# smu-ivpl/FastInterCU-VVC

Measured on AMD Instinct MI355X. Metric: CU-inferences/sec (batch 4096, 128x128), higher is better.
Workload: dtype f16 (fp32 accumulate)

## Files before the change

fastintercu-vvc_amd/csrc/mlt_dispatch.cpp:

```cpp
#include "mlt_runtime.h"

const char *tuning_env(const char *name) {
  const char *e = std::getenv("MLT_TUNING");
  return (e && e[0] == '1') ? std::getenv(name) : nullptr;
}

const Tuning &tuning() {
  static const Tuning t = [] {
    auto num = [](const char *name, long dflt) { const char *e = tuning_env(name); return e ? std::atol(e) : dflt; };
    auto on = [](const char *name) { return tuning_env(name) != nullptr; };
    auto cap = [&](const char *name) { const long v = num(name, 0); return (int)(v > 0 ? v : 256); };
    Tuning u{};
    u.debug_dump_dir = tuning_env("MLT_DEBUG_DUMP_DIR");
    u.xl_kill = (int)num("MLT_XL_KILL", 0); u.xl_kill_layer = (int)num("MLT_XL_KILL_LAYER", -1);
    u.lat_pixels = num("MLT_LAT_PIXELS", 16384L);
    u.no_exact_lat = on("MLT_NO_EXACT_LAT"); u.exact_patch_big = !on("MLT_EXACT_PATCH_64K");
    u.wg_cap = cap("MLT_WG_CAP"); u.wg_cap0 = cap("MLT_WG_CAP0"); u.wg_cap1 = cap("MLT_WG_CAP1"); u.wg_cap2 = cap("MLT_WG_CAP2");
    u.l0_mfma32 = on("MLT_L0_MFMA32"); u.l1_mfma32 = !on("MLT_L1_MFMA16");
    u.no_block_fusion = on("MLT_NO_BLOCK_FUSION");
    u.no_chain = on("MLT_NO_CHAIN") || u.no_block_fusion; u.no_chain_s2 = on("MLT_NO_CHAIN_S2"); u.no_c16 = on("MLT_NO_C16"); u.chain64 = !on("MLT_NO_CHAIN64");
    u.no_l0_s5 = on("MLT_NO_L0_S5");
    u.l0_stream_min = on("MLT_NO_L0_STREAM") ? 0 : (int)num("MLT_L0_STREAM_MIN", 128);
    u.l1_stream_min = on("MLT_NO_L1_STREAM") ? 0 : (int)num("MLT_L1_STREAM_MIN", 128);
    u.guard_wait_mode = on("MLT_GUARD_SPIN_WAIT") ? 1 : on("MLT_GUARD_BLOCKING_WAIT") ? 2 : 0;
    u.no_small_mix = on("MLT_NO_SMALL_MIX"); u.no_mag_guard = on("MLT_NO_MAG_GUARD");
    u.no_graph = on("MLT_NO_GRAPH") || u.debug_dump_dir != nullptr;
    return u;
  }();
  return t;
}

namespace {

int gap_slots(int hw) { return hw >= 32 ? hw / 32 : 1; }

size_t ws_per_cu(const mlt::Model &m, int S, bool some_exact = false) {
  const int h0 = S / 2 > 0 ? S / 2 : 1;
  const int planes = (m.exact || some_exact) ? 2 : 1;
  size_t b = 4 * ((size_t)h0 * h0 * 32 * 2 * planes + 256);
  int h = S;
  for (int s = 0; s < m.n_stages; ++s) {
    h = h / 2 > 0 ? h / 2 : 1;
    b += (size_t)h * h * m.planes[s] * 2 * planes + 256;
    if (s >= 1) b += (size_t)gap_slots(h * h) * m.planes[s] * 4 + 256;
  }
  return b + 4096;
}

int ensure_ws(mlt_ctx *ctx, size_t bytes) {
  if (bytes <= ctx->ws_bytes) return MLT_OK;
  if (ctx->ws) { HIP_TRY(ctx, hipStreamSynchronize(ctx->stream)); (void)hipFree(ctx->ws); ctx->ws = nullptr; ctx->ws_bytes = 0; }
  ++ctx->ws_gen;
  HIP_TRY(ctx, hipMalloc((void **)&ctx->ws, bytes));
  ctx->ws_bytes = bytes;
  return MLT_OK;
}
}
void release_ws(mlt_ctx *ctx) {
  if (ctx->ws) { (void)hipFree(ctx->ws); ctx->ws = nullptr; ctx->ws_bytes = 0; }
  ++ctx->ws_gen;
}
namespace {

int debug_dump(mlt_ctx *ctx, const char *name, const void *dptr, size_t bytes) {
  const char *dir = tuning().debug_dump_dir;
  static int seq = 0;
  if (!dir) return MLT_OK;
  std::vector<char> host(bytes);
  HIP_TRY(ctx, hipStreamSynchronize(ctx->stream));
  HIP_TRY(ctx, hipMemcpy(host.data(), dptr, bytes, hipMemcpyDeviceToHost));
  char path[1200];
  std::snprintf(path, sizeof path, "%s/%02d_%s.bin", dir, seq++, name);
  if (FILE *f = std::fopen(path, "wb")) { std::fwrite(host.data(), 1, bytes, f); std::fclose(f); }
  return MLT_OK;
}

}

int Launch::prof_begin(const std::string &name, double flops, double bytes, hipEvent_t &e0, hipEvent_t &e1, const char *variant) {
  if (ctx->plan) { ctx->plan->push_back(variant && variant[0] ? name + " [" + variant + "]" : name); return MLT_OK; }
  if (!ctx->profile) return MLT_OK;
  auto it = ctx->prof.find(name);
  if (it == ctx->prof.end()) { ctx->prof_order.push_back(name); it = ctx->prof.emplace(name, ProfAcc()).first; }
  it->second.launches++; it->second.flops += flops; it->second.bytes += bytes;
  HIP_TRY(ctx, hipEventCreate(&e0));
  HIP_TRY(ctx, hipEventCreate(&e1));
  it->second.ev.emplace_back(e0, e1);
  HIP_TRY(ctx, hipEventRecord(e0, ctx->stream));
  return MLT_OK;
}
int Launch::prof_end(hipEvent_t e1) {
  if (!ctx->profile) return MLT_OK;
  HIP_TRY(ctx, hipEventRecord(e1, ctx->stream));
  return MLT_OK;
}

namespace {

void plan_note(mlt_ctx *ctx, std::initializer_list<std::pair<const char *, const void *>> ptrs, std::initializer_list<std::pair<const char *, long>> vals = {}) {
  if (!ctx->plan || !ctx->plan_detail || ctx->plan->empty()) return;
  std::string t = " {";
  char b[64];
  bool first = true;
  for (const auto &q : ptrs) {
    if (!q.second) continue;
    std::snprintf(b, sizeof b, "%s%s=0x%llx", first ? "" : " ", q.first, (unsigned long long)(uintptr_t)q.second);
    t += b; first = false;
  }
  for (const auto &q : vals) {
    std::snprintf(b, sizeof b, "%s%s=%ld", first ? "" : " ", q.first, q.second);
    t += b; first = false;
  }
  ctx->plan->back() += t + "}";
}

struct ConvIO {
  const void *x = nullptr;
  void *y = nullptr;
  void *y_sc = nullptr;
  const void *res = nullptr;
  float *gap = nullptr;
  bool relu = false;
  bool y_c16 = false;
  bool ysc_c16 = false;
  size_t x_lo = 0, y_lo = 0, res_lo = 0, ysc_lo = 0;
};

int run_conv(mlt_ctx *ctx, const mlt::PackedConv &pc, int n, int hin, const ConvIO &io, int *hout_out) {
  const int hout = hin / pc.stride > 0 ? hin / pc.stride : 1;
  *hout_out = hout;
  ConvArgs a{};
  a.x = io.x; a.y = io.y; a.w = pc.d_w; a.bias = pc.d_bias; a.res = io.res; a.n = n; a.relu = io.relu ? 1 : 0;
  a.y_sc = io.y_sc; a.bias_sc = pc.d_bias_sc; a.acc_scale = pc.acc_scale; a.y_c16 = io.y_c16 ? 1 : 0; a.ysc_c16 = io.ysc_c16 ? 1 : 0;
  a.hin_l = ilog2(hin); a.hout_l = ilog2(hout);
  a.x_lo_off = io.x_lo; a.y_lo_off = io.y_lo; a.res_lo_off = io.res_lo; a.ysc_lo_off = io.ysc_lo; a.w_lo_off = pc.plane_halves * 2;
  a.lo8_scale = 0x01010101 * ((127 - pc.lo8_exp) & 0xFF);
  a.xl_sa0 = 0x01010101 * ((127 - pc.xl_ewl) & 0xFF); a.xl_sa1 = 0x01010101 * ((127 - pc.xl_ewh) & 0xFF); a.xl_sb1 = 0x01010101 * (127 - 12);
  { const int kill = tuning().xl_kill, only = tuning().xl_kill_layer;
    if (only < 0 || only == pc.cin * 1000 + pc.cout) { if (kill & 1) a.xl_sa0 = 0; if (kill & 2) a.xl_sb1 = 0; } }
  const long lat_px = tuning().lat_pixels;
  const bool no_exact_lat = tuning().no_exact_lat;
  const bool lat = !(pc.exact && no_exact_lat) && pc.lat && hout >= 8 && (pc.w2 ? pc.stride == 1 : (long)n * hout * hout <= lat_px);
  const int dma = (pc.exact || pc.w2 || lat) ? 0 : (pc.dma == 1 && hout >= 16) ? 1 : (pc.dma == 2 && hout >= 8) ? 2 : 0;
  const int MT = lat ? 128 : dma == 2 ? pc.mt_dma : pc.mt;
  const int nsplit = pc.xl ? 6 : pc.exact ? 2 : pc.w2 ? 4 : 1;
  const int act_planes = (nsplit == 2 || nsplit == 6) ? 2 : 1;
  int tw = hout < 32 ? hout : 32;
  int th = MT / tw < hout ? MT / tw : hout;
  int spw = MT / (tw * th);
  const int halo = pc.taps == 9 ? 3 : 1;
  const int PS = pc.kc * 2 + 16;
  const int ph = (th - 1) * pc.stride + halo, pw = (tw - 1) * pc.stride + halo;
  int half = pc.stride == 2 ? (pw + 1) / 2 : 0;
  if (pc.stride == 2 && tw == 8 && (2 * half) % 4 != 2) ++half;
  int rp = pc.stride == 2 ? 2 * half : pw;
  if (pc.stride == 1 && tw == 8) while (rp % 4 != 2) ++rp;
  size_t patch_budget = 64 * 1024;
  if (nsplit == 2 || nsplit == 6) {
    const int tt = pc.taps + (pc.has_sc ? 1 : 0), nbuf = tt / pc.gt > 1 ? 2 : 1;
    const size_t ring = (size_t)nbuf * 2 * pc.gt * (pc.kc / 16) * (pc.ct / 32) * 1024;
    const bool big = tuning().exact_patch_big;
    if (big && ring + 64 * 1024 < 160 * 1024) patch_budget = 160 * 1024 - ring;
  }
  while (spw > 1 && (((size_t)spw * ph * rp * PS + 1023) / 1024 * 1024) * act_planes > patch_budget) spw /= 2;
  a.tw_l = ilog2(tw); a.th_l = ilog2(th); a.spw_l = ilog2(spw);
  a.ph = ph; a.pw = pw; a.rp = rp; a.half = half;
  auto magic = [](int d) { return d < 2 ? 0u : (uint32_t)((0x100000000ull + d - 1) / d); };
  a.pw_magic = magic(pw); a.ph_magic = magic(ph);
  a.patch_bytes = (int)((((size_t)spw * ph * rp * PS) + 1023) / 1024 * 1024);
  if (dma) {
    a.patch_bytes = (int)((((size_t)spw * ph * rp * pc.kc * 2) + 1023) / 1024 * 1024);
    a.rp_magic = magic(rp);
    a.zero = ctx->zero_page;
  }
  const int extra_lds = 0;
  const int hw = hout * hout;
  a.gap = io.gap; a.gap_slots = gap_slots(hw); a.gap_l = hw >= 32 ? 5 : ilog2(hw);
  a.ntiles = ((n + spw - 1) / spw) * (hout / th) * (hout / tw);
  const int wg_cap = tuning().wg_cap;
  const int gt = (nsplit == 4 && !lat) ? pc.gt_w2 : pc.gt;
  const bool persistent = (gt == pc.taps + (pc.has_sc ? 1 : 0) && pc.cin == pc.kc) || dma == 2;
  const int cap = dma == 2 ? wg_cap * ((pc.mt_dma >= 256 || pc.stride == 2) ? 1 : 2) / (pc.cout / pc.ct) : wg_cap;
  const int grid_x = (persistent && a.ntiles > cap) ? cap : a.ntiles;
  char name[48];
  std::snprintf(name, sizeof name, "conv3x3_s%d_%dto%d_h%d%s", pc.stride, pc.cin, pc.cout, hout, pc.has_sc ? "+sc" : "");
  const double px = (double)n * hw;
  const double flops = 2.0 * px * pc.cout * pc.cin * (pc.taps + (pc.has_sc ? 1 : 0));
  const double in_bytes = (double)n * hin * hin * pc.cin * 2;
  const double bytes = in_bytes + px * pc.cout * 2 * ((io.y ? 1 : 0) + (io.y_sc ? 1 : 0) + (io.res ? 1 : 0)) + (double)pc.w.size() * 2;
  Launch L{ctx};
  hipEvent_t e0 = nullptr, e1 = nullptr;
  char variant[96];
  std::snprintf(variant, sizeof variant, "%s%s%s%s%s", nsplit == 1 ? "single pass" : nsplit == 2 ? "exact" : nsplit == 4 ? "hi+lo weights" : nsplit == 6 ? "exact-lite" : "?",
                pc.taps == 1 ? ", centre tap" : lat ? ", latency tiles" : dma == 1 ? ", resident weights + LDS-DMA patches" : dma == 2 ? ", weight ring + LDS-DMA" : "",
                io.y_c16 ? ", y chunk-major" : "", io.ysc_c16 ? ", sc chunk-major" : "", io.gap ? ", GAP" : "");
  int rc = L.prof_begin(name, flops, bytes, e0, e1, variant);
  if (rc) return rc;
  plan_note(ctx, {{"x", io.x}, {"y", io.y}, {"y_sc", io.y_sc}, {"res", io.res}, {"gap", io.gap}},
            {{"x_lo", (long)io.x_lo}, {"y_lo", (long)io.y_lo}, {"res_lo", (long)io.res_lo}, {"ysc_lo", (long)io.ysc_lo}, {"relu", io.relu}, {"grid", grid_x}});
  LAUNCH_TRY(ctx, mlt_launch_conv(pc.cin, pc.cout, pc.stride, nsplit, pc.taps == 1 ? MLT_CONV_CENTRE : lat ? MLT_CONV_LATENCY : dma ? MLT_CONV_DMA : MLT_CONV_DEFAULT, a, grid_x, extra_lds, ctx->stream));
  if ((rc = L.prof_end(e1))) return rc;
  if (io.y && (rc = debug_dump(ctx, name, io.y, (size_t)px * pc.cout * 2))) return rc;
  if (io.y_sc && (rc = debug_dump(ctx, (std::string(name) + "_sc").c_str(), io.y_sc, (size_t)px * pc.cout * 2))) return rc;
  return MLT_OK;
}

int run_stem5(mlt_ctx *ctx, const mlt::PackedConv &pc, int n, int S, const Planes &pl, void *y, void *y_sc, size_t lo_off) {
  const int hout = S / 2;
  Stem5Args a{};
  pl.fill(a);
  a.w = pc.d_w; a.bias = pc.d_bias; a.bias_sc = pc.d_bias_sc; a.y = y; a.y_sc = y_sc;
  a.y_lo_off = lo_off; a.ysc_lo_off = lo_off; a.w_lo_off = pc.plane_halves * 2; a.acc_scale = pc.acc_scale;
  a.n = n; a.s_l = ilog2(S); a.hout_l = ilog2(hout);
  const int MT = 256;
  const int tw = hout < 32 ? hout : 32;
  const int th = MT / tw < hout ? MT / tw : hout;
  const int spw = MT / (tw * th);
  a.tw_l = ilog2(tw); a.th_l = ilog2(th); a.spw_l = ilog2(spw);
  a.rh = 2 * th + 3; a.rw = 2 * tw + 3; a.halfw = (a.rw + 1) / 2;
  a.rw_magic = (uint32_t)((0x100000000ull + a.rw - 1) / a.rw);
  a.rh_magic = (uint32_t)((0x100000000ull + a.rh - 1) / a.rh);
  const int lds = spw * a.rh * 2 * a.halfw * 4;
  const int grid_x = ((n + spw - 1) / spw) * (hout / th) * (hout / tw);
  char name[48];
  std::snprintf(name, sizeof name, "stem5x5_s2_2to32_h%d+sc", hout);
  const double px = (double)n * hout * hout;
  Launch L{ctx};
  hipEvent_t e0 = nullptr, e1 = nullptr;
  int rc = L.prof_begin(name, 2.0 * px * 32 * (50 + 18), (double)n * S * S * 4 + px * 32 * 2 * 2, e0, e1, pc.xl ? "exact-lite" : pc.exact ? "exact" : pc.w2 ? "hi+lo weights" : "single pass");
  if (rc) return rc;
  plan_note(ctx, {{"y", y}, {"y_sc", y_sc}}, {{"lo", (long)lo_off}, {"grid", grid_x}});
  LAUNCH_TRY(ctx, mlt_launch_stem5(a, pc.exact ? 2 : pc.w2 ? 3 : 1, grid_x, lds, ctx->stream));
  if ((rc = L.prof_end(e1))) return rc;
  if ((rc = debug_dump(ctx, name, y, (size_t)px * 32 * 2))) return rc;
  return debug_dump(ctx, (std::string(name) + "_sc").c_str(), y_sc, (size_t)px * 32 * 2);
}

int run_stem_block(mlt_ctx *ctx, const mlt::Model &m, int n, int S, const Planes &pl, void *y, int32_t *d_flat, bool flat_is_clear) {
  const int h = S / 2;
  const mlt::PackedConv &c2 = m.blocks[0][0].conv2;
  StemBlockArgs a{};
  pl.fill(a);
  a.w = m.stem_b.d_w; a.w2 = c2.d_w; a.bias = m.stem.d_bias; a.bias_sc = m.stem.d_bias_sc; a.bias2 = c2.d_bias; a.y = y;
  a.flat = d_flat;
  a.w_lo_off = m.stem_b.plane_halves * 2; a.w2_lo_off = c2.plane_halves * 2; a.scale2 = c2.acc_scale;
  if (d_flat && !flat_is_clear) LAUNCH_TRY(ctx, hipMemsetAsync(d_flat, 0, (size_t)n * 4, ctx->stream));
  a.acc_scale = m.stem.acc_scale; a.n = n; a.hout_l = ilog2(h); a.ntiles = n * (h / 16) * (h / 32);
  const int wg_cap = tuning().wg_cap2;
  const int grid_x = a.ntiles > wg_cap ? wg_cap : a.ntiles;
  char name[48];
  std::snprintf(name, sizeof name, "stem+block_s2_2to32_h%d(layer0.0)", h);
  const double px = (double)n * h * h;
  Launch L{ctx};
  hipEvent_t e0 = nullptr, e1 = nullptr;
  int rc = L.prof_begin(name, 2.0 * px * 32 * (50 + 18 + 288), (double)n * S * S * 4 + px * 32 * 2, e0, e1, m.w2 ? "hi+lo weights" : "single pass");
  if (rc) return rc;
  plan_note(ctx, {{"y", y}, {"flat", d_flat}}, {{"flat_is_clear", flat_is_clear}, {"grid", grid_x}});
  LAUNCH_TRY(ctx, mlt_launch_stem_block(a, m.w2, grid_x, ctx->stream));
  if ((rc = L.prof_end(e1))) return rc;
  return debug_dump(ctx, name, y, (size_t)px * 32 * 2);
}

int run_layer0_stream(mlt_ctx *ctx, const mlt::Model &m0, const mlt::Model &m1, int n, const Planes &pl, void *y, int32_t *d_flat, bool flat_is_clear,
                      const mlt::PackedConv *c5, void *y_t, void *y_sc) {
  const mlt::PackedConv &c2 = m0.blocks[0][0].conv2;
  const mlt::Block &B1 = m1.blocks[0][1];
  Layer0Args a{};
  pl.fill(a);
  a.w = m0.stem_b.d_w; a.w2 = c2.d_w; a.w3 = B1.conv1.d_w; a.w4 = B1.conv2.d_w;
  a.bias = m0.stem.d_bias; a.bias_sc = m0.stem.d_bias_sc; a.bias2 = c2.d_bias; a.bias3 = B1.conv1.d_bias; a.bias4 = B1.conv2.d_bias;
  a.y = y; a.flat = d_flat; a.acc_scale = m0.stem.acc_scale; a.n = n;
  if (c5) { a.w5 = c5->d_w; a.bias5 = c5->d_bias; a.bias5_sc = c5->d_bias_sc; a.scale5 = c5->acc_scale; a.y_t = y_t; a.y_sc = y_sc; }
  if (d_flat && !flat_is_clear) LAUNCH_TRY(ctx, hipMemsetAsync(d_flat, 0, (size_t)n * 4, ctx->stream));
  const int wg_cap = tuning().wg_cap0;
  const int grid_x = n > wg_cap ? wg_cap : n;
  const double px = (double)n * 64 * 64;
  Launch L{ctx};
  hipEvent_t e0 = nullptr, e1 = nullptr;
  int rc = c5 ? L.prof_begin("layer0_stream_h64(stem+layer0+layer1.0.conv1+sc)", 2.0 * px * 32 * (50 + 18 + 3 * 288) + 2.0 * (px / 4) * 64 * (288 + 32),
                             (double)n * 128 * 128 * 4 + (px / 4) * 64 * 2 * 2, e0, e1)
              : L.prof_begin("layer0_stream_h64(stem+layer0.0+layer0.1)", 2.0 * px * 32 * (50 + 18 + 3 * 288), (double)n * 128 * 128 * 4 + px * 32 * 2, e0, e1);
  if (rc) return rc;
  const bool mfma32 = tuning().l0_mfma32;
  plan_note(ctx, {{"y", c5 ? nullptr : y}, {"y_t", c5 ? y_t : nullptr}, {"y_sc", c5 ? y_sc : nullptr}, {"flat", d_flat}}, {{"flat_is_clear", flat_is_clear}, {"grid", grid_x}});
  LAUNCH_TRY(ctx, mlt_launch_layer0_stream(a, c5 != nullptr, mfma32, grid_x, ctx->stream));
  if ((rc = L.prof_end(e1))) return rc;
  if (c5) {
    if ((rc = debug_dump(ctx, "conv3x3_s2_32to64_h32+sc", y_t, (size_t)(px / 4) * 64 * 2))) return rc;
    return debug_dump(ctx, "conv3x3_s2_32to64_h32+sc_sc", y_sc, (size_t)(px / 4) * 64 * 2);
  }
  return debug_dump(ctx, "block_s1_32_h64(conv1+conv2)", y, (size_t)px * 32 * 2);
}

int run_block32(mlt_ctx *ctx, const mlt::Block &B, int n, int h, const void *x, void *y) {
  Block32Args a{};
  const bool w2 = B.conv1.w2;
  a.x = x; a.y = y; a.w1 = B.conv1.d_w; a.w2 = B.conv2.d_w; a.bias1 = B.conv1.d_bias; a.bias2 = B.conv2.d_bias;
  a.w1_lo_off = B.conv1.plane_halves * 2; a.w2_lo_off = B.conv2.plane_halves * 2; a.scale1 = B.conv1.acc_scale; a.scale2 = B.conv2.acc_scale;
  a.n = n; a.h_l = ilog2(h); a.ntiles = n * (h / (w2 ? 8 : 16)) * (h / 32);
  const int wg_cap = tuning().wg_cap;
  const int grid_x = a.ntiles > wg_cap ? wg_cap : a.ntiles;
  char name[48];
  std::snprintf(name, sizeof name, "block_s1_32_h%d(conv1+conv2)", h);
  const double px = (double)n * h * h;
  Launch L{ctx};
  hipEvent_t e0 = nullptr, e1 = nullptr;
  int rc = L.prof_begin(name, 2.0 * px * 32 * 32 * 9 * 2, px * 32 * 2 * 2 + 2.0 * 18 * 1024, e0, e1, w2 ? "hi+lo weights" : "single pass");
  if (rc) return rc;
  plan_note(ctx, {{"x", x}, {"y", y}}, {{"grid", grid_x}});
  LAUNCH_TRY(ctx, mlt_launch_block32(a, w2, grid_x, ctx->stream));
  if ((rc = L.prof_end(e1))) return rc;
  return debug_dump(ctx, name, y, (size_t)px * 32 * 2);
}

int run_chain3(mlt_ctx *ctx, const mlt::Block &B0, const mlt::Block &B1, int n, int h, const void *t, const void *sc, void *y, float *gap,
               const void *s2_in, bool x_c16, bool y_c16, void *b0_hbm, bool sc_c16) {
  const int c = B0.conv2.cout;
  ChainArgs a{};
  a.x = s2_in ? s2_in : t; a.nconv = 3; a.y = y; a.gap = gap; a.n = n; a.zero = ctx->zero_page;
  a.x_c16 = x_c16 ? 1 : 0; a.y_c16 = y_c16 ? 1 : 0; a.res0_c16 = sc_c16 ? 1 : 0;
  const mlt::PackedConv *pcs[3] = {&B0.conv2, &B1.conv1, &B1.conv2};
  const bool w2 = B0.conv2.w2;
  for (int k = 0; k < 3; ++k) {
    a.cv[k].w = pcs[k]->d_w; a.cv[k].bias = pcs[k]->d_bias; a.cv[k].acc_scale = pcs[k]->acc_scale; a.cv[k].relu = 1;
    a.cv[k].w_lo_off = pcs[k]->plane_halves * 2;
    a.cv[k].lo8_scale = 0x01010101 * ((127 - pcs[k]->lo8_exp) & 0xFF);
  }
  a.cv[0].res_mode = s2_in ? 2 : 1; a.cv[0].res = sc; a.cv[0].save = 1; a.cv[2].res_mode = 2;
  if (c == 64) {
    a.cv[0].save = 0; a.cv[0].y = b0_hbm; a.cv[2].res_mode = 1; a.cv[2].res = b0_hbm;
  }
  if (s2_in) {
    const mlt::PackedConv &p2 = B0.conv1_s2c;
    a.s2_w = p2.d_w; a.s2_bias = p2.d_bias; a.s2_bias_sc = p2.d_bias_sc; a.s2_scale = p2.acc_scale;
  }
  const int hw = h * h;
  a.gap_slots = gap_slots(hw); a.gap_l = hw >= 32 ? 5 : ilog2(hw);
  const int wg_cap = tuning().wg_cap;
  const int spw = c == 256 ? 2 : 1;
  const int ntiles = (n + spw - 1) / spw;
  const int grid_x = ntiles > wg_cap ? wg_cap : ntiles;
  char name[48];
  std::snprintf(name, sizeof name, s2_in ? "stage_%d_h%d(s2+sc,conv2,conv1,conv2)" : "chain3_s1_%d_h%d(conv2+conv1+conv2)", c, h);
  const double px = (double)n * hw;
  const double flops = 3.0 * 2.0 * px * c * c * 9 + (s2_in ? 2.0 * px * c * (c / 2) * 10 : 0.0);
  const double bytes = (s2_in ? px * 4 * (c / 2) * 2 : px * c * 2 * 2) + (y ? px * c * 2 : 0.0) + 3.0 * (double)B0.conv2.w.size() * 2 +
                       (s2_in ? (double)B0.conv1_s2c.w.size() * 2 : 0.0);
  Launch L{ctx};
  hipEvent_t e0 = nullptr, e1 = nullptr;
  char variant[96];
  std::snprintf(variant, sizeof variant, "%s%s%s%s%s", w2 ? "hi+lo weights" : "single pass", x_c16 ? ", x chunk-major" : "", sc_c16 ? ", sc chunk-major" : "", y_c16 ? ", y chunk-major" : "",
                gap ? ", GAP" : "");
  int rc = L.prof_begin(name, flops, bytes, e0, e1, variant);
  if (rc) return rc;
  plan_note(ctx, {{"x", a.x}, {"sc", s2_in ? nullptr : sc}, {"y", y}, {"gap", gap}, {"b0", c == 64 ? b0_hbm : nullptr}}, {{"grid", grid_x}});
  LAUNCH_TRY(ctx, mlt_launch_chain(c, h, s2_in != nullptr, ctx->lds_oob_zero, w2, a, grid_x, ctx->stream));
  if ((rc = L.prof_end(e1))) return rc;
  if (y && (rc = debug_dump(ctx, name, y, (size_t)px * c * 2))) return rc;
  return MLT_OK;
}

int run_layer1_stream(mlt_ctx *ctx, const mlt::Block &B0, const mlt::Block &B1, int n, const void *t, const void *sc, void *y, float *gap, bool y_c16) {
  Layer1Args a{};
  a.t = t; a.sc = sc; a.y = y; a.y_c16 = y_c16 ? 1 : 0; a.gap = gap; a.gap_slots = gap_slots(32 * 32); a.n = n;
  const mlt::PackedConv *pcs[3] = {&B0.conv2, &B1.conv1, &B1.conv2};
  for (int k = 0; k < 3; ++k) { a.w[k] = pcs[k]->d_w; a.bias[k] = pcs[k]->d_bias; a.scale[k] = pcs[k]->acc_scale; }
  const int wg_cap = tuning().wg_cap1;
  const int grid_x = n > wg_cap ? wg_cap : n;
  const double px = (double)n * 32 * 32;
  Launch L{ctx};
  hipEvent_t e0 = nullptr, e1 = nullptr;
  int rc = L.prof_begin("layer1_stream_h32(conv2+conv1+conv2)", 3.0 * 2.0 * px * 64 * 64 * 9, px * 64 * 2 * 3 + 3.0 * 72 * 1024, e0, e1, y_c16 ? "single pass, y chunk-major, GAP" : "single pass, GAP");
  if (rc) return rc;
  const bool mfma32 = tuning().l1_mfma32;
  plan_note(ctx, {{"t", t}, {"sc", sc}, {"y", y}, {"gap", gap}}, {{"grid", grid_x}});
  LAUNCH_TRY(ctx, mlt_launch_layer1_stream(a, mfma32, grid_x, ctx->stream));
  if ((rc = L.prof_end(e1))) return rc;
  return debug_dump(ctx, "chain3_s1_64_h32(conv2+conv1+conv2)", y, (size_t)px * 64 * 2);
}

enum : unsigned { CLS_QUADS = 1u, CLS_FLAT = 2u, CLS_L0_STREAM = 4u, CLS_L1_STREAM = 8u, CLS_CHAIN0 = 16u  };
unsigned batch_class(const NetCfg &c, int n, const Planes &pl, bool has_flat) {
  const Tuning &tn = tuning();
  unsigned cls = 0;
  if (pl.aligned8()) cls |= CLS_QUADS;
  if (has_flat) cls |= CLS_FLAT;
  if (tn.l0_stream_min > 0 && n >= tn.l0_stream_min) cls |= CLS_L0_STREAM;
  if (tn.l1_stream_min > 0 && n >= tn.l1_stream_min) cls |= CLS_L1_STREAM;
  for (int s = 1; s < c.m->n_stages; ++s) {
    const int h = c.h_in(s), ho = h / 2 > 0 ? h / 2 : 1;
    if ((long)n * ho * ho > tn.lat_pixels) cls |= CLS_CHAIN0 << s;
  }
  return cls;
}


NetPlan plan_network(const mlt_ctx *ctx, const NetCfg &c, unsigned cls) {
  const Tuning &tn = tuning();
  const mlt::Model &m = *c.m;
  NetPlan P;
  auto add = [&](PlanStep::Kind k, int s) -> PlanStep & { PlanStep st{}; st.kind = k; st.s = (int8_t)s; P.push_back(st); return P.back(); };
  auto wants_chain = [&](int s) -> bool {
    if (s <= 0 || s >= m.n_stages || tn.no_chain || !(cls & (CLS_CHAIN0 << s))) return false;
    const mlt::Model &mm = c.model_of(s, 1);
    if (mm.exact || (mm.w2 && !ctx->lds_oob_zero)) return false;
    const int h = c.h_in(s), ho = h / 2 > 0 ? h / 2 : 1;
    const mlt::PackedConv &c2 = mm.blocks[s][0].conv2;
    const bool packing_ok = (m.planes[s] == 64 ? (c2.ct == 64 && c2.gt == 9 && tn.chain64) : (c2.ct == 128 && c2.gt == 3)) && (!mm.w2 || c2.lo8 || m.planes[s] == 64);
    return mlt_chain_supported(m.planes[s], ho) && c2.taps == 9 && c2.kc == 64 && packing_ok;
  };
  auto wants_s2 = [&](int s) -> bool {
    if (!wants_chain(s) || tn.no_chain_s2 || c.model_of(s, 0).w2 || c.model_of(s, 1).w2) return false;
    const mlt::PackedConv &p2 = c.model_of(s, 0).blocks[s][0].conv1_s2c;
    return ctx->plan ? !p2.w.empty() : p2.d_w != nullptr;
  };
  bool cur_c16 = false;
  bool l0_front = false;
  for (int s = 0; s < m.n_stages; ++s) {
    const bool last = s == m.n_stages - 1;
    const mlt::Model &ms = c.model_of(s, 0);
    const mlt::Model &mt = c.model_of(s, 1);
    const int h = c.h_in(s), ho = h / 2 > 0 ? h / 2 : 1;
    const bool fused_b0 = s == 0 && !ms.exact && ho >= 32 && !tn.no_block_fusion && (cls & CLS_QUADS);
    if (s == 0 && (cls & CLS_FLAT) && !fused_b0) add(PlanStep::FLAT_STAT, 0);
    if (fused_b0 && ho == 64 && !ms.w2 && !mt.exact && !mt.w2 && (cls & CLS_L0_STREAM)) {
      const mlt::Model &m10 = c.model_of(1, 0);
      const mlt::PackedConv &c5 = m10.blocks[1][0].conv1;
      l0_front = !tn.no_l0_s5 && m.n_stages > 1 && !m10.exact && !m10.w2 && wants_chain(1) && !wants_s2(1) && m.planes[1] == 64 && !tn.no_c16 &&
                 c5.has_sc && c5.taps == 9 && c5.kc == 32 && c5.ct == 64 && c5.cin == 32 && c5.cout == 64 && c5.stride == 2;
      add(PlanStep::LAYER0_STREAM, 0).front = l0_front;
      continue;
    }
    if (fused_b0) add(PlanStep::STEM_BLOCK, 0);
    else {
      const bool chain = wants_chain(s), chain_s2 = wants_s2(s);
      bool sc_c16 = false;
      if (s == 0) add(PlanStep::STEM5, 0);
      else if (chain_s2) {}
      else if (s == 1 && l0_front) sc_c16 = true;
      else {
        sc_c16 = chain && m.planes[s] == 64 && !tn.no_c16 && !ms.exact;
        add(PlanStep::CONV_S2, s).sc_c16 = sc_c16;
      }
      if (chain) {
        const bool out_c16 = !last && !tn.no_c16 && wants_s2(s + 1);
        const mlt::PackedConv &q2 = mt.blocks[s][0].conv2;
        const bool stream = s == 1 && !chain_s2 && m.planes[s] == 64 && ho == 32 && sc_c16 && !mt.w2 && !mt.exact && (cls & CLS_L1_STREAM) &&
                            q2.taps == 9 && q2.kc == 64 && q2.ct == 64 && !last;
        PlanStep &st = add(stream ? PlanStep::LAYER1_STREAM : PlanStep::CHAIN, s);
        st.inside_s2 = chain_s2; st.x_c16 = cur_c16; st.sc_c16 = sc_c16; st.y_c16 = out_c16;
        cur_c16 = out_c16;
        continue;
      }
      add(PlanStep::CONV_B0C2, s);
    }
    if (s == 0 && !mt.exact && ho >= 32 && !tn.no_block_fusion) { add(PlanStep::BLOCK32, 0); continue; }
    add(PlanStep::CONV_B1C1, s);
    PlanStep &st = add(PlanStep::CONV_B1C2, s);
    st.y_c16 = !last && !tn.no_c16 && wants_s2(s + 1);
    cur_c16 = st.y_c16;
  }
  add(PlanStep::HEADS, m.n_stages - 1);
  return P;
}

}

int run_network(mlt_ctx *ctx, SizeState &st, const NetCfg &c, int n, const PassIO &io, const GuardOut &go) {
  const int S = st.size;
  mlt::Model &m = *c.m;
  const unsigned cls = batch_class(c, n, io.pl, go.d_flat != nullptr);
  NetPlan fresh;
  const NetPlan *plan;
  if (st.loaded && !ctx->plan) {
    const PlanKey key{c.m, c.mback, c.mx, c.back_mask, c.x_units, cls};
    auto it = st.plans.find(key);
    if (it == st.plans.end()) it = st.plans.emplace(key, plan_network(ctx, c, cls)).first;
    plan = &it->second;
  } else {
    fresh = plan_network(ctx, c, cls);
    plan = &fresh;
  }
  int rc = ctx->plan ? MLT_OK : ensure_ws(ctx, ws_per_cu(m, S, c.x_units != 0) * (size_t)n);
  if (rc) return rc;
  char *p = ctx->ws;
  auto carve = [&](size_t bytes) { char *r = p; p += (bytes + 255) / 256 * 256; return (void *)r; };
  const int h0 = S / 2 > 0 ? S / 2 : 1;
  const int nplanes = (m.exact || c.x_units) ? 2 : 1;
  void *pool[4];
  for (int i = 0; i < 4; ++i) pool[i] = carve((size_t)n * h0 * h0 * 32 * 2 * nplanes);
  void *outs[5];
  float *gaps[5] = {nullptr, nullptr, nullptr, nullptr, nullptr};
  {
    int h = S;
    for (int s = 0; s < m.n_stages; ++s) {
      h = h / 2 > 0 ? h / 2 : 1;
      outs[s] = carve((size_t)n * h * h * m.planes[s] * 2 * nplanes);
      if (s >= 1) gaps[s] = (float *)carve((size_t)n * gap_slots(h * h) * m.planes[s] * 4);
    }
  }
  Launch L{ctx};
  const bool quad_ok = (cls & CLS_QUADS) != 0;
  for (const PlanStep &ps : *plan) {
    const int s = ps.s;
    const bool last = s == m.n_stages - 1;
    mlt::Model &ms = c.model_of(s, 0), &mt = c.model_of(s, 1);
    const int h = c.h_in(s), ho = h / 2 > 0 ? h / 2 : 1;
    const void *cur = s > 0 ? outs[s - 1] : nullptr;
    const bool ex0 = ms.exact, ex1 = mt.exact;
    const size_t lo_in = ex0 ? (size_t)n * h * h * (s == 0 ? 32 : m.planes[s - 1]) * 2 : 0;
    const size_t lo_st = (ex0 || ex1) ? (size_t)n * ho * ho * m.planes[s] * 2 : 0;
    const bool in_has_lo = s > 0 && c.model_of(s - 1, 1).exact;
    const bool b0_has_lo = s == 0 ? ex0 : ex1;
    int hh = 0;
    ConvIO cv;
    switch (ps.kind) {
    case PlanStep::FLAT_STAT: {
      FlatStatArgs fa{};
      io.pl.fill(fa);
      fa.flat = go.d_flat; fa.n = n; fa.s_l = ilog2(S);
      hipEvent_t e0 = nullptr, e1 = nullptr;
      if ((rc = L.prof_begin("guard_flat_stat", 0.0, (double)n * S * S * 4, e0, e1))) return rc;
      plan_note(ctx, {{"flat", go.d_flat}}, {{"quads", quad_ok}});
      LAUNCH_TRY(ctx, mlt_launch_flat_stat(fa, quad_ok, ctx->stream));
      rc = L.prof_end(e1);
      break;
    }
    case PlanStep::LAYER0_STREAM:
      rc = run_layer0_stream(ctx, ms, mt, n, io.pl, outs[0], go.d_flat, go.flat_is_clear,
                             ps.front ? &c.model_of(1, 0).blocks[1][0].conv1 : nullptr, pool[0], pool[1]);
      break;
    case PlanStep::STEM_BLOCK:
      rc = run_stem_block(ctx, ms, n, S, io.pl, pool[2], go.d_flat, go.flat_is_clear);
      break;
    case PlanStep::STEM5:
      rc = run_stem5(ctx, ms.stem, n, S, io.pl, pool[0], pool[1], lo_st);
      break;
    case PlanStep::CONV_S2:
      cv.x = cur; cv.y = pool[0]; cv.y_sc = pool[1]; cv.relu = true;
      cv.x_lo = in_has_lo ? lo_in : 0; cv.y_lo = lo_st; cv.ysc_lo = lo_st;
      cv.ysc_c16 = ps.sc_c16;
      rc = run_conv(ctx, ms.blocks[s][0].conv1, n, h, cv, &hh);
      break;
    case PlanStep::CHAIN:
      rc = run_chain3(ctx, mt.blocks[s][0], mt.blocks[s][1], n, ho, pool[0], pool[1], last ? nullptr : outs[s], gaps[s], ps.inside_s2 ? cur : nullptr,
                      ps.x_c16, ps.y_c16, pool[2], ps.sc_c16);
      break;
    case PlanStep::LAYER1_STREAM:
      rc = run_layer1_stream(ctx, mt.blocks[s][0], mt.blocks[s][1], n, pool[0], pool[1], outs[s], gaps[s], ps.y_c16);
      break;
    case PlanStep::CONV_B0C2:
      cv.x = pool[0]; cv.y = pool[2]; cv.res = pool[1]; cv.relu = true;
      cv.x_lo = cv.y_lo = cv.res_lo = lo_st;
      if (s > 0 && ex1 && !ex0) cv.x_lo = cv.res_lo = 0;
      rc = run_conv(ctx, (s == 0 ? ms : mt).blocks[s][0].conv2, n, ho, cv, &hh);
      break;
    case PlanStep::BLOCK32:
      rc = run_block32(ctx, mt.blocks[0][1], n, ho, pool[2], outs[0]);
      break;
    case PlanStep::CONV_B1C1:
      cv.x = pool[2]; cv.y = pool[3]; cv.relu = true;
      cv.x_lo = cv.y_lo = lo_st;
      if (!b0_has_lo) cv.x_lo = 0;
      rc = run_conv(ctx, mt.blocks[s][1].conv1, n, ho, cv, &hh);
      break;
    case PlanStep::CONV_B1C2:
      cv.x = pool[3]; cv.y = last ? nullptr : outs[s]; cv.res = pool[2]; cv.relu = true; cv.gap = gaps[s];
      cv.x_lo = cv.y_lo = cv.res_lo = lo_st;
      if (!b0_has_lo) cv.res_lo = 0;
      cv.y_c16 = ps.y_c16;
      rc = run_conv(ctx, mt.blocks[s][1].conv2, n, ho, cv, &hh);
      break;
    case PlanStep::HEADS: {
      HeadArgs ha{};
      for (int t = 1; t < m.n_stages; ++t) {
        const int hd = t - 1, hs = c.h_in(t + 1);
        ha.gap[hd] = gaps[t]; ha.slots[hd] = gap_slots(hs * hs); ha.w[hd] = m.heads[hd].d_w; ha.b[hd] = m.heads[hd].d_b;
        ha.c[hd] = m.planes[t]; ha.hw[hd] = hs * hs; ha.classes[hd] = m.heads[hd].classes;
      }
      ha.n_heads = m.n_heads; ha.decision_head = st.head_index; ha.poc = io.poc; ha.qp = io.qp; ha.logits = io.logits; ha.split = io.split;
      ha.mag = go.d_mag;
      ha.dec = io.dec; ha.min_conf = st.min_conf;
      ha.cand = io.cand; ha.cand_cov = st.cand_cov; ha.cand_max = st.cand_max;
      const GuardTail *tail = go.tail;
      if (tail && (n == 1 || tail->next)) {
        ha.g_conf_band = tail->conf_band; ha.g_cand_band = tail->cand_band;
        ha.g_next = tail->next;
        ha.g_count = tail->count; ha.g_idx = tail->idx; ha.g_flat = tail->flat; ha.g_flat_thr = tail->flat_thr; ha.g_near_thr = tail->near_thr; ha.g_margin = tail->margin;
        ha.g_mag_thr = tail->mag_thr;
      }
      hipEvent_t e0 = nullptr, e1 = nullptr;
      if (io.sweep.n_qps > 0) {
        HeadSweepArgs sa{};
        sa.h = ha; sa.h.mag = nullptr;
        sa.n_qps = io.sweep.n_qps; sa.slab = io.sweep.slab; sa.fix_idx = io.sweep.idx; sa.mask = io.sweep.mask; sa.active = io.sweep.idx ? nullptr : io.sweep.active;
        std::memcpy(sa.qps, io.sweep.qps, sizeof sa.qps);
        if ((rc = L.prof_begin("heads_sweep", 0.0, 0.0, e0, e1))) return rc;
        LAUNCH_TRY(ctx, mlt_launch_heads_sweep(sa, n, ctx->stream));
        rc = L.prof_end(e1);
        break;
      }
      if ((rc = L.prof_begin("heads", 0.0, 0.0, e0, e1))) return rc;
      plan_note(ctx, {{"gap0", ha.gap[0]}, {"gap1", ha.gap[1]}, {"gap2", ha.gap[2]}, {"gap3", ha.gap[3]}},
                {{"slots0", ha.slots[0]}, {"slots1", ha.slots[1]}, {"slots2", ha.slots[2]}, {"slots3", ha.slots[3]}, {"c0", ha.c[0]}, {"c1", ha.c[1]}, {"c2", ha.c[2]}, {"c3", ha.c[3]},
                 {"hw0", ha.hw[0]}, {"hw1", ha.hw[1]}, {"hw2", ha.hw[2]}, {"hw3", ha.hw[3]}, {"heads", ha.n_heads}});
      LAUNCH_TRY(ctx, mlt_launch_heads(ha, n, ctx->stream));
      rc = L.prof_end(e1);
      break;
    }
    }
    if (rc) return rc;
  }
  return MLT_OK;
}

extern "C" {
#pragma GCC visibility push(default)

int mlt_plan_describe(const void *blob, size_t bytes, int size, int n, int tier, unsigned w2_units, unsigned x_units, int aligned, char *out, size_t cap) {
  const int si = size_index(size);
  if (!blob || !out || cap == 0 || si < 0 || n <= 0) return -1;
  mlt_ctx ctx;
  std::vector<std::string> plan;
  ctx.plan = &plan;
  ctx.plan_detail = (aligned & 2) != 0;
  ctx.lds_oob_zero = true;
  SizeState &st = ctx.sz[si];
  st.size = size; st.enabled = st.loaded = true;
  st.head_index = size == 128 ? 2 : 0;
  std::string err;
  const bool whole_exact = tier == 1 || tier == 5;
  if (!mlt::build_model(blob, bytes, tier == 5 ? mlt::MLT_MODEL_XLITE : tier == 1 ? mlt::MLT_MODEL_EXACT : mlt::MLT_MODEL_FAST, size, st.model, err)) return -1;
  if (!whole_exact && w2_units && !mlt::build_model(blob, bytes, mlt::MLT_MODEL_W2, size, st.model_w2, err)) return -1;
  if (!whole_exact && x_units && !mlt::build_model(blob, bytes, mlt::MLT_MODEL_EXACT, size, st.model_exact, err)) return -1;
  st.exact = whole_exact;
  st.w2 = !whole_exact && w2_units != 0; st.w2_units = st.w2 ? w2_units : 0; st.x_units = whole_exact ? 0 : x_units;
  const int16_t *planes = (const int16_t *)(uintptr_t)((aligned & 1) ? 0x1000 : 0x1002);
  int32_t *const flat_fake = (int32_t *)(uintptr_t)0x2000;
  ctx.ws = (char *)(uintptr_t)0x100000000ull;
  GuardOut go;
  go.d_flat = whole_exact ? nullptr : flat_fake;
  const int rc = run_network(&ctx, st, st.main_cfg(), n, PassIO{Planes::dense(planes, planes, size), nullptr, nullptr, nullptr, nullptr, nullptr}, go);
  ctx.ws = nullptr;
  if (rc) return -1;
  size_t pos = 0;
  for (const std::string &l : plan) {
    if (pos + l.size() + 2 > cap) return -1;
    std::memcpy(out + pos, l.data(), l.size());
    pos += l.size();
    out[pos++] = '\n';
  }
  out[pos] = 0;
  return (int)plan.size();
}

#pragma GCC visibility pop
}
```

fastintercu-vvc_amd/csrc/mlt_kernels.h:

```cpp
#pragma once
#include <hip/hip_runtime.h>
#include <stdint.h>

#define MLT_MAX_HEADS_K 4
#define MLT_MAX_LOGITS_K 16
#define MLT_FLAT_RANGE 6
#define MLT_FLAT_EXACT_SHIFT 16

struct ConvArgs {
  const void *x;
  void *y;
  const void *w;
  const float *bias;
  const void *res;
  const void *zero;
  int n;
  int ntiles;
  int hin_l, hout_l;
  int tw_l, th_l, spw_l;
  int ph, pw, rp, half;
  uint32_t pw_magic, ph_magic, rp_magic;
  int patch_bytes;
  int relu;
  int y_c16;
  int ysc_c16;
  float acc_scale;
  void *y_sc;
  const float *bias_sc;
  float *gap;
  int gap_slots, gap_l;
  size_t x_lo_off, y_lo_off, res_lo_off, ysc_lo_off, w_lo_off;
  int lo8_scale;
  int xl_sa0, xl_sa1, xl_sb1;
};

struct ConvCfg { int kc, ct, mt, gt, dma, mt_dma, lat, gt_w2; };

struct Stem5Args {
  const int16_t *org, *pred;
  long org_row_stride, org_cu_stride, pred_row_stride, pred_cu_stride;
  const void *w;
  const float *bias, *bias_sc;
  void *y, *y_sc;
  size_t y_lo_off, ysc_lo_off, w_lo_off;
  float acc_scale;
  int n, s_l, hout_l, tw_l, th_l, spw_l;
  int rh, rw, halfw;
  uint32_t rw_magic, rh_magic;
};

struct Block32Args {
  const void *x;
  void *y;
  const void *w1, *w2;
  const float *bias1, *bias2;
  int n, h_l, ntiles;
  size_t w1_lo_off, w2_lo_off;
  float scale1, scale2;
};

struct StemBlockArgs {
  const int16_t *org, *pred;
  long org_row_stride, org_cu_stride, pred_row_stride, pred_cu_stride;
  const void *w;
  const void *w2;
  const float *bias, *bias_sc, *bias2;
  void *y;
  int32_t *flat;
  float acc_scale;
  int n, hout_l, ntiles;
  size_t w_lo_off, w2_lo_off;
  float scale2;
};

#define MLT_L0F_LDS_BYTES 161040
#define MLT_L0_LDS_BYTES 145872
struct Layer0Args {
  const int16_t *org, *pred;
  long org_row_stride, org_cu_stride, pred_row_stride, pred_cu_stride;
  const void *w;
  const void *w2, *w3, *w4;
  const float *bias, *bias_sc, *bias2, *bias3, *bias4;
  void *y;
  int32_t *flat;
  float acc_scale;
  int n;
  const void *w5;
  const float *bias5, *bias5_sc;
  void *y_t, *y_sc;
  float scale5;
};

#define MLT_L1_LDS_BYTES 159008
struct Layer1Args {
  const void *t;
  const void *sc;
  const void *w[3];
  const float *bias[3];
  float scale[3];
  void *y;
  int y_c16;
  float *gap;
  int gap_slots, n;
};

struct ChainConv {
  const void *w;
  size_t w_lo_off;
  int lo8_scale;
  const float *bias;
  float acc_scale;
  int relu;
  int res_mode;
  int save;
  const void *res;
  void *y;
};
struct ChainArgs {
  const void *x;
  const void *s2_w;
  const float *s2_bias, *s2_bias_sc;
  float s2_scale;
  const void *zero;
  ChainConv cv[3];
  int nconv;
  void *y;
  int y_c16;
  int x_c16;
  int res0_c16;
  float *gap;
  int gap_slots, gap_l;
  int n;
};
hipError_t mlt_launch_chain(int c, int h, bool with_s2, bool oob_zero, bool w2, const ChainArgs &a, int grid_x, hipStream_t st);
bool mlt_chain_supported(int c, int h);
hipError_t mlt_probe_lds_oob(int *d_ok, hipStream_t st);
bool mlt_stage_supported(int c, int h);

struct DecisionRec {
  int32_t split_mode, raw_mode;
  float confidence, margin;
  int32_t level_mode[MLT_MAX_HEADS_K];
  float level_conf[MLT_MAX_HEADS_K];
};
#define MLT_CONF_BAND_FRAC 0.75f

#define MLT_MAX_CAND_K 6
struct CandRec {
  uint32_t mask;
  int32_t count;
  int8_t order[8];
  float prob[MLT_MAX_CAND_K];
};

struct HeadArgs {
  const float *gap[MLT_MAX_HEADS_K];
  int slots[MLT_MAX_HEADS_K];
  const float *w[MLT_MAX_HEADS_K];
  const float *b[MLT_MAX_HEADS_K];
  int c[MLT_MAX_HEADS_K], hw[MLT_MAX_HEADS_K], classes[MLT_MAX_HEADS_K];
  int n_heads, decision_head;
  const int32_t *poc, *qp;
  float *logits;
  int32_t *split;
  DecisionRec *dec;
  float min_conf, g_conf_band;
  CandRec *cand;
  float cand_cov, g_cand_band;
  int cand_max;
  int32_t *g_count, *g_idx, *g_flat;
  int g_flat_thr, g_near_thr;
  float g_margin;
  float *mag;
  float g_mag_thr;
  int32_t *g_next;
};

#define MLT_SWEEP_MAX_QPS_K 32
struct HeadSweepArgs {
  HeadArgs h;
  int32_t qps[MLT_SWEEP_MAX_QPS_K];
  int n_qps;
  long slab;
  const int32_t *fix_idx;
  uint32_t *mask;
  const uint32_t *active;
};

struct FlatStatArgs {
  const int16_t *org, *pred;
  long org_row_stride, org_cu_stride, pred_row_stride, pred_cu_stride;
  int32_t *flat;
  int n, s_l;
};
struct GuardSelectArgs {
  const int32_t *flat;
  const float *logits;
  int32_t *idx;
  int32_t *count;
  int n, n_logits, head_off, head_classes;
  int flat_thr;
  int near_thr;
  float margin;
  const float *mag;
  float mag_thr;
  float min_conf, conf_band;
  float cand_cov, cand_band;
  int cand_max;
};
struct GuardGatherArgs {
  const int16_t *org, *pred;
  long org_row_stride, org_cu_stride, pred_row_stride, pred_cu_stride;
  const int32_t *poc, *qp, *idx;
  int16_t *g_org, *g_pred;
  int32_t *g_poc, *g_qp;
  int k, s_l;
};
struct GuardScatterArgs {
  const int32_t *idx, *g_split;
  const float *g_logits;
  int32_t *split;
  float *logits;
  int k, n_logits;
  const DecisionRec *g_dec;
  DecisionRec *dec;
  const CandRec *g_cand;
  CandRec *cand;
};
struct PictureGatherArgs {
  const int16_t *org, *pred;
  long org_pitch, pred_pitch;
  const int32_t *xy;
  int16_t *g_org, *g_pred;
  int c, s_l;
  int vec_org, vec_pred;
};
hipError_t mlt_launch_picture_gather(const PictureGatherArgs &a, hipStream_t st);
#define MLT_TREES_LEVELS 4
#define MLT_TREES_ROW 15
struct TreeNodeRec {
  int32_t x, y;
  int16_t size;
  int8_t depth;
  uint8_t flags;
  int32_t parent, first_child, split_mode;
  float confidence;
  uint32_t cand_mask;
};
struct TreesEntry {
  const int16_t *org, *pred;
  long org_pitch, pred_pitch;
  int32_t vec_org, vec_pred;
  int32_t poc, qp;
};
struct TreesSegs { int32_t *start, *n, *pack_base; };
struct TreeExpandArgs {
  TreeNodeRec *nodes;
  int32_t *xy;
  int32_t *pic;
  int node_cap;
  int lvl_start, lvl_n;
  int size;
  int lvl, n_levels;
  const DecisionRec *dec;
  const CandRec *cand;
  const float *logits;
  int n_logits, head_off, head_classes;
  uint32_t descend_mask;
  int by_candidates;
  const int32_t *next_roots;
  int n_next_roots, root_flags;
  int32_t *count;
  TreesSegs segs;
  int n_pictures;
  int32_t *first_node;
};
struct TreeRasterArgs {
  const TreeNodeRec *nodes;
  const int32_t *pic;
  int lvl_start, lvl_n;
  int blk_l;
  uint8_t *map;
  size_t map_bytes;
  int map_w, map_h;
};
struct PictureGatherMultiArgs {
  const TreesEntry *entries;
  const int32_t *pic;
  const int32_t *xy;
  int16_t *g_org, *g_pred;
  int32_t *g_poc, *g_qp;
  int c, s_l, n_entries;
};
struct TreesPackArgs {
  const TreeNodeRec *nodes; const int32_t *pic; const float *logits; const DecisionRec *dec; const CandRec *cand;
  TreeNodeRec *o_nodes; float *o_logits; DecisionRec *o_dec; CandRec *o_cand;
  TreesSegs segs;
  const int32_t *first_node;
  int n_pictures, n_levels, total;
  int lvl_start[MLT_TREES_LEVELS], n_logits[MLT_TREES_LEVELS];
};
struct TreeSweepExpandArgs {
  TreeNodeRec *nodes;
  int32_t *xy;
  uint32_t *alive, *desc;
  int32_t *pic;
  int32_t *seg_start, *seg_n;
  int n_pictures;
  int node_cap;
  int lvl_start, lvl_n;
  int next_start, next_cap;
  int size, lvl;
  const DecisionRec *dec;
  const CandRec *cand;
  const float *logits;
  long slab;
  int n_qps, n_logits, head_off, head_classes;
  uint32_t descend_mask;
  int by_candidates;
  const int32_t *next_roots;
  int n_next_roots, root_flags;
  int32_t *count;
};
struct TreeSweepRasterArgs {
  const TreeNodeRec *nodes;
  const uint32_t *alive, *desc;
  const int32_t *pic;
  const DecisionRec *dec;
  long slab;
  int lvl_start, lvl_n, blk_l, n_qps, n_pictures;
  uint8_t *map;
  size_t map_bytes;
  int map_w, map_h;
};
struct TreeSweepPackArgs {
  const TreeNodeRec *nodes; const uint32_t *alive, *desc; const DecisionRec *dec; const float *logits; const CandRec *cand;
  const int32_t *pic, *seg_start, *seg_n;
  int n_pictures;
  int32_t *idx, *total, *first_node, *union_nodes;
  TreeNodeRec *o_nodes; float *o_logits; DecisionRec *o_dec; CandRec *o_cand;
  int n_qps, n_levels, node_cap, out_cap;
  int lvl_start[MLT_TREES_LEVELS], lvl_n[MLT_TREES_LEVELS], lvl_cap[MLT_TREES_LEVELS];
  int n_logits[MLT_TREES_LEVELS], head_off[MLT_TREES_LEVELS], head_classes[MLT_TREES_LEVELS], has_cand[MLT_TREES_LEVELS];
};
hipError_t mlt_launch_tree_expand_sweep(const TreeSweepExpandArgs &a, hipStream_t st);
hipError_t mlt_launch_tree_sweep_raster(const TreeSweepRasterArgs &a, hipStream_t st);
hipError_t mlt_launch_tree_sweep_rank(const TreeSweepPackArgs &a, hipStream_t st);
hipError_t mlt_launch_tree_sweep_pack(const TreeSweepPackArgs &a, hipStream_t st);
hipError_t mlt_launch_tree_expand(const TreeExpandArgs &a, hipStream_t st);
hipError_t mlt_launch_tree_raster(const TreeRasterArgs &a, hipStream_t st);
hipError_t mlt_launch_picture_gather_multi(const PictureGatherMultiArgs &a, hipStream_t st);
hipError_t mlt_launch_trees_pack(const TreesPackArgs &a, hipStream_t st);
hipError_t mlt_launch_flat_stat(const FlatStatArgs &a, bool aligned8, hipStream_t st);
hipError_t mlt_launch_guard_select(const GuardSelectArgs &a, hipStream_t st);
hipError_t mlt_launch_guard_gather(const GuardGatherArgs &a, hipStream_t st);
hipError_t mlt_launch_guard_scatter(const GuardScatterArgs &a, hipStream_t st);

enum { MLT_CONV_DEFAULT = 0, MLT_CONV_DMA = 1, MLT_CONV_LATENCY = 2, MLT_CONV_CENTRE = 3 };
bool mlt_conv_has_centre_variant(int cin, int cout);
hipError_t mlt_launch_conv(int cin, int cout, int stride, int nsplit, int variant, const ConvArgs &a, int grid_x, int extra_lds, hipStream_t st);
bool mlt_conv_cfg(int cin, int cout, int stride, int exact, ConvCfg *out);
hipError_t mlt_launch_stem5(const Stem5Args &a, int nsplit, int grid_x, int lds, hipStream_t st);
hipError_t mlt_launch_block32(const Block32Args &a, bool w2, int grid_x, hipStream_t st);
hipError_t mlt_launch_stem_block(const StemBlockArgs &a, bool w2, int grid_x, hipStream_t st);
hipError_t mlt_launch_layer0_stream(const Layer0Args &a, bool fuse5, bool mfma32, int grid_x, hipStream_t st);
hipError_t mlt_launch_layer1_stream(const Layer1Args &a, bool mfma32, int grid_x, hipStream_t st);
hipError_t mlt_launch_heads(const HeadArgs &a, int n, hipStream_t st);
hipError_t mlt_launch_heads_sweep(const HeadSweepArgs &a, int n, hipStream_t st);
```

fastintercu-vvc_amd/csrc/mlt_kernels.hip:

```cpp
#include <hip/hip_runtime.h>
#include <hip/hip_fp16.h>
#include <stdint.h>

#include <atomic>
#include <utility>

#include "mlt_kernels.h"

#ifndef CFG_ASM_PIPE
#define CFG_ASM_PIPE 1
#endif
#ifndef CFG_S2_BIAS_EARLY
#define CFG_S2_BIAS_EARLY 1
#endif
#ifndef CFG_DMA_SPREAD
#define CFG_DMA_SPREAD 5
#endif
#ifndef CFG_RING_FD16
#define CFG_RING_FD16 1
#endif
#ifndef CFG_RING_RES_EARLY
#define CFG_RING_RES_EARLY 1
#endif
#ifndef CFG_BIAS_EARLY
#define CFG_BIAS_EARLY 1
#endif

#ifdef MLT_PHASE_TIMING
__device__ unsigned long long g_phase[16][8];
__device__ unsigned long long g_phase_chain[4][16];
extern "C" __attribute__((visibility("default"))) int mlt_debug_phase_read(unsigned long long *out, int reset) {
  if (hipMemcpyFromSymbol(out, HIP_SYMBOL(g_phase), sizeof(g_phase)) != hipSuccess) return 1;
  if (reset) {
    static unsigned long long z[16][8];
    if (hipMemcpyToSymbol(HIP_SYMBOL(g_phase), z, sizeof(z)) != hipSuccess) return 1;
  }
  return 0;
}
__device__ unsigned long long g_phase_l0[4][8];
extern "C" __attribute__((visibility("default"))) int mlt_debug_phase_read_l0(unsigned long long *out, int reset) {
  if (hipMemcpyFromSymbol(out, HIP_SYMBOL(g_phase_l0), sizeof(g_phase_l0)) != hipSuccess) return 1;
  if (reset) {
    static unsigned long long z[4][8];
    if (hipMemcpyToSymbol(HIP_SYMBOL(g_phase_l0), z, sizeof(z)) != hipSuccess) return 1;
  }
  return 0;
}
extern "C" __attribute__((visibility("default"))) int mlt_debug_phase_read_chain(unsigned long long *out, int reset) {
  if (hipMemcpyFromSymbol(out, HIP_SYMBOL(g_phase_chain), sizeof(g_phase_chain)) != hipSuccess) return 1;
  if (reset) {
    static unsigned long long z[4][16];
    if (hipMemcpyToSymbol(HIP_SYMBOL(g_phase_chain), z, sizeof(z)) != hipSuccess) return 1;
  }
  return 0;
}
#define PHC_STAMP(t_) asm volatile("s_memtime %0\n\ts_waitcnt lgkmcnt(0)" : "=s"(t_)::"memory")
#define PHC_DECL unsigned int phc_acc[16] = {0, 0, 0, 0, 0, 0, 0, 0, 0, 0, 0, 0, 0, 0, 0, 0}; unsigned long long phc_t; PHC_STAMP(phc_t)
#define PHC_MARK(i) do { unsigned long long n_; PHC_STAMP(n_); phc_acc[i] += (unsigned int)(n_ - phc_t); phc_t = n_; } while (0)
#define PHC_FLUSH(id) do { if (threadIdx.x == 0) { for (int i_ = 0; i_ < 16; ++i_) atomicAdd(&g_phase_chain[id][i_], (unsigned long long)phc_acc[i_]); } } while (0)
#define PH_DECL unsigned long long ph_acc[8] = {0, 0, 0, 0, 0, 0, 0, 0}, ph_t = __builtin_readcyclecounter()
#define PH_MARK(i) do { unsigned long long n_ = __builtin_readcyclecounter(); ph_acc[i] += n_ - ph_t; ph_t = n_; } while (0)
#define PH_FLUSH(id) do { if (threadIdx.x == 0) { for (int i_ = 0; i_ < 8; ++i_) atomicAdd(&g_phase[id][i_], ph_acc[i_]); } } while (0)
#else
#define PH_DECL
#define PH_MARK(i)
#define PH_FLUSH(id)
#define PHC_DECL
#define PHC_MARK(i)
#define PHC_FLUSH(id)
#endif

typedef _Float16 half8 __attribute__((ext_vector_type(8)));
typedef _Float16 half4 __attribute__((ext_vector_type(4)));
typedef _Float16 half2v __attribute__((ext_vector_type(2)));
typedef float float16v __attribute__((ext_vector_type(16)));
typedef float float4v __attribute__((ext_vector_type(4)));

#define LDS_PTR(p) ((__attribute__((address_space(3))) void *)(p))
#define GLB_PTR(p) ((const __attribute__((address_space(1))) void *)(p))

__device__ __forceinline__ void glds16(const void *gsrc_lane, void *lds_wave_base) {
  __builtin_amdgcn_global_load_lds(GLB_PTR(gsrc_lane), LDS_PTR(lds_wave_base), 16, 0, 0);
}

template <int... I, class F> __device__ __forceinline__ void static_for_impl(std::integer_sequence<int, I...>, F &&f) {
  (f(std::integral_constant<int, I>{}), ...);
}
template <int N, class F> __device__ __forceinline__ void static_for(F &&f) {
  static_for_impl(std::make_integer_sequence<int, N>{}, static_cast<F &&>(f));
}

template <int OFF> __device__ __forceinline__ void lds_read128(half8 &dst, uint32_t addr) {
  static_assert(OFF >= 0 && OFF < 65536, "ds_read offset field is 16 bits");
  asm volatile("ds_read_b128 %0, %1 offset:%2" : "=v"(dst) : "v"(addr), "n"(OFF) : "memory");
}
template <int N> __device__ __forceinline__ void lds_wait() {
  static_assert(N >= 0 && N <= 15, "lgkmcnt is 4 bits");
  asm volatile("s_waitcnt lgkmcnt(%0)" ::"n"(N) : "memory");
}
__device__ __forceinline__ void lds_touch(half8 &v) { asm volatile("" : "+v"(v)); }

__device__ __forceinline__ void stagger_start(int phases, int units) {
  const int k = ((int)blockIdx.x % phases) * units;
  for (int i = 0; i < k; ++i) __builtin_amdgcn_s_sleep(127);
}

__device__ __forceinline__ uint32_t udiv_magic(uint32_t n, uint32_t magic) { return magic ? __umulhi(n, magic) : n; }

__device__ __forceinline__ uint32_t prep_pair(int16_t so, int16_t sp) {
  uint16_t o = (uint16_t)so, q = (uint16_t)sp;
  uint16_t r = o > q ? o - q : q - o;
  o = o > 1023 ? 1023 : o;
  r = r > 1023 ? 1023 : r;
  half2v hv;
  hv[0] = (_Float16)(float)o;
  hv[1] = (_Float16)(float)r;
  return *(uint32_t *)&hv;
}


__device__ __forceinline__ int quad_flat_bits(uint32_t w0, uint32_t w1, uint32_t w2, uint32_t w3) {
  const half2v a = *(half2v *)&w0, b = *(half2v *)&w1, c = *(half2v *)&w2, d = *(half2v *)&w3;
  const half2v mx = __builtin_elementwise_max(__builtin_elementwise_max(a, b), __builtin_elementwise_max(c, d));
  const half2v mn = __builtin_elementwise_min(__builtin_elementwise_min(a, b), __builtin_elementwise_min(c, d));
  const half2v r = mx - mn;
  const half2v d1 = (a + c) - (b + b), d2 = (b + d) - (c + c);
  const half2v l = __builtin_elementwise_max(__builtin_elementwise_max(d1, -d1), __builtin_elementwise_max(d2, -d2));
  const _Float16 R = (_Float16)MLT_FLAT_RANGE, one = (_Float16)1, zero = (_Float16)0;
  const bool near = (r[0] <= R || l[0] <= one) && (r[1] <= R || l[1] <= one);
  const bool exact = (r[0] == zero || l[0] == zero) && (r[1] == zero || l[1] == zero);
  return (near ? 1 : 0) | (exact ? 2 : 0);
}

typedef int int8v __attribute__((ext_vector_type(8)));
typedef short short2v __attribute__((ext_vector_type(2)));
__device__ __forceinline__ void cvt_frag_fp8(const half8 &v, uint32_t &d0, uint32_t &d1) {
  const half2v top = {(_Float16)448, (_Float16)448};
  const half2v *h = (const half2v *)&v;
  short2v r = {0, 0};
  r = __builtin_amdgcn_cvt_scalef32_pk_fp8_f16(r, __builtin_elementwise_min(h[0], top), 1.0f, false);
  r = __builtin_amdgcn_cvt_scalef32_pk_fp8_f16(r, __builtin_elementwise_min(h[1], top), 1.0f, true);
  d0 = *(uint32_t *)&r;
  short2v q = {0, 0};
  q = __builtin_amdgcn_cvt_scalef32_pk_fp8_f16(q, __builtin_elementwise_min(h[2], top), 1.0f, false);
  q = __builtin_amdgcn_cvt_scalef32_pk_fp8_f16(q, __builtin_elementwise_min(h[3], top), 1.0f, true);
  d1 = *(uint32_t *)&q;
}
__device__ __forceinline__ float16v mfma_lo8(const half8 &a_lo, const half8 &a_hi, const half8 &b_lo, const half8 &b_hi, const float16v &c, int scale_a) {
  int8v a, b;
  const uint32_t *pl = (const uint32_t *)&a_lo, *ph = (const uint32_t *)&a_hi, *ql = (const uint32_t *)&b_lo, *qh = (const uint32_t *)&b_hi;
#pragma unroll
  for (int e = 0; e < 4; ++e) { a[e] = (int)pl[e]; a[4 + e] = (int)ph[e]; b[e] = (int)ql[e]; b[4 + e] = (int)qh[e]; }
  return __builtin_amdgcn_mfma_scale_f32_32x32x64_f8f6f4(a, b, c, 0, 0, 0, scale_a, 0, 0x7F7F7F7F);
}

#define MLT_XL_LO_EXP 12
__device__ __forceinline__ void cvt_frag_fp8_lo(const half8 &v, uint32_t &d0, uint32_t &d1) {
  const half2v top = {(_Float16)0.109375, (_Float16)0.109375}, mul = {(_Float16)4096, (_Float16)4096};
  const half2v *h = (const half2v *)&v;
  short2v r = {0, 0}, q = {0, 0};
  auto prep = [&](half2v x) { return __builtin_elementwise_max(__builtin_elementwise_min(x, top), -top) * mul; };
  r = __builtin_amdgcn_cvt_scalef32_pk_fp8_f16(r, prep(h[0]), 1.0f, false);
  r = __builtin_amdgcn_cvt_scalef32_pk_fp8_f16(r, prep(h[1]), 1.0f, true);
  q = __builtin_amdgcn_cvt_scalef32_pk_fp8_f16(q, prep(h[2]), 1.0f, false);
  q = __builtin_amdgcn_cvt_scalef32_pk_fp8_f16(q, prep(h[3]), 1.0f, true);
  d0 = *(uint32_t *)&r;
  d1 = *(uint32_t *)&q;
}
__device__ __forceinline__ float16v mfma_xl8(const half8 &a_lo, const half8 &a_hi, const half8 &b_lo, const half8 &b_hi, const float16v &c, int scale_a, int scale_b) {
  int8v a, b;
  const uint32_t *pl = (const uint32_t *)&a_lo, *ph = (const uint32_t *)&a_hi, *ql = (const uint32_t *)&b_lo, *qh = (const uint32_t *)&b_hi;
#pragma unroll
  for (int e = 0; e < 4; ++e) { a[e] = (int)pl[e]; a[4 + e] = (int)ph[e]; b[e] = (int)ql[e]; b[4 + e] = (int)qh[e]; }
  return __builtin_amdgcn_mfma_scale_f32_32x32x64_f8f6f4(a, b, c, 0, 0, 0, scale_a, 0, scale_b);
}

typedef uint32_t uint4v __attribute__((ext_vector_type(4)));
__device__ __forceinline__ uint4v pair16(half4 qa, half4 qb) {
  uint32_t ax = ((uint32_t *)&qa)[0], ay = ((uint32_t *)&qa)[1], bx = ((uint32_t *)&qb)[0], by = ((uint32_t *)&qb)[1];
  auto r0 = __builtin_amdgcn_permlane32_swap(ax, bx, false, false);
  auto r1 = __builtin_amdgcn_permlane32_swap(ay, by, false, false);
  uint4v v;
  v[0] = r0[0]; v[1] = r1[0]; v[2] = r0[1]; v[3] = r1[1];
  return v;
}
__device__ __forceinline__ void unpair16(uint4v v, half4 &qa, half4 &qb) {
  auto r0 = __builtin_amdgcn_permlane32_swap(v[0], v[2], false, false);
  auto r1 = __builtin_amdgcn_permlane32_swap(v[1], v[3], false, false);
  ((uint32_t *)&qa)[0] = r0[0]; ((uint32_t *)&qa)[1] = r1[0];
  ((uint32_t *)&qb)[0] = r0[1]; ((uint32_t *)&qb)[1] = r1[1];
}

typedef float float2v __attribute__((ext_vector_type(2)));
template <int Q, class ACC = float16v> __device__ __forceinline__ half4 act_quad(const ACC &A, float scale, const float4v &b, bool has_res, const half4 &r, bool relu, float *x4 = nullptr) {
  half4 out;
#pragma unroll
  for (int ep = 0; ep < 2; ++ep) {
    float2v a2 = {A[4 * Q + 2 * ep], A[4 * Q + 2 * ep + 1]};
    const float2v b2 = {b[2 * ep], b[2 * ep + 1]};
    float2v x2 = a2 * scale + b2;
    if (has_res) {
      const float2v r2 = {(float)r[2 * ep], (float)r[2 * ep + 1]};
      x2 += r2;
    }
    if (x4) { x4[2 * ep] = x2[0]; x4[2 * ep + 1] = x2[1]; }
    half2v h2 = __builtin_convertvector(x2, half2v);
    if (relu) h2 = __builtin_elementwise_max(h2, (half2v){(_Float16)0, (_Float16)0});
    out[2 * ep] = h2[0];
    out[2 * ep + 1] = h2[1];
  }
  return out;
}

#include "mlt_conv_kernels.inc"
#include "mlt_chain_kernel.inc"
#include "mlt_front_kernels.inc"
#include "mlt_layer0_kernel.inc"
#include "mlt_layer1_kernel.inc"
#include "mlt_tail_kernels.inc"
#include "mlt_picture_kernels.inc"
#include "mlt_tree_kernels.inc"

struct DeviceOnce {
  std::atomic<uint64_t> mask[4] = {};
  bool need(int *dev) const {
    if (hipGetDevice(dev) != hipSuccess) *dev = 0;
    return !(mask[(*dev >> 6) & 3].load(std::memory_order_acquire) & (1ull << (*dev & 63)));
  }
  void done(int dev) { mask[(dev >> 6) & 3].fetch_or(1ull << (dev & 63), std::memory_order_release); }
};
template <class K> static hipError_t ensure_big_lds(K kern, DeviceOnce &once) {
  int dev = 0;
  if (!once.need(&dev)) return hipSuccess;
  hipError_t e = hipFuncSetAttribute((const void *)kern, hipFuncAttributeMaxDynamicSharedMemorySize, 160 * 1024);
  if (e == hipSuccess) once.done(dev);
  return e;
}
template <int CIN, int COUT, int STRIDE, int TAPS, bool SC, int KC, int NSPLIT, int WCB, int WPB, int WAVES_C, int WAVES_P, int GT, int RB, int UN, int MINW, bool DMA, int CBP = 0, bool KMAJ = false>
static hipError_t launch_conv_t(const ConvArgs &a, int grid_x, int extra_lds, hipStream_t st) {
  auto kern = conv_mfma_kernel<CIN, COUT, STRIDE, TAPS, SC, KC, NSPLIT, WCB, WPB, WAVES_C, WAVES_P, GT, RB, UN, MINW, DMA, CBP, KMAJ>;
  constexpr int CBT = WCB * WAVES_C;
  constexpr int TT = TAPS + (SC ? 1 : 0);
  constexpr int NBUF = (TT / GT) > 1 ? RB : 1;
  const int patch_lds = (DMA ? 2 : ((NSPLIT == 2 || NSPLIT == 6) ? 2 : 1)) * a.patch_bytes;
  const int patch8 = NSPLIT == 5 ? ((a.patch_bytes / (KC * 2 + 16) + 1) * (KC + 16) + 1023) / 1024 * 1024 : 0;
  const int lds = patch_lds + NBUF * ((NSPLIT == 2 || NSPLIT == 3 || NSPLIT == 6 ? 2 : 1) * GT * (KC / 16) * CBT * 1024 + (NSPLIT == 5 ? GT * CBT * 2048 : 0)) + patch8 + extra_lds;
  static DeviceOnce once;
  if (hipError_t e = ensure_big_lds(kern, once); e != hipSuccess) return e;
  if (lds > 160 * 1024) return hipErrorInvalidValue;
  dim3 grid(grid_x, COUT / (32 * CBT));
  hipLaunchKernelGGL(kern, grid, dim3(64 * WAVES_C * WAVES_P), lds, st, a);
  return hipGetLastError();
}

template <int CIN, int COUT, int STRIDE, bool SC, int KC, int WCB, int WPB, int WAVES_C, int WAVES_P, int GT, int RB, int UNP, int MINW, int NWL, int FD>
static hipError_t launch_ring_dma_t(const ConvArgs &a, int grid_x, hipStream_t st) {
  auto kern = conv_ring_dma_kernel<CIN, COUT, STRIDE, SC, KC, WCB, WPB, WAVES_C, WAVES_P, GT, RB, UNP, MINW, NWL, FD>;
  constexpr int CBT = WCB * WAVES_C, NW = WAVES_C * WAVES_P;
  constexpr int NWP = NWL ? NWL - NWL / 2 : NW - NW / 2;
  const int lds = 2 * a.patch_bytes + RB * GT * (KC / 16) * CBT * 1024 + (NWL ? 32 * CBT * 4 * (SC ? 2 : 1) : 0);
  static DeviceOnce once;
  if (hipError_t e = ensure_big_lds(kern, once); e != hipSuccess) return e;
  if (lds > 160 * 1024 || (a.patch_bytes >> 10) > UNP * NWP) return hipErrorInvalidValue;
  dim3 grid(grid_x, COUT / (32 * CBT));
  hipLaunchKernelGGL(kern, grid, dim3(64 * (NW + NWL)), lds, st, a);
  return hipGetLastError();
}

#ifndef CFG_3264_GT
#define CFG_3264_GT 10
#endif
#ifndef CFG_3264_RB
#define CFG_3264_RB 1
#endif
#ifndef CFG_S1_RB
#define CFG_S1_RB 2
#endif
#ifndef CFG_64_WPB
#define CFG_64_WPB 1
#endif
#ifndef CFG_64_WP
#define CFG_64_WP 8
#endif
#ifndef CFG_64_WCB
#define CFG_64_WCB 2
#endif
#ifndef CFG_64_WC
#define CFG_64_WC 1
#endif
#ifndef CFG_S2BIG_WCB
#define CFG_S2BIG_WCB 2
#endif
#ifndef CFG_S2BIG_WC
#define CFG_S2BIG_WC 2
#endif
#ifndef CFG_BIG_WPB
#define CFG_BIG_WPB 1
#endif
#ifndef CFG_BIG_WP
#define CFG_BIG_WP 8
#endif
#ifndef CFG_GTE_S1
#define CFG_GTE_S1 1
#endif
#ifndef CFG_GTE_S2
#define CFG_GTE_S2 2
#endif
#ifndef CFG_UNE_32
#define CFG_UNE_32 5
#endif
#ifndef CFG_UNE_64
#define CFG_UNE_64 3
#endif
#ifndef CFG_UNE_S2
#define CFG_UNE_S2 3
#endif
#ifndef CFG_BIG_WP_EXACT
#define CFG_BIG_WP_EXACT 4
#endif
#ifndef CFG_BIG_WCB
#define CFG_BIG_WCB 2
#endif
#ifndef CFG_128_WPB
#define CFG_128_WPB CFG_BIG_WPB
#endif
#ifndef CFG_S2BIG_WPB
#define CFG_S2BIG_WPB 1
#endif
#ifndef CFG_S2BIG_WP
#define CFG_S2BIG_WP 4
#endif
#ifndef CFG_3264_WP
#define CFG_3264_WP 4
#endif
#ifndef CFG_3264_UN
#define CFG_3264_UN 5
#endif
#ifndef CFG_3264_WCB
#define CFG_3264_WCB 1
#endif
#ifndef CFG_3264_WC
#define CFG_3264_WC 2
#endif
#ifndef CFG_32_WPB
#define CFG_32_WPB 2
#endif
#ifndef CFG_32_WP
#define CFG_32_WP 8
#endif
#ifndef CFG_64_GT
#define CFG_64_GT 9
#endif
#ifndef CFG_BIG_GT
#define CFG_BIG_GT 3
#endif
#ifndef CFG_S1_MINW
#define CFG_S1_MINW 1
#endif
#ifndef CFG_S2_MINW
#define CFG_S2_MINW 1
#endif
#ifndef CFG_32_MINW
#define CFG_32_MINW 1
#endif
#ifndef CFG_BIG_WC
#define CFG_BIG_WC 2
#endif
#ifndef CFG_64_DMA
#define CFG_64_DMA 1
#endif
#ifndef CFG_64_DMA_UN
#define CFG_64_DMA_UN 6
#endif
#ifndef CFG_BIG_DMA
#define CFG_BIG_DMA 0
#endif
#ifndef CFG_BIG_DMA_WP
#define CFG_BIG_DMA_WP 4
#endif
#ifndef CFG_BIG_DMA_WPB
#define CFG_BIG_DMA_WPB 1
#endif
#ifndef CFG_BIG_DMA_UNP
#define CFG_BIG_DMA_UNP 7
#endif
#ifndef CFG_BIG_DMA_NWL
#define CFG_BIG_DMA_NWL 0
#endif
#ifndef CFG_BIG_DMA_FD
#define CFG_BIG_DMA_FD 2
#endif
#ifndef CFG_BIG_DMA_MINW
#define CFG_BIG_DMA_MINW 4
#endif
#ifndef CFG_BIG_DMA_RB
#define CFG_BIG_DMA_RB 2
#endif
#ifndef CFG_256_DMA_RB
#define CFG_256_DMA_RB (CFG_BIG_DMA_RB > 3 ? 3 : CFG_BIG_DMA_RB)
#endif
#ifndef CFG_S2A_DMA
#define CFG_S2A_DMA 1
#endif
#ifndef CFG_S2B_DMA
#define CFG_S2B_DMA 1
#endif
#ifndef CFG_S2_DMA_RB
#define CFG_S2_DMA_RB 2
#endif
#ifndef CFG_S2A_GT
#define CFG_S2A_GT 5
#endif
#ifndef CFG_S2B_GT
#define CFG_S2B_GT 5
#endif
#ifndef CFG_S2_DMA_NWL
#define CFG_S2_DMA_NWL 0
#endif
#ifndef CFG_S2_DMA_MINW
#define CFG_S2_DMA_MINW 2
#endif
#ifndef CFG_LAT
#define CFG_LAT 1
#endif
#ifndef CFG_LAT_GT
#define CFG_LAT_GT 9
#endif
#ifndef CFG_LAT_GT2
#define CFG_LAT_GT2 10
#endif
struct CfgRow { int cin, cout, stride, kc[2], wcb, wpb, wc, wp, gt[2], dma, wpb_dma, wp_dma, lat; };
static const CfgRow kCfg[] = {
    {32, 32, 1, {32, 32}, 1, CFG_32_WPB, 1, CFG_32_WP, {9, 3}},
    {32, 64, 2, {32, 32}, CFG_3264_WCB, 1, CFG_3264_WC, CFG_3264_WP, {CFG_3264_GT, CFG_GTE_S2}},
    {64, 64, 1, {64, 32}, CFG_64_WCB, CFG_64_WPB, CFG_64_WC, CFG_64_WP, {CFG_64_GT, CFG_GTE_S1}, CFG_64_DMA, 0, 0, CFG_LAT},
    {64, 128, 2, {32, 32}, CFG_S2BIG_WCB, CFG_S2BIG_WPB, CFG_S2BIG_WC, CFG_S2BIG_WP, {2, CFG_GTE_S2}, CFG_S2A_DMA ? 2 : 0, CFG_S2BIG_WPB, CFG_S2BIG_WP, CFG_LAT},
    {128, 128, 1, {64, 32}, CFG_BIG_WCB, CFG_128_WPB, CFG_BIG_WC, CFG_BIG_WP, {CFG_BIG_GT, CFG_GTE_S1}, CFG_BIG_DMA ? 2 : 0, CFG_BIG_DMA_WPB, CFG_BIG_DMA_WP, CFG_LAT},
    {128, 256, 2, {32, 32}, CFG_S2BIG_WCB, CFG_S2BIG_WPB, CFG_S2BIG_WC, CFG_S2BIG_WP, {CFG_S2B_GT, CFG_GTE_S2}, CFG_S2B_DMA ? 2 : 0, CFG_S2BIG_WPB, CFG_S2BIG_WP, CFG_LAT},
    {256, 256, 1, {64, 32}, CFG_BIG_WCB, CFG_BIG_WPB, CFG_BIG_WC, CFG_BIG_WP, {CFG_BIG_GT, CFG_GTE_S1}, CFG_BIG_DMA ? 2 : 0, CFG_BIG_DMA_WPB, CFG_BIG_DMA_WP, CFG_LAT},
    {64, 96, 2, {32, 32}, 3, 1, 1, 4, {1, CFG_GTE_S2}},
    {96, 96, 1, {32, 32}, 3, 1, 1, 4, {3, CFG_GTE_S1}},
    {96, 128, 2, {32, 32}, 2, 2, 2, 2, {2, CFG_GTE_S2}},
};

static int w2_gt(int cin, int cout, int stride, int gt_exact) {
  if (cin == 32 && cout == 32 && stride == 1) return 9;
  if (cin == 32 && cout == 64 && stride == 2) return CFG_3264_GT;
  if (cin == 64 && cout == 128 && stride == 2) return 2;
  if (cin == 128 && cout == 256 && stride == 2) return 2;
  return gt_exact;
}

bool mlt_conv_cfg(int cin, int cout, int stride, int exact, ConvCfg *out) {
  for (const CfgRow &r : kCfg)
    if (r.cin == cin && r.cout == cout && r.stride == stride) {
      out->kc = r.kc[exact ? 1 : 0];
      out->ct = 32 * r.wcb * r.wc;
      out->dma = exact ? 0 : r.dma;
      out->mt = 32 * r.wpb * ((exact && r.cin >= 128 && r.stride == 1) ? CFG_BIG_WP_EXACT : r.wp);
      out->mt_dma = r.dma == 2 ? 32 * r.wpb_dma * r.wp_dma : out->mt;
      out->lat = (r.lat && r.wcb * r.wc == (r.cout == 64 ? 2 : 4)) ? 1 : 0;
      out->gt = r.gt[exact ? 1 : 0];
      out->gt_w2 = w2_gt(r.cin, r.cout, r.stride, r.gt[1]);
      return true;
    }
  return false;
}

#define CONV_CASE2(CIN, COUT, STRIDE, SCF, KCF, KCE, WCB, WPB, WC, WPF, WPE, GTF, GTE, RBF, RBE, UNF, UNE, MWF)                              \
  if (cin == CIN && cout == COUT && stride == STRIDE) {                                                                             \
    if (!exact) return launch_conv_t<CIN, COUT, STRIDE, 9, SCF, KCF, 1, WCB, WPB, WC, WPF, GTF, RBF, UNF, MWF, false>(a, grid_x, extra_lds, st); \
    if (nsplit == 3) return launch_conv_t<CIN, COUT, STRIDE, 9, SCF, KCE, 3, WCB, WPB, WC, WPE, GTE, RBE, UNE, 1, false>(a, grid_x, extra_lds, st); \
    if (nsplit == 6) return launch_conv_t<CIN, COUT, STRIDE, 9, SCF, KCE, 6, WCB, WPB, WC, WPE, GTE, RBE, UNE, 1, false>(a, grid_x, extra_lds, st); \
    return launch_conv_t<CIN, COUT, STRIDE, 9, SCF, KCE, 2, WCB, WPB, WC, WPE, GTE, RBE, UNE, 1, false>(a, grid_x, extra_lds, st);          \
  }
#define CONV_CASE(CIN, COUT, STRIDE, SCF, KCF, KCE, WCB, WPB, WC, WP, GTF, GTE, RBF, RBE, UNF, UNE, MWF) \
  CONV_CASE2(CIN, COUT, STRIDE, SCF, KCF, KCE, WCB, WPB, WC, WP, WP, GTF, GTE, RBF, RBE, UNF, UNE, MWF)

bool mlt_conv_has_centre_variant(int cin, int cout) { return (cin == cout && (cin == 128 || cin == 256)) || (cin == 128 && cout == 256); }

hipError_t mlt_launch_conv(int cin, int cout, int stride, int nsplit, int variant, const ConvArgs &a, int grid_x, int extra_lds, hipStream_t st) {
  if (nsplit == 4) {
    if (stride == 1 && cin == cout && cin >= 64) {
      if (variant != MLT_CONV_LATENCY) return hipErrorInvalidValue;
      if (cin == 64) return launch_conv_t<64, 64, 1, 9, false, 64, 3, 1, 1, 1, 4, 9, 1, 6, 1, false, 2>(a, grid_x, extra_lds, st);
      if (cin == 128) return launch_conv_t<128, 128, 1, 9, false, 64, 5, 1, 1, 1, 4, 3, 2, 6, 1, false, 4>(a, grid_x, extra_lds, st);
      if (cin == 256) return launch_conv_t<256, 256, 1, 9, false, 64, 5, 1, 1, 1, 4, 3, 2, 6, 1, false, 4>(a, grid_x, extra_lds, st);
      return hipErrorInvalidValue;
    }
    if (variant != MLT_CONV_DEFAULT) return hipErrorInvalidValue;
    nsplit = 3;
  }
  const bool exact = nsplit >= 2;
  const bool dma = variant == MLT_CONV_DMA;
  if (variant == MLT_CONV_CENTRE && (nsplit == 3 || nsplit == 6)) return hipErrorInvalidValue;
  if (variant == MLT_CONV_CENTRE) {
    if (cin == 128 && cout == 128 && stride == 1)
      return exact ? launch_conv_t<128, 128, 1, 1, false, 32, 2, CFG_BIG_WCB, 1, CFG_BIG_WC, CFG_BIG_WP_EXACT, 1, 1, 2, 1, false>(a, grid_x, extra_lds, st)
                   : launch_conv_t<128, 128, 1, 1, false, 64, 1, CFG_BIG_WCB, 1, CFG_BIG_WC, CFG_BIG_WP, 1, 1, 2, 1, false>(a, grid_x, extra_lds, st);
    if (cin == 128 && cout == 256 && stride == 2)
      return exact ? launch_conv_t<128, 256, 2, 1, true, 32, 2, CFG_S2BIG_WCB, CFG_S2BIG_WPB, CFG_S2BIG_WC, CFG_S2BIG_WP, 1, 2, 3, 1, false>(a, grid_x, extra_lds, st)
                   : launch_conv_t<128, 256, 2, 1, true, 32, 1, CFG_S2BIG_WCB, CFG_S2BIG_WPB, CFG_S2BIG_WC, CFG_S2BIG_WP, 1, 2, 5, 1, false>(a, grid_x, extra_lds, st);
    if (cin == 256 && cout == 256 && stride == 1)
      return exact ? launch_conv_t<256, 256, 1, 1, false, 32, 2, CFG_BIG_WCB, 1, CFG_BIG_WC, CFG_BIG_WP_EXACT, 1, 1, 2, 1, false>(a, grid_x, extra_lds, st)
                   : launch_conv_t<256, 256, 1, 1, false, 64, 1, CFG_BIG_WCB, 1, CFG_BIG_WC, CFG_BIG_WP, 1, 1, 2, 1, false>(a, grid_x, extra_lds, st);
    return hipErrorInvalidValue;
  }
#if CFG_LAT
  if (variant == MLT_CONV_LATENCY && nsplit == 6) {
    if (cin == 64 && cout == 64 && stride == 1) return launch_conv_t<64, 64, 1, 9, false, 32, 6, 1, 1, 1, 4, CFG_GTE_S1, 2, 4, 1, false, 2>(a, grid_x, extra_lds, st);
    if (cin == 128 && cout == 128 && stride == 1) return launch_conv_t<128, 128, 1, 9, false, 32, 6, 1, 1, 1, 4, CFG_GTE_S1, 2, 4, 1, false, 4>(a, grid_x, extra_lds, st);
    if (cin == 256 && cout == 256 && stride == 1) return launch_conv_t<256, 256, 1, 9, false, 32, 6, 1, 1, 1, 4, CFG_GTE_S1, 2, 4, 1, false, 4>(a, grid_x, extra_lds, st);
    if (cin == 64 && cout == 128 && stride == 2) return launch_conv_t<64, 128, 2, 9, true, 32, 6, 1, 1, 1, 4, CFG_GTE_S2, 2, 5, 1, false, 4>(a, grid_x, extra_lds, st);
    if (cin == 128 && cout == 256 && stride == 2) return launch_conv_t<128, 256, 2, 9, true, 32, 6, 1, 1, 1, 4, CFG_GTE_S2, 2, 5, 1, false, 4>(a, grid_x, extra_lds, st);
    return hipErrorInvalidValue;
  }
  if (variant == MLT_CONV_LATENCY && nsplit == 2) {
    if (cin == 64 && cout == 64 && stride == 1) return launch_conv_t<64, 64, 1, 9, false, 32, 2, 1, 1, 1, 4, CFG_GTE_S1, 2, 4, 1, false, 2>(a, grid_x, extra_lds, st);
    if (cin == 128 && cout == 128 && stride == 1) return launch_conv_t<128, 128, 1, 9, false, 32, 2, 1, 1, 1, 4, CFG_GTE_S1, 2, 4, 1, false, 4>(a, grid_x, extra_lds, st);
    if (cin == 256 && cout == 256 && stride == 1) return launch_conv_t<256, 256, 1, 9, false, 32, 2, 1, 1, 1, 4, CFG_GTE_S1, 2, 4, 1, false, 4>(a, grid_x, extra_lds, st);
    if (cin == 64 && cout == 128 && stride == 2) return launch_conv_t<64, 128, 2, 9, true, 32, 2, 1, 1, 1, 4, CFG_GTE_S2, 2, 5, 1, false, 4>(a, grid_x, extra_lds, st);
    if (cin == 128 && cout == 256 && stride == 2) return launch_conv_t<128, 256, 2, 9, true, 32, 2, 1, 1, 1, 4, CFG_GTE_S2, 2, 5, 1, false, 4>(a, grid_x, extra_lds, st);
    return hipErrorInvalidValue;
  }
  if (variant == MLT_CONV_LATENCY && !exact) {
    if (cin == 64 && cout == 64 && stride == 1) return launch_conv_t<64, 64, 1, 9, false, 64, 1, 1, 1, 1, 4, 9, 1, 6, 1, false, 2>(a, grid_x, extra_lds, st);
    if (cin == 128 && cout == 128 && stride == 1) return launch_conv_t<128, 128, 1, 9, false, 64, 1, 1, 1, 1, 4, CFG_LAT_GT, 2, 6, 1, false, 4>(a, grid_x, extra_lds, st);
    if (cin == 256 && cout == 256 && stride == 1) return launch_conv_t<256, 256, 1, 9, false, 64, 1, 1, 1, 1, 4, CFG_LAT_GT, 2, 6, 1, false, 4>(a, grid_x, extra_lds, st);
    static_assert(CFG_LAT_GT2 == 10, "the stride-2 latency variants take all 10 weight taps of a chunk per step");
    if (cin == 64 && cout == 128 && stride == 2) return launch_conv_t<64, 128, 2, 9, true, 32, 1, 1, 1, 1, 4, CFG_LAT_GT2, 2, 10, 1, false, 4, true>(a, grid_x, extra_lds, st);
    if (cin == 128 && cout == 256 && stride == 2) return launch_conv_t<128, 256, 2, 9, true, 32, 1, 1, 1, 1, 4, CFG_LAT_GT2, 2, 10, 1, false, 4, true>(a, grid_x, extra_lds, st);
    return hipErrorInvalidValue;
  }
#endif
#if CFG_BIG_DMA
  if (dma && !exact && cin == 128 && cout == 128 && stride == 1)
    return launch_ring_dma_t<128, 128, 1, false, 64, CFG_BIG_WCB, CFG_BIG_DMA_WPB, CFG_BIG_WC, CFG_BIG_DMA_WP, CFG_BIG_GT, CFG_BIG_DMA_RB, CFG_BIG_DMA_UNP, CFG_BIG_DMA_MINW, CFG_BIG_DMA_NWL, CFG_BIG_DMA_FD>(a, grid_x, st);
  if (dma && !exact && cin == 256 && cout == 256 && stride == 1)
    return launch_ring_dma_t<256, 256, 1, false, 64, CFG_BIG_WCB, CFG_BIG_DMA_WPB, CFG_BIG_WC, CFG_BIG_DMA_WP, CFG_BIG_GT, CFG_256_DMA_RB, CFG_BIG_DMA_UNP, CFG_BIG_DMA_MINW, CFG_BIG_DMA_NWL, CFG_BIG_DMA_FD>(a, grid_x, st);
#endif
#if CFG_S2A_DMA
  if (dma && !exact && cin == 64 && cout == 128 && stride == 2)
    return launch_ring_dma_t<64, 128, 2, true, 32, CFG_S2BIG_WCB, CFG_S2BIG_WPB, CFG_S2BIG_WC, CFG_S2BIG_WP, CFG_S2A_GT, CFG_S2_DMA_RB, 20, CFG_S2_DMA_MINW, CFG_S2_DMA_NWL, 2>(a, grid_x, st);
#endif
#if CFG_S2B_DMA
  if (dma && !exact && cin == 128 && cout == 256 && stride == 2)
    return launch_ring_dma_t<128, 256, 2, true, 32, CFG_S2BIG_WCB, CFG_S2BIG_WPB, CFG_S2BIG_WC, CFG_S2BIG_WP, CFG_S2B_GT, CFG_S2_DMA_RB, 20, CFG_S2_DMA_MINW, CFG_S2_DMA_NWL, 2>(a, grid_x, st);
#endif
#if CFG_64_DMA
  if (dma && !exact && cin == 64 && cout == 64 && stride == 1)
    return launch_conv_t<64, 64, 1, 9, false, 64, 1, CFG_64_WCB, CFG_64_WPB, CFG_64_WC, CFG_64_WP, 9, 1, CFG_64_DMA_UN, CFG_S1_MINW, true>(a, grid_x, extra_lds, st);
#endif
  if (nsplit == 3 && variant == MLT_CONV_DEFAULT) {
    static_assert(CFG_3264_GT == 10, "32->64 stride-2: all ten weight taps resident");
    if (cin == 32 && cout == 32 && stride == 1) return launch_conv_t<32, 32, 1, 9, false, 32, 3, 1, CFG_32_WPB, 1, CFG_32_WP, 9, 1, 5, 1, false>(a, grid_x, extra_lds, st);
    if (cin == 32 && cout == 64 && stride == 2) return launch_conv_t<32, 64, 2, 9, true, 32, 3, CFG_3264_WCB, 1, CFG_3264_WC, CFG_3264_WP, CFG_3264_GT, 1, CFG_3264_UN, 1, false>(a, grid_x, extra_lds, st);
    if (cin == 64 && cout == 128 && stride == 2) return launch_conv_t<64, 128, 2, 9, true, 32, 3, CFG_S2BIG_WCB, CFG_S2BIG_WPB, CFG_S2BIG_WC, CFG_S2BIG_WP, 2, 2, 5, 1, false>(a, grid_x, extra_lds, st);
    if (cin == 128 && cout == 256 && stride == 2) return launch_conv_t<128, 256, 2, 9, true, 32, 3, CFG_S2BIG_WCB, CFG_S2BIG_WPB, CFG_S2BIG_WC, CFG_S2BIG_WP, 2, 2, 5, 1, false>(a, grid_x, extra_lds, st);
  }
  CONV_CASE(32, 32, 1, false, 32, 32, 1, CFG_32_WPB, 1, CFG_32_WP, 9, 3, 1, 2, 5, CFG_UNE_32, CFG_32_MINW)
  CONV_CASE(32, 64, 2, true, 32, 32, CFG_3264_WCB, 1, CFG_3264_WC, CFG_3264_WP, CFG_3264_GT, CFG_GTE_S2, CFG_3264_RB, 2, CFG_3264_UN, CFG_UNE_32, CFG_32_MINW)
  CONV_CASE(64, 64, 1, false, 64, 32, CFG_64_WCB, CFG_64_WPB, CFG_64_WC, CFG_64_WP, CFG_64_GT, CFG_GTE_S1, CFG_S1_RB, 2, 6, CFG_UNE_64, CFG_S1_MINW)
  CONV_CASE(64, 128, 2, true, 32, 32, CFG_S2BIG_WCB, CFG_S2BIG_WPB, CFG_S2BIG_WC, CFG_S2BIG_WP, 2, CFG_GTE_S2, 2, 2, 5, CFG_UNE_S2, CFG_S2_MINW)
  CONV_CASE2(128, 128, 1, false, 64, 32, CFG_BIG_WCB, CFG_128_WPB, CFG_BIG_WC, CFG_BIG_WP, CFG_BIG_WP_EXACT, CFG_BIG_GT, CFG_GTE_S1, CFG_S1_RB, 2, 3, 2, CFG_S1_MINW)
  CONV_CASE(128, 256, 2, true, 32, 32, CFG_S2BIG_WCB, CFG_S2BIG_WPB, CFG_S2BIG_WC, CFG_S2BIG_WP, CFG_S2B_GT, CFG_GTE_S2, 2, 2, 5, CFG_UNE_S2, CFG_S2_MINW)
  CONV_CASE2(256, 256, 1, false, 64, 32, CFG_BIG_WCB, CFG_BIG_WPB, CFG_BIG_WC, CFG_BIG_WP, CFG_BIG_WP_EXACT, CFG_BIG_GT, CFG_GTE_S1, CFG_S1_RB, 2, 4, 2, CFG_S1_MINW)
  CONV_CASE(64, 96, 2, true, 32, 32, 3, 1, 1, 4, 1, CFG_GTE_S2, 2, 2, 5, 3, 1)
  CONV_CASE(96, 96, 1, false, 32, 32, 3, 1, 1, 4, 3, CFG_GTE_S1, 2, 2, 3, 2, 1)
  CONV_CASE(96, 128, 2, true, 32, 32, 2, 2, 2, 2, 2, CFG_GTE_S2, 2, 2, 5, 3, 1)
  return hipErrorInvalidValue;
}

__global__ __launch_bounds__(64) void lds_oob_probe_kernel(int *ok) {
  extern __shared__ __attribute__((aligned(16))) char smem[];
  const int lane = threadIdx.x;
  *(uint4v *)(smem + 160 * 1024 - 1024 + lane * 16) = uint4v{0xDEADBEEFu, 0xDEADBEEFu, 0xDEADBEEFu, 0xDEADBEEFu};
  __syncthreads();
  half8 v;
  lds_read128<96>(v, 0x100000u + (uint32_t)lane * 16);
  lds_wait<0>();
  lds_touch(v);
  const uint4v u = *(const uint4v *)&v;
  const bool zero = (u[0] | u[1] | u[2] | u[3]) == 0;
  const unsigned long long all = __ballot(zero);
  if (lane == 0) *ok = all == ~0ull ? 1 : 0;
}
hipError_t mlt_probe_lds_oob(int *d_ok, hipStream_t st) {
  static DeviceOnce once;
  hipError_t e = ensure_big_lds(lds_oob_probe_kernel, once);
  if (e != hipSuccess) return e;
  hipLaunchKernelGGL(lds_oob_probe_kernel, dim3(1), dim3(64), 160 * 1024, st, d_ok);
  return hipGetLastError();
}

bool mlt_chain_supported(int c, int h) { return (c == 64 && h == 32) || (c == 128 && h == 16) || (c == 256 && h == 8); }
bool mlt_stage_supported(int c, int h) { return (c == 128 && h == 16) || (c == 256 && h == 8); }

#ifndef CFG_CHAIN64_GT
#define CFG_CHAIN64_GT 2
#endif
#ifndef CFG_CHAIN_FD
#define CFG_CHAIN_FD 2
#endif
#ifndef CFG_CHAIN_SPLIT
#define CFG_CHAIN_SPLIT 1
#endif
#ifndef CFG_CHAINW2_RB
#define CFG_CHAINW2_RB 3
#endif
template <class K> static hipError_t launch_chain_t(K kern, DeviceOnce &once, const ChainArgs &a, int grid_x, int threads, int lds, hipStream_t st) {
  if (hipError_t e = ensure_big_lds(kern, once); e != hipSuccess) return e;
  hipLaunchKernelGGL(kern, dim3(grid_x), dim3(threads), lds, st, a);
  return hipGetLastError();
}
hipError_t mlt_launch_chain(int c, int h, bool with_s2, bool oob_zero, bool w2, const ChainArgs &a, int grid_x, hipStream_t st) {
  static_assert(CFG_BIG_GT == 3 && CFG_BIG_WCB == 2 && CFG_BIG_WC == 2, "chain_kernel reads the packing of the stand-alone 128->128 / 256->256 layers");
  constexpr int lds = 64 * 1024 + 2 * (CFG_BIG_GT * 4 * 4 * 1024);
  static DeviceOnce once[13];
  if (w2) {
    if (!oob_zero || with_s2 || a.nconv != 3) return hipErrorInvalidValue;
    if (c == 64 && h == 32)
      return launch_chain_t(chain_kernel<64, 5, 0, 2, 4, 1, 8, 1, 2, 1, 2, 3, true, false, false, true, true, false>, once[10], a, grid_x, 512, 128 * 1024 + 2 * 16 * 1024, st);
    if (c == 128 && h == 16)
      return launch_chain_t(chain_kernel<128, 4, 0, 2, 2, 2, 4, 1, 2, 1, 2, 3, true, false, true, true, true, true>, once[11], a, grid_x, 512, (64 + 2 * 24 + 32) * 1024, st);
    if (c == 256 && h == 8)
      return launch_chain_t(chain_kernel<256, 3, 1, 2, 1, 2, 4, 1, 2, 1, 2, 3, true, false, true, true, true, true>, once[12], a, grid_x, 512, (64 + 2 * 24 + 32) * 1024, st);
    return hipErrorInvalidValue;
  }
  if (c == 64 && h == 32 && a.nconv == 3 && !with_s2) {
    static_assert(CFG_64_WCB == 2 && CFG_64_WC == 1 && CFG_64_GT == 9, "chain_kernel<64,...> reads the packing of the stand-alone 64->64 layer");
    constexpr int RB64 = CFG_CHAIN64_GT == 1 ? 4 : 2, lds64 = 128 * 1024 + 4 * 8 * 1024;
    if (oob_zero) return launch_chain_t(chain_kernel<64, 5, 0, 2, 4, 1, 8, CFG_CHAIN64_GT, RB64, 1, 2, 3, true, false, false, true>, once[6], a, grid_x, 512, lds64, st);
    return launch_chain_t(chain_kernel<64, 5, 0, 2, 4, 1, 8, CFG_CHAIN64_GT, RB64, 1, 2, 3, true, false, false, false>, once[7], a, grid_x, 512, lds64, st);
  }
  if (c == 128 && h == 16) {
    if (with_s2 && a.nconv == 3) {
      if (oob_zero) return launch_chain_t(chain_kernel<128, 4, 0, 2, 2, 2, 4, 3, 2, CFG_CHAIN_FD, 2, 3, true, true, true, true>, once[4], a, grid_x, 512, lds, st);
      return launch_chain_t(chain_kernel<128, 4, 0, 2, 2, 2, 4, 3, 2, CFG_CHAIN_FD, 2, 3, true, true, true, false>, once[8], a, grid_x, 512, lds, st);
    }
    if (a.nconv == 3) return launch_chain_t(chain_kernel<128, 4, 0, 2, 2, 2, 4, 3, 2, CFG_CHAIN_FD, 2, 3, CFG_CHAIN_SPLIT != 0>, once[0], a, grid_x, 512, lds, st);
    if (a.nconv == 2) return launch_chain_t(chain_kernel<128, 4, 0, 2, 2, 2, 4, 3, 2, CFG_CHAIN_FD, 2, 2, CFG_CHAIN_SPLIT != 0>, once[1], a, grid_x, 512, lds, st);
  }
  if (c == 256 && h == 8) {
    if (with_s2 && a.nconv == 3) {
      if (oob_zero) return launch_chain_t(chain_kernel<256, 3, 1, 2, 1, 2, 4, 3, 2, CFG_CHAIN_FD, 2, 3, true, true, true, true>, once[5], a, grid_x, 512, lds, st);
      return launch_chain_t(chain_kernel<256, 3, 1, 2, 1, 2, 4, 3, 2, CFG_CHAIN_FD, 2, 3, true, true, true, false>, once[9], a, grid_x, 512, lds, st);
    }
    if (a.nconv == 3) return launch_chain_t(chain_kernel<256, 3, 1, 2, 1, 2, 4, 3, 2, CFG_CHAIN_FD, 2, 3, CFG_CHAIN_SPLIT != 0>, once[2], a, grid_x, 512, lds, st);
    if (a.nconv == 2) return launch_chain_t(chain_kernel<256, 3, 1, 2, 1, 2, 4, 3, 2, CFG_CHAIN_FD, 2, 2, CFG_CHAIN_SPLIT != 0>, once[3], a, grid_x, 512, lds, st);
  }
  return hipErrorInvalidValue;
}

hipError_t mlt_launch_stem5(const Stem5Args &a, int nsplit, int grid_x, int lds, hipStream_t st) {
  if (nsplit == 3) hipLaunchKernelGGL(stem5_kernel<3>, dim3(grid_x), dim3(256), lds, st, a);
  else if (nsplit == 2) hipLaunchKernelGGL(stem5_kernel<2>, dim3(grid_x), dim3(256), lds, st, a);
  else hipLaunchKernelGGL(stem5_kernel<1>, dim3(grid_x), dim3(256), lds, st, a);
  return hipGetLastError();
}

hipError_t mlt_launch_block32(const Block32Args &a, bool w2, int grid_x, hipStream_t st) {
  static DeviceOnce once[2];
  if (w2) {
    constexpr int lds = (12 * 36 + 10 * 34) * 80 + 4 * 18 * 1024;
    if (hipError_t e = ensure_big_lds(block32_kernel<3, true>, once[1]); e != hipSuccess) return e;
    hipLaunchKernelGGL((block32_kernel<3, true>), dim3(grid_x), dim3(512), lds, st, a);
    return hipGetLastError();
  }
  constexpr int lds = (20 * 36 + 18 * 34) * 80 + 2 * 18 * 1024;
  if (hipError_t e = ensure_big_lds(block32_kernel<4, false>, once[0]); e != hipSuccess) return e;
  hipLaunchKernelGGL((block32_kernel<4, false>), dim3(grid_x), dim3(512), lds, st, a);
  return hipGetLastError();
}

hipError_t mlt_launch_stem_block(const StemBlockArgs &a, bool w2, int grid_x, hipStream_t st) {
  constexpr int lds = 3 * (39 * 72 * 4 + 16) + 2 * (18 * 34 * 80) + 18 * 1024 + 256 + 2 * 1024;
  static DeviceOnce once[2];
  if (w2) {
    if (hipError_t e = ensure_big_lds(stem_block_kernel<true>, once[1]); e != hipSuccess) return e;
    hipLaunchKernelGGL(stem_block_kernel<true>, dim3(grid_x), dim3(128 * CFG_SB_NWS), lds + 2 * 1024, st, a);
    return hipGetLastError();
  }
  if (hipError_t e = ensure_big_lds(stem_block_kernel<false>, once[0]); e != hipSuccess) return e;
  hipLaunchKernelGGL(stem_block_kernel<false>, dim3(grid_x), dim3(128 * CFG_SB_NWS), lds, st, a);
  return hipGetLastError();
}

template <bool F5, bool M16> static hipError_t launch_layer0_stream_t(const Layer0Args &a, int grid_x, hipStream_t st) {
  static DeviceOnce once;
  if (hipError_t e = ensure_big_lds(layer0_stream_kernel<F5, M16>, once); e != hipSuccess) return e;
  hipLaunchKernelGGL((layer0_stream_kernel<F5, M16>), dim3(grid_x), dim3(1024), F5 ? MLT_L0F_LDS_BYTES : MLT_L0_LDS_BYTES, st, a);
  return hipGetLastError();
}
hipError_t mlt_launch_layer0_stream(const Layer0Args &a, bool fuse5, bool mfma32, int grid_x, hipStream_t st) {
  if (fuse5) return mfma32 ? launch_layer0_stream_t<true, false>(a, grid_x, st) : launch_layer0_stream_t<true, true>(a, grid_x, st);
  return launch_layer0_stream_t<false, false>(a, grid_x, st);
}

hipError_t mlt_launch_layer1_stream(const Layer1Args &a, bool mfma32, int grid_x, hipStream_t st) {
  static DeviceOnce once[2];
  if (mfma32) {
    if (hipError_t e = ensure_big_lds(layer1_stream_kernel<false>, once[0]); e != hipSuccess) return e;
    hipLaunchKernelGGL(layer1_stream_kernel<false>, dim3(grid_x), dim3(1024), MLT_L1_LDS_BYTES, st, a);
    return hipGetLastError();
  }
  if (hipError_t e = ensure_big_lds(layer1_stream_kernel<true>, once[1]); e != hipSuccess) return e;
  hipLaunchKernelGGL(layer1_stream_kernel<true>, dim3(grid_x), dim3(1024), MLT_L1_LDS_BYTES, st, a);
  return hipGetLastError();
}

hipError_t mlt_launch_heads(const HeadArgs &a, int n, hipStream_t st) {
  if (a.cand || a.cand_cov > 0.f || a.cand_max > 0) hipLaunchKernelGGL(heads_cand_kernel, dim3(n), dim3(256), 0, st, a);
  else if (a.dec || a.min_conf > 0.f) hipLaunchKernelGGL(heads_kernel<true>, dim3(n), dim3(256), 0, st, a);
  else hipLaunchKernelGGL(heads_kernel<false>, dim3(n), dim3(256), 0, st, a);
  return hipGetLastError();
}

hipError_t mlt_launch_heads_sweep(const HeadSweepArgs &a, int n, hipStream_t st) {
  if (a.n_qps < 1 || a.n_qps > MLT_SWEEP_MAX_QPS_K || ((a.fix_idx || a.h.g_next) && !a.mask)) return hipErrorInvalidValue;
  hipLaunchKernelGGL(sweep_heads_kernel, dim3(n), dim3(256), 0, st, a);
  return hipGetLastError();
}

hipError_t mlt_launch_flat_stat(const FlatStatArgs &a, bool aligned8, hipStream_t st) {
  if (aligned8) hipLaunchKernelGGL(flat_stat_kernel<true>, dim3(a.n), dim3(256), 0, st, a);
  else hipLaunchKernelGGL(flat_stat_kernel<false>, dim3(a.n), dim3(256), 0, st, a);
  return hipGetLastError();
}

hipError_t mlt_launch_guard_select(const GuardSelectArgs &a, hipStream_t st) {
  hipLaunchKernelGGL(guard_select_kernel, dim3(1), dim3(1024), 0, st, a);
  return hipGetLastError();
}

hipError_t mlt_launch_guard_gather(const GuardGatherArgs &a, hipStream_t st) {
  hipLaunchKernelGGL(guard_gather_kernel, dim3(a.k, 2), dim3(256), 0, st, a);
  return hipGetLastError();
}

hipError_t mlt_launch_guard_scatter(const GuardScatterArgs &a, hipStream_t st) {
  const int items = a.k * (a.n_logits + 1);
  hipLaunchKernelGGL(guard_scatter_kernel, dim3((items + 255) / 256), dim3(256), 0, st, a);
  return hipGetLastError();
}

hipError_t mlt_launch_picture_gather(const PictureGatherArgs &a, hipStream_t st) {
  const size_t items = (size_t)a.c << (2 * a.s_l - 2);
  const size_t want = (items + 255) / 256;
  hipLaunchKernelGGL(picture_gather_kernel, dim3((unsigned)(want < 2048 ? want : 2048)), dim3(256), 0, st, a);
  return hipGetLastError();
}

hipError_t mlt_launch_tree_expand(const TreeExpandArgs &a, hipStream_t st) {
  if (a.n_pictures < 1 || a.n_pictures > MLT_TREES_MAX_PICTURES_K) return hipErrorInvalidValue;
  hipLaunchKernelGGL(tree_expand_kernel, dim3(1), dim3(MLT_TREE_TILE), 0, st, a);
  return hipGetLastError();
}

hipError_t mlt_launch_tree_raster(const TreeRasterArgs &a, hipStream_t st) {
  const size_t items = (size_t)a.lvl_n << (2 * a.blk_l);
  if (!items) return hipSuccess;
  const size_t want = (items + 255) / 256;
  hipLaunchKernelGGL(tree_raster_kernel, dim3((unsigned)(want < 2048 ? want : 2048)), dim3(256), 0, st, a);
  return hipGetLastError();
}

hipError_t mlt_launch_picture_gather_multi(const PictureGatherMultiArgs &a, hipStream_t st) {
  const size_t items = (size_t)a.c << (2 * a.s_l - 2);
  if (!items) return hipSuccess;
  const size_t want = (items + 255) / 256;
  hipLaunchKernelGGL(picture_gather_multi_kernel, dim3((unsigned)(want < 2048 ? want : 2048)), dim3(256), 0, st, a);
  return hipGetLastError();
}

hipError_t mlt_launch_trees_pack(const TreesPackArgs &a, hipStream_t st) {
  if (a.total <= 0) return hipSuccess;
  const int want = (a.total + 255) / 256;
  hipLaunchKernelGGL(tree_pack_kernel, dim3((unsigned)(want < 2048 ? want : 2048)), dim3(256), 0, st, a);
  return hipGetLastError();
}

hipError_t mlt_launch_tree_expand_sweep(const TreeSweepExpandArgs &a, hipStream_t st) {
  if (a.n_qps < 1 || a.n_qps > MLT_SWEEP_MAX_QPS_K || a.n_pictures < 1 || a.n_pictures > MLT_TREES_MAX_PICTURES_K) return hipErrorInvalidValue;
  hipLaunchKernelGGL(tree_expand_sweep_kernel, dim3(1), dim3(MLT_TREE_TILE), 0, st, a);
  return hipGetLastError();
}

hipError_t mlt_launch_tree_sweep_raster(const TreeSweepRasterArgs &a, hipStream_t st) {
  const size_t items = (size_t)a.lvl_n << (2 * a.blk_l);
  if (!items) return hipSuccess;
  const size_t want = (items + 255) / 256;
  hipLaunchKernelGGL(tree_sweep_raster_kernel, dim3((unsigned)(want < 2048 ? want : 2048)), dim3(256), 0, st, a);
  return hipGetLastError();
}

hipError_t mlt_launch_tree_sweep_rank(const TreeSweepPackArgs &a, hipStream_t st) {
  if (a.n_qps < 1 || a.n_qps > MLT_SWEEP_MAX_QPS_K || a.n_pictures < 1 || a.n_pictures > MLT_TREES_MAX_PICTURES_K) return hipErrorInvalidValue;
  hipLaunchKernelGGL(tree_sweep_rank_kernel, dim3((unsigned)(a.n_pictures * a.n_qps)), dim3(MLT_TREE_TILE), 0, st, a);
  return hipGetLastError();
}

hipError_t mlt_launch_tree_sweep_pack(const TreeSweepPackArgs &a, hipStream_t st) {
  if (a.n_qps < 1 || a.n_qps > MLT_SWEEP_MAX_QPS_K || a.n_pictures < 1 || a.n_pictures > MLT_TREES_MAX_PICTURES_K) return hipErrorInvalidValue;
  size_t items = 0;
  for (int l = 0; l < a.n_levels; ++l) items += (size_t)a.lvl_n[l];
  const size_t want = (items * (size_t)a.n_qps + 255) / 256;
  hipLaunchKernelGGL(tree_sweep_pack_kernel, dim3((unsigned)(want < 1 ? 1 : want < 2048 ? want : 2048)), dim3(256), 0, st, a);
  return hipGetLastError();
}
```

fastintercu-vvc_amd/csrc/mlt_layer0_kernel.inc:

```
#ifndef CFG_L0_PD
#define CFG_L0_PD 4
#endif
#ifndef CFG_L0_RD
#define CFG_L0_RD 4
#endif
#ifndef CFG_L0_PRIO
#define CFG_L0_PRIO 0
#endif
#ifndef CFG_L0_XPRE
#define CFG_L0_XPRE 1
#endif
#ifndef CFG_L0_PKEPI
#define CFG_L0_PKEPI 1
#endif
#ifndef CFG_L0_KO
#define CFG_L0_KO 0
#endif
#ifndef CFG_L0_MAP
#define CFG_L0_MAP 0
#endif
template <bool F5, bool M16>
__global__ __launch_bounds__(1024) void layer0_stream_kernel(const Layer0Args a) {
  constexpr int PS = 80, RW = 66, ROWB = RW * PS;
  constexpr int NRT = F5 ? 6 : 8, NRB = 8, NRU = F5 ? 6 : 8, NRO = F5 ? 6 : 0;
  constexpr int RP = 136, RAWB = RP * 4, NRAW = 16;
  typedef uint32_t uint2v __attribute__((ext_vector_type(2)));
  extern __shared__ __attribute__((aligned(16))) char smem[];
  char *Tr = smem, *Br = Tr + NRT * ROWB, *Ur = Br + NRB * ROWB, *Or = Ur + NRU * ROWB, *Z = Or + NRO * ROWB;
  char *Raw = Z + ROWB, *RawZ = Raw + NRAW * RAWB;
  float *BL = (float *)(RawZ + RAWB);
  constexpr int NBL = F5 ? 256 : 128;
  char *WB = (char *)(BL + NBL);
  int *FL = (int *)(WB + 4096);
  char *W5 = (char *)(FL + 4);
  constexpr int ZERO_BYTES = (NRT + NRB + NRU + NRO + 1) * ROWB + (NRAW + 1) * RAWB;
  static_assert(ZERO_BYTES % 16 == 0 && (F5 ? MLT_L0F_LDS_BYTES : MLT_L0_LDS_BYTES) == ZERO_BYTES + NBL * 4 + 4096 + 16 + (F5 ? 4096 : 0), "LDS layout");
  const int tid = threadIdx.x, lane = tid & 63;
  const int wave = __builtin_amdgcn_readfirstlane(tid >> 6);
  const int stage = F5 ? (wave < 2 ? 0 : wave < 4 ? 4 : wave >> 2) : CFG_L0_MAP ? wave & 3 : wave >> 2;
  const int unit = F5 ? wave & 3 : CFG_L0_MAP ? wave >> 2 : wave & 3;
  const int par = unit >> 1, blk = (F5 && stage == 0) ? wave : unit & 1;
  const int p = lane & 31, h = lane >> 5, x = 32 * blk + p;
  const int p16 = lane & 15, g4 = lane >> 4, x16 = 32 * blk + p16;
  if ((int)blockIdx.x >= a.n) return;
  if (CFG_L0_PRIO == 1) { if (stage == 0) __builtin_amdgcn_s_setprio(3); else if (stage == 1) __builtin_amdgcn_s_setprio(2); else if (stage == 2) __builtin_amdgcn_s_setprio(1); }
  if (CFG_L0_PRIO == 2) { if (stage == 3) __builtin_amdgcn_s_setprio(3); else if (stage == 2) __builtin_amdgcn_s_setprio(2); else if (stage == 1) __builtin_amdgcn_s_setprio(1); }
  if (CFG_L0_PRIO == 3) { if (stage == 0) __builtin_amdgcn_s_setprio(3); }
  const int nloc = (a.n - (int)blockIdx.x + (int)gridDim.x - 1) / (int)gridDim.x;
  const int rows_total = 64 * nloc, ksteps = 32 * nloc + (F5 ? 6 : 5);
  for (int o = tid * 16; o < ZERO_BYTES; o += 1024 * 16) *(uint4v *)(smem + o) = uint4v{0u, 0u, 0u, 0u};
  if (tid < 2) FL[tid] = 0;
  if (tid < 32) {
    BL[tid] = a.bias[tid];
    BL[32 + tid] = a.bias2[tid] + a.bias_sc[tid];
    BL[64 + tid] = a.bias3[tid];
    BL[96 + tid] = a.bias4[tid];
    if constexpr (F5) {
      BL[128 + tid] = a.bias5[tid]; BL[160 + tid] = a.bias5[32 + tid];
      BL[192 + tid] = a.bias5_sc[tid]; BL[224 + tid] = a.bias5_sc[32 + tid];
    }
  }
  if (wave < 4) *(uint4v *)(WB + wave * 1024 + lane * 16) = *(const uint4v *)((const char *)a.w + ((wave < 2 ? 7 : 3) + wave) * 1024 + lane * 16);
  if (F5 && wave >= 4 && wave < 8) {
    const int cb = (wave - 4) >> 1, ks = (wave - 4) & 1;
    *(uint4v *)(W5 + (cb * 2 + ks) * 1024 + lane * 16) = *(const uint4v *)((const char *)a.w5 + ((18 + ks) * 2 + cb) * 1024 + lane * 16);
  }
  asm volatile("s_waitcnt vmcnt(0) lgkmcnt(0)\n\ts_barrier" ::: "memory");
  auto read16 = [&](const char *row, int dword_index) -> half8 {
    const uint2v lo = *(const uint2v *)(row + 4 * dword_index), hi = *(const uint2v *)(row + 4 * dword_index + 8);
    uint4v v;
    v[0] = lo[0]; v[1] = lo[1]; v[2] = hi[0]; v[3] = hi[1];
    return *(half8 *)&v;
  };
  auto raw_row = [&](int c, int y) -> const char * { return (y >= 0 && y < 128) ? Raw + ((128 * c + y) & (NRAW - 1)) * RAWB : RawZ; };
  auto slot_of = [&](auto nrc, int g) -> int {
    constexpr int NRr = decltype(nrc)::value;
    if constexpr (NRr == 8) return g & 7;
    else return g - NRr * (int)__umulhi((uint32_t)g, (uint32_t)(0xFFFFFFFFu / NRr + 1));
  };
  auto map_row = [&](char *ring, auto nrc, int g, int r) -> const char * { return (r >= 0 && r < 64) ? ring + slot_of(nrc, g) * ROWB : Z; };
  constexpr std::integral_constant<int, NRT> nrt{};
  constexpr std::integral_constant<int, NRB> nrb{};
  constexpr std::integral_constant<int, NRU> nru{};
  constexpr std::integral_constant<int, NRO ? NRO : 8> nro{};
  const uint32_t lds0 = (uint32_t)(uintptr_t)LDS_PTR(smem);
  auto lds_of = [&](const char *q) -> uint32_t { return lds0 + (uint32_t)(q - smem); };
  auto conv18 = [&](const half8 (&wf)[18], auto &bf, bool pre, const char *rm, const char *r0, const char *rp, int bias_off, float4v (&bq)[4], auto pdc, auto bc) -> float16v {
    constexpr int PD = decltype(pdc)::value;
    constexpr bool BIAS = decltype(bc)::value;
    const int lo = x * PS + h * 16;
    const uint32_t rows[3] = {lds_of(rm) + lo, lds_of(r0) + lo, lds_of(rp) + lo};
    const uint32_t ba = BIAS ? lds_of((const char *)(BL + bias_off + 4 * h)) : 0u;
    static_assert(PD <= 6 && (!BIAS || PD >= 4), "the first PD items lie in one row; bias quads ride in the last four fragment slots");
    auto rd = [&](auto itc) {
      constexpr int item = decltype(itc)::value, tp = item >> 1, ks = item & 1, dy = tp / 3, dx = tp - dy * 3;
      if constexpr (CFG_L0_KO & 1) bf[item % PD] = wf[item];
      else lds_read128<dx * PS + ks * 32>(bf[item % PD], rows[dy]);
    };
    if (!pre) static_for<PD>([&](auto ic) { rd(ic); });
    float16v acc;
#pragma unroll
    for (int r = 0; r < 16; ++r) acc[r] = 0.f;
    static_for<18>([&](auto itc) {
      constexpr int item = decltype(itc)::value;
      constexpr int frags_behind = (17 - item) < (PD - 1) ? (17 - item) : (PD - 1);
      constexpr int bias_behind = !BIAS ? 0 : item - (18 - PD) > 0 ? (item - (18 - PD) < 4 ? item - (18 - PD) : 4) : 0;
      if constexpr (!(CFG_L0_KO & 1)) { lds_wait<frags_behind + bias_behind>(); lds_touch(bf[item % PD]); }
      if (CFG_L0_KO & 2) asm volatile("" ::"v"(bf[item % PD]), "v"(wf[item]));
      else acc = __builtin_amdgcn_mfma_f32_32x32x16_f16(wf[item], bf[item % PD], acc, 0, 0, 0);
      if constexpr (item + PD < 18) rd(std::integral_constant<int, item + PD>{});
      else if constexpr (BIAS && item - (18 - PD) < 4) lds_read128<(item - (18 - PD)) * 32>(bf[item % PD], ba);
    });
    if (CFG_L0_KO & 2) asm volatile("" : "+v"(acc));
    if constexpr (BIAS) {
      lds_wait<0>();
      static_for<4>([&](auto qc) {
        constexpr int q = decltype(qc)::value;
        lds_touch(bf[(18 - PD + q) % PD]);
        bq[q] = *(const float4v *)&bf[(18 - PD + q) % PD];
      });
    }
    return acc;
  };
  auto prefetch_row = [&](auto &bf, const char *rm, auto pdc) {
    constexpr int PD = decltype(pdc)::value;
    if constexpr (M16) {
      const uint32_t row = lds_of(rm) + x16 * PS + g4 * 16;
      static_for<PD>([&](auto ic) {
        constexpr int item = decltype(ic)::value, dx = item >> 1, hf = item & 1;
        lds_read128<(dx + 16 * hf) * PS>(bf[item], row);
      });
      return;
    }
    const uint32_t row = lds_of(rm) + x * PS + h * 16;
    static_for<PD>([&](auto ic) {
      constexpr int item = decltype(ic)::value, dx = item >> 1, ks = item & 1;
      lds_read128<dx * PS + ks * 32>(bf[item], row);
    });
  };
  auto load_wf = [&](half8 (&wf)[18], const void *w) {
#pragma unroll
    for (int i = 0; i < 18; ++i) wf[i] = *(const half8 *)((const char *)w + i * 1024 + lane * 16);
#pragma unroll
    for (int i = 0; i < 18; ++i) asm volatile("" ::"v"(wf[i]));
  };
  auto store_row = [&](char *ring, auto nrc, int g, const half4 (&o)[4]) {
    char *dst = ring + slot_of(nrc, g) * ROWB + (x + 1) * PS + 16 * h;
#pragma unroll
    for (int qq = 0; qq < 2; ++qq) *(uint4v *)(dst + 32 * qq) = pair16(o[2 * qq], o[2 * qq + 1]);
  };
  auto load_wf_m = [&](half8 (&wf)[18], const char *w, int istride) {
#pragma unroll
    for (int i = 0; i < 18; ++i) wf[i] = *(const half8 *)(w + (size_t)((i & ~1) + (g4 >> 1)) * istride + ((g4 & 1) * 32 + 16 * (i & 1) + p16) * 16);
#pragma unroll
    for (int i = 0; i < 18; ++i) asm volatile("" ::"v"(wf[i]));
  };
  auto conv18m = [&](const half8 (&wf)[18], auto &bf, bool pre, const char *rm, const char *r0, const char *rp, int bias_off, float4v (&bq)[2], auto pdc, auto bc, float4v (&acc)[2][2]) {
    constexpr int PD = decltype(pdc)::value;
    constexpr bool BIAS = decltype(bc)::value;
    const int lo = x16 * PS + g4 * 16;
    const uint32_t rows[3] = {lds_of(rm) + lo, lds_of(r0) + lo, lds_of(rp) + lo};
    const uint32_t ba = BIAS ? lds_of((const char *)(BL + bias_off + 4 * g4)) : 0u;
    static_assert(PD <= 6 && (!BIAS || PD >= 2), "the first PD items lie in one row; the two bias quads ride in the last fragment slots");
    auto rd = [&](auto itc) {
      constexpr int item = decltype(itc)::value, tp = item >> 1, hf = item & 1, dy = tp / 3, dx = tp - dy * 3;
      lds_read128<(dx + 16 * hf) * PS>(bf[item % PD], rows[dy]);
    };
    if (!pre) static_for<PD>([&](auto ic) { rd(ic); });
#pragma unroll
    for (int q = 0; q < 4; ++q) acc[q >> 1][q & 1] = float4v{0.f, 0.f, 0.f, 0.f};
    static_for<18>([&](auto itc) {
      constexpr int item = decltype(itc)::value, tp = item >> 1, hf = item & 1;
      constexpr int frags_behind = (17 - item) < (PD - 1) ? (17 - item) : (PD - 1);
      constexpr int bias_behind = !BIAS ? 0 : item - (18 - PD) > 0 ? (item - (18 - PD) < 2 ? item - (18 - PD) : 2) : 0;
      lds_wait<frags_behind + bias_behind>();
      lds_touch(bf[item % PD]);
      acc[0][hf] = __builtin_amdgcn_mfma_f32_16x16x32_f16(wf[2 * tp], bf[item % PD], acc[0][hf], 0, 0, 0);
      acc[1][hf] = __builtin_amdgcn_mfma_f32_16x16x32_f16(wf[2 * tp + 1], bf[item % PD], acc[1][hf], 0, 0, 0);
      if constexpr (item + PD < 18) rd(std::integral_constant<int, item + PD>{});
      else if constexpr (BIAS && item - (18 - PD) < 2) lds_read128<(item - (18 - PD)) * 64>(bf[item % PD], ba);
    });
    if constexpr (BIAS) {
      lds_wait<0>();
      static_for<2>([&](auto cc) {
        constexpr int c = decltype(cc)::value;
        lds_touch(bf[(18 - PD + c) % PD]);
        bq[c] = *(const float4v *)&bf[(18 - PD + c) % PD];
      });
    }
  };
  auto store_row_m = [&](char *ring, auto nrc, int g, const half4 (&o)[2][2]) {
    char *dst = ring + slot_of(nrc, g) * ROWB + (x16 + 1) * PS + 8 * g4;
#pragma unroll
    for (int q = 0; q < 4; ++q) *(half4 *)(dst + 32 * (q >> 1) + 16 * PS * (q & 1)) = o[q >> 1][q & 1];
  };
#ifdef MLT_PHASE_TIMING
#define L0_PH_FLUSH() do { if (lane == 0 && unit == 0 && stage < 4) { for (int i_ = 0; i_ < 8; ++i_) atomicAdd(&g_phase_l0[stage][i_], ph_acc[i_]); } } while (0)
#else
#define L0_PH_FLUSH()
#endif
#define L0_STEP_END_PRE(n) asm volatile("s_waitcnt lgkmcnt(%0)\n\ts_barrier" ::"n"(n) : "memory")
#define L0_STEP_END() do { if (CFG_L0_KO & 8) asm volatile("s_waitcnt lgkmcnt(0)" ::: "memory"); else asm volatile("s_waitcnt lgkmcnt(0)\n\ts_barrier" ::: "memory"); } while (0)
  auto step_end = [&](auto &bf, bool &pre, char *ring, auto nrc, int g_next, auto pdc) {
    constexpr int PD = decltype(pdc)::value;
    if (CFG_L0_XPRE && !(CFG_L0_KO & 9) && g_next >= 0 && g_next < rows_total) {
      prefetch_row(bf, map_row(ring, nrc, g_next - 1, (g_next & 63) - 1), pdc);
      pre = true;
      L0_STEP_END_PRE(PD);
    } else {
      pre = false;
      L0_STEP_END();
    }
  };

  if (stage == 0) {
    half8 am[5];
#pragma unroll
    for (int k = 0; k < 5; ++k) am[k] = *(const half8 *)((const char *)a.w + k * 1024 + lane * 16);
#pragma unroll
    for (int k = 0; k < 5; ++k) asm volatile("" ::"v"(am[k]));
    constexpr int RD = CFG_L0_RD;
    static_assert(RD % 2 == 0, "RD");
    uint2v vo[RD], vp[RD], no[RD], np[RD];
    const int rsel = F5 ? 2 * wave + h : unit;
    const bool rlane = F5 || h == 0;
    auto issue = [&](uint2v &o2, uint2v &p2, int G) {
      G = G < 128 * nloc ? G : 128 * nloc - 1;
      const int c = G >> 7, y = G & 127;
      const size_t n = (size_t)blockIdx.x + (size_t)c * gridDim.x;
      o2 = *(const uint2v *)(a.org + n * a.org_cu_stride + (size_t)y * a.org_row_stride + 4 * p);
      p2 = *(const uint2v *)(a.pred + n * a.pred_cu_stride + (size_t)y * a.pred_row_stride + 4 * p);
    };
    auto commit = [&](const uint2v &o2, const uint2v &p2, int G, bool live = true) {
      live = live && rlane && G < 128 * nloc;
      uint4v w;
#pragma unroll
      for (int jj = 0; jj < 4; ++jj) {
        const int16_t o = (int16_t)(o2[jj >> 1] >> (16 * (jj & 1))), q = (int16_t)(p2[jj >> 1] >> (16 * (jj & 1)));
        w[jj] = prep_pair(o, q);
      }
      if (a.flat) {
        const int fb = live ? quad_flat_bits(w[0], w[1], w[2], w[3]) : 0;
        const unsigned long long b1 = __ballot(fb & 1), b2 = __ballot(fb & 2);
        const int nflat = __builtin_popcount((unsigned)(h ? b1 >> 32 : b1)) + (__builtin_popcount((unsigned)(h ? b2 >> 32 : b2)) << MLT_FLAT_EXACT_SHIFT);
        if (nflat && p == 0 && live) atomicAdd(FL + ((G >> 7) & 1), nflat);
      }
      if (live) *(uint4v *)(Raw + (G & (NRAW - 1)) * RAWB + 16 + 16 * p) = w;
    };
    issue(vo[0], vp[0], rsel); commit(vo[0], vp[0], rsel);
    if (unit == 0) { issue(vo[0], vp[0], 4); commit(vo[0], vp[0], 4, h == 0); }
#pragma unroll
    for (int d = 0; d < RD; ++d) issue(vo[d], vp[d], 4 * d + 5 + rsel);
    L0_STEP_END();
    PH_DECL;
    for (int k0 = 0; k0 < ksteps; k0 += RD) { static_for<RD>([&](auto slc) {
      constexpr int sl = decltype(slc)::value;
      const int k = k0 + sl;
      if (k >= ksteps) return;
      PH_MARK(3);
      commit(vo[sl], vp[sl], 4 * k + 5 + rsel);
      if constexpr (sl < RD / 2) {
        issue(no[2 * sl], np[2 * sl], 4 * (k0 + RD + 2 * sl) + 5 + rsel);
        issue(no[2 * sl + 1], np[2 * sl + 1], 4 * (k0 + RD + 2 * sl + 1) + 5 + rsel);
      }
      PH_MARK(0);
#pragma unroll
      for (int u = 0; u < (F5 ? 2 : 1); ++u) {
      const int g = 2 * k + (F5 ? u : par);
      if (g < rows_total) {
        const int c = g >> 6, r = g & 63;
        half8 bk[5];
#pragma unroll
        for (int dy = 0; dy < 5; ++dy) bk[dy] = read16(raw_row(c, 2 * r - 2 + dy), 2 * x + 2 + 4 * h);
        float16v acc;
#pragma unroll
        for (int i = 0; i < 16; ++i) acc[i] = 0.f;
#pragma unroll
        for (int dy = 0; dy < 5; ++dy) acc = __builtin_amdgcn_mfma_f32_32x32x16_f16(am[dy], bk[dy], acc, 0, 0, 0);
        if (r == 0 || blk == 0) {
          const bool topb = r == 0, leftb = x == 0;
          if (blk == 0) {
            const uint32_t l4 = *(const uint32_t *)(raw_row(c, 2 * r + 2) + 16), c0 = *(const uint32_t *)(raw_row(c, 0) + 16);
            uint4v bb;
            if (h == 0) {
              bb[0] = ((const uint32_t *)&bk[0])[2]; bb[1] = ((const uint32_t *)&bk[1])[2];
              bb[2] = ((const uint32_t *)&bk[2])[2]; bb[3] = ((const uint32_t *)&bk[3])[2];
            } else {
              bb[0] = l4; bb[1] = topb ? c0 : 0u; bb[2] = 0u; bb[3] = 0u;
            }
            if (!leftb) bb = uint4v{0u, 0u, 0u, 0u};
            acc = __builtin_amdgcn_mfma_f32_32x32x16_f16(*(const half8 *)(WB + lane * 16), *(half8 *)&bb, acc, 0, 0, 0);
          }
          if (topb) {
            uint4v bb = *(const uint4v *)&bk[2];
            if (h == 1) { bb[1] = 0u; bb[2] = 0u; bb[3] = 0u; }
            acc = __builtin_amdgcn_mfma_f32_32x32x16_f16(*(const half8 *)(WB + 1024 + lane * 16), *(half8 *)&bb, acc, 0, 0, 0);
          }
        }
        PH_MARK(1);
        half4 ov[4];
        static_for<4>([&](auto qc) {
          constexpr int q = decltype(qc)::value;
          const float4v b1q = *(const float4v *)(BL + 4 * h + 8 * q);
          const half4 none{};
          ov[q] = act_quad<q>(acc, a.acc_scale, b1q, false, none, true);
        });
        store_row(Tr, nrt, g, ov);
        PH_MARK(2);
      }
      }
      L0_STEP_END();
    });
#pragma unroll
      for (int d = 0; d < RD; ++d) { vo[d] = no[d]; vp[d] = np[d]; }
    }
    L0_PH_FLUSH();
  } else if (stage == 1) {
    half8 wf[18], bf[CFG_L0_PD - 1];
    bool pre = false;
    constexpr std::integral_constant<int, CFG_L0_PD - 1> pdc{};
    if constexpr (M16) load_wf_m(wf, (const char *)a.w2, 1024); else load_wf(wf, a.w2);
    L0_STEP_END();
    PH_DECL;
    for (int k = 0; k < ksteps; ++k) {
      PH_MARK(3);
      const int g = 2 * k + par - 3;
      if constexpr (M16) {
        if (g >= 0 && g < rows_total) {
          const int c = g >> 6, r = g & 63;
          const char *s0 = (g4 >> 1) ? raw_row(c, 2 * r + 1) : (g4 & 1) ? raw_row(c, 2 * r) : raw_row(c, 2 * r - 1);
          const uint32_t wa = lds_of(WB + 2048 + (g4 >> 1) * 1024 + ((g4 & 1) * 32 + p16) * 16);
          float4v accs[2][2];
          {
            half8 a0, a1;
            lds_read128<0>(a0, wa);
            lds_read128<256>(a1, wa);
            const half8 sb0 = read16(s0, 2 * x16 + 2), sb1 = read16(s0, 2 * (x16 + 16) + 2);
            lds_wait<0>();
            lds_touch(a0); lds_touch(a1);
            const float4v z4 = {0.f, 0.f, 0.f, 0.f};
            accs[0][0] = __builtin_amdgcn_mfma_f32_16x16x32_f16(a0, sb0, z4, 0, 0, 0);
            accs[1][0] = __builtin_amdgcn_mfma_f32_16x16x32_f16(a1, sb0, z4, 0, 0, 0);
            accs[0][1] = __builtin_amdgcn_mfma_f32_16x16x32_f16(a0, sb1, z4, 0, 0, 0);
            accs[1][1] = __builtin_amdgcn_mfma_f32_16x16x32_f16(a1, sb1, z4, 0, 0, 0);
          }
          static_for<2>([&](auto cc) {
            constexpr int cq = decltype(cc)::value;
            const float4v bq = *(const float4v *)(BL + 32 + 16 * cq + 4 * g4);
#pragma unroll
            for (int hf = 0; hf < 2; ++hf)
#pragma unroll
              for (int ep = 0; ep < 2; ++ep) {
                const float2v s2 = {accs[cq][hf][2 * ep], accs[cq][hf][2 * ep + 1]}, b2 = {bq[2 * ep], bq[2 * ep + 1]};
                const float2v y2 = s2 * a.acc_scale + b2;
                accs[cq][hf][2 * ep] = y2[0]; accs[cq][hf][2 * ep + 1] = y2[1];
              }
          });
          float4v bqs[2], acc[2][2];
          PH_MARK(0);
          conv18m(wf, bf, pre, map_row(Tr, nrt, g - 1, r - 1), map_row(Tr, nrt, g, r), map_row(Tr, nrt, g + 1, r + 1), 32, bqs, pdc, std::false_type{}, acc);
          half4 hq[2][2];
          PH_MARK(1);
#pragma unroll
          for (int q = 0; q < 4; ++q)
#pragma unroll
            for (int ep = 0; ep < 2; ++ep) {
              const float2v c2 = {acc[q >> 1][q & 1][2 * ep], acc[q >> 1][q & 1][2 * ep + 1]}, y2 = {accs[q >> 1][q & 1][2 * ep], accs[q >> 1][q & 1][2 * ep + 1]};
              const float2v x2 = c2 + y2;
              half2v h2 = __builtin_convertvector(x2, half2v);
              h2 = __builtin_elementwise_max(h2, (half2v){(_Float16)0, (_Float16)0});
              hq[q >> 1][q & 1][2 * ep] = h2[0];
              hq[q >> 1][q & 1][2 * ep + 1] = h2[1];
            }
          store_row_m(Br, nrb, g, hq);
          PH_MARK(2);
        }
        step_end(bf, pre, Tr, nrt, g + 2, pdc);
        continue;
      }
      if (g >= 0 && g < rows_total) {
        const int c = g >> 6, r = g & 63;
        const char *s0 = h ? raw_row(c, 2 * r) : raw_row(c, 2 * r - 1);
        const half8 sb0 = read16(s0, 2 * x + 2), sb1 = read16(raw_row(c, 2 * r + 1), 2 * x + 2);
        float16v accs;
#pragma unroll
        for (int i = 0; i < 16; ++i) accs[i] = 0.f;
        accs = __builtin_amdgcn_mfma_f32_32x32x16_f16(*(const half8 *)(WB + 2048 + lane * 16), sb0, accs, 0, 0, 0);
        accs = __builtin_amdgcn_mfma_f32_32x32x16_f16(*(const half8 *)(WB + 3072 + lane * 16), sb1, accs, 0, 0, 0);
        static_for<4>([&](auto qc) {
          constexpr int q = decltype(qc)::value;
          const float4v bq = *(const float4v *)(BL + 32 + 4 * h + 8 * q);
#pragma unroll
          for (int ep = 0; ep < 2; ++ep) {
            const float2v s2 = {accs[4 * q + 2 * ep], accs[4 * q + 2 * ep + 1]}, b2 = {bq[2 * ep], bq[2 * ep + 1]};
            const float2v y2 = s2 * a.acc_scale + b2;
            accs[4 * q + 2 * ep] = y2[0]; accs[4 * q + 2 * ep + 1] = y2[1];
          }
        });
        float4v bqs[4];
        PH_MARK(0);
        const float16v acc = conv18(wf, bf, pre, map_row(Tr, nrt, g - 1, r - 1), map_row(Tr, nrt, g, r), map_row(Tr, nrt, g + 1, r + 1), 32, bqs, pdc, std::false_type{});
        half4 hq[4];
        PH_MARK(1);
        if (CFG_L0_KO & 4) { asm volatile("" ::"v"(acc), "v"(accs)); step_end(bf, pre, Tr, nrt, g + 2, pdc); continue; }
        static_for<4>([&](auto qc) {
          constexpr int q = decltype(qc)::value;
#pragma unroll
          for (int ep = 0; ep < 2; ++ep) {
            const float2v c2 = {acc[4 * q + 2 * ep], acc[4 * q + 2 * ep + 1]}, y2 = {accs[4 * q + 2 * ep], accs[4 * q + 2 * ep + 1]};
            const float2v x2 = c2 + y2;
            half2v h2 = __builtin_convertvector(x2, half2v);
            h2 = __builtin_elementwise_max(h2, (half2v){(_Float16)0, (_Float16)0});
            hq[q][2 * ep] = h2[0];
            hq[q][2 * ep + 1] = h2[1];
          }
        });
        store_row(Br, nrb, g, hq);
        PH_MARK(2);
      }
      step_end(bf, pre, Tr, nrt, g + 2, pdc);
    }
    L0_PH_FLUSH();
  } else if (stage == 2) {
    half8 wf[18], bf[CFG_L0_PD];
    bool pre = false;
    constexpr std::integral_constant<int, CFG_L0_PD> pdc{};
    if constexpr (M16) load_wf_m(wf, (const char *)a.w3, 1024); else load_wf(wf, a.w3);
    L0_STEP_END();
    PH_DECL;
    for (int k = 0; k < ksteps; ++k) {
      PH_MARK(3);
      const int g = 2 * k + par - 6;
      if constexpr (M16) {
        if (g >= 0 && g < rows_total) {
          const int r = g & 63;
          float4v bqs[2], acc[2][2];
          PH_MARK(0);
          conv18m(wf, bf, pre, map_row(Br, nrb, g - 1, r - 1), map_row(Br, nrb, g, r), map_row(Br, nrb, g + 1, r + 1), 64, bqs, pdc, std::true_type{}, acc);
          half4 o[2][2];
          PH_MARK(1);
          const half4 none{};
#pragma unroll
          for (int q = 0; q < 4; ++q) o[q >> 1][q & 1] = act_quad<0>(acc[q >> 1][q & 1], 1.f, bqs[q >> 1], false, none, true);
          store_row_m(Ur, nru, g, o);
          PH_MARK(2);
        }
        step_end(bf, pre, Br, nrb, g + 2, pdc);
        continue;
      }
      if (g >= 0 && g < rows_total) {
        const int r = g & 63;
        float4v bqs[4];
        PH_MARK(0);
        const float16v acc = conv18(wf, bf, pre, map_row(Br, nrb, g - 1, r - 1), map_row(Br, nrb, g, r), map_row(Br, nrb, g + 1, r + 1), 64, bqs, pdc, std::true_type{});
        half4 o[4];
        PH_MARK(1);
        if (CFG_L0_KO & 4) { asm volatile("" ::"v"(acc)); step_end(bf, pre, Br, nrb, g + 2, pdc); continue; }
        if constexpr (CFG_L0_PKEPI) {
          static_for<4>([&](auto qc) {
            constexpr int q = decltype(qc)::value;
            const half4 none{};
            o[q] = act_quad<q>(acc, 1.f, bqs[q], false, none, true);
          });
        } else {
#pragma unroll
          for (int q = 0; q < 4; ++q) {
            const float4v bq = bqs[q];
#pragma unroll
            for (int e = 0; e < 4; ++e) o[q][e] = (_Float16)fmaxf(acc[4 * q + e] + bq[e], 0.f);
          }
        }
        store_row(Ur, nru, g, o);
        PH_MARK(2);
      }
      step_end(bf, pre, Br, nrb, g + 2, pdc);
    }
    L0_PH_FLUSH();
  } else if (stage == 3) {
    half8 wf[18], bf[CFG_L0_PD];
    bool pre = false;
    constexpr std::integral_constant<int, CFG_L0_PD> pdc{};
    if constexpr (M16) load_wf_m(wf, (const char *)a.w4, 1024); else load_wf(wf, a.w4);
    L0_STEP_END();
    PH_DECL;
    for (int k = 0; k < ksteps; ++k) {
      PH_MARK(3);
      const int g = 2 * k + par - 9;
      if constexpr (M16) {
        if (g >= 0 && g < rows_total) {
          const int c = g >> 6, r = g & 63;
          float4v bqs[2], acc[2][2];
          PH_MARK(0);
          conv18m(wf, bf, pre, map_row(Ur, nru, g - 1, r - 1), map_row(Ur, nru, g, r), map_row(Ur, nru, g + 1, r + 1), 96, bqs, pdc, std::true_type{}, acc);
          const char *rsrc = Br + slot_of(nrb, g) * ROWB + (x16 + 1) * PS + 8 * g4;
          half4 hq[2][2];
          PH_MARK(1);
#pragma unroll
          for (int q = 0; q < 4; ++q) {
            const half4 rr = *(const half4 *)(rsrc + 32 * (q >> 1) + 16 * PS * (q & 1));
            hq[q >> 1][q & 1] = act_quad<0>(acc[q >> 1][q & 1], 1.f, bqs[q >> 1], true, rr, true);
          }
          const size_t n = (size_t)blockIdx.x + (size_t)c * gridDim.x;
          if (a.flat && r == 63 && blk == 0 && lane == 0) {
            const int v = FL[c & 1];
            FL[c & 1] = 0;
            if (v) atomicAdd(a.flat + n, v);
          }
          if constexpr (F5) store_row_m(Or, nro, g, hq);
          else {
            char *cu_out = (char *)a.y + n * (size_t)(64 * 64 * 32 * 2);
            const uint32_t ob = (uint32_t)(((r * 64 + x16) * 32 + 4 * g4) * 2);
#pragma unroll
            for (int q = 0; q < 4; ++q) *(half4 *)(cu_out + ob + 32 * (q >> 1) + 16 * 64 * (q & 1)) = hq[q >> 1][q & 1];
          }
        }
        PH_MARK(2);
        step_end(bf, pre, Ur, nru, g + 2, pdc);
        continue;
      }
      if (g >= 0 && g < rows_total) {
        const int c = g >> 6, r = g & 63;
        float4v bqs[4];
        PH_MARK(0);
        const float16v acc = conv18(wf, bf, pre, map_row(Ur, nru, g - 1, r - 1), map_row(Ur, nru, g, r), map_row(Ur, nru, g + 1, r + 1), 96, bqs, pdc, std::true_type{});
        const char *rsrc = Br + slot_of(nrb, g) * ROWB + (x + 1) * PS + 16 * h;
        half4 hq[4];
        PH_MARK(1);
        if (CFG_L0_KO & 4) { asm volatile("" ::"v"(acc)); step_end(bf, pre, Ur, nru, g + 2, pdc); continue; }
        static_for<2>([&](auto qc) {
          constexpr int qq = decltype(qc)::value;
          half4 rr[2];
          unpair16(*(const uint4v *)(rsrc + 32 * qq), rr[0], rr[1]);
          if constexpr (CFG_L0_PKEPI) {
            hq[2 * qq] = act_quad<2 * qq>(acc, 1.f, bqs[2 * qq], true, rr[0], true);
            hq[2 * qq + 1] = act_quad<2 * qq + 1>(acc, 1.f, bqs[2 * qq + 1], true, rr[1], true);
          } else {
#pragma unroll
            for (int kk = 0; kk < 2; ++kk) {
              const float4v bq = bqs[2 * qq + kk];
#pragma unroll
              for (int e = 0; e < 4; ++e) hq[2 * qq + kk][e] = (_Float16)fmaxf(acc[8 * qq + 4 * kk + e] + bq[e] + (float)rr[kk][e], 0.f);
            }
          }
        });
        const size_t n = (size_t)blockIdx.x + (size_t)c * gridDim.x;
        if (a.flat && r == 63 && blk == 0 && lane == 0) {
          const int v = FL[c & 1];
          FL[c & 1] = 0;
          if (v) atomicAdd(a.flat + n, v);
        }
        if constexpr (F5) store_row(Or, nro, g, hq);
        else {
          char *cu_out = (char *)a.y + n * (size_t)(64 * 64 * 32 * 2);
          const uint32_t ob = (uint32_t)(((r * 64 + x) * 32 + 8 * h) * 2);
#pragma unroll
          for (int qq = 0; qq < 2; ++qq) *(uint4v *)(cu_out + ob + 32 * qq) = pair16(hq[2 * qq], hq[2 * qq + 1]);
        }
      }
      PH_MARK(2);
      step_end(bf, pre, Ur, nru, g + 2, pdc);
    }
    L0_PH_FLUSH();
  } else if constexpr (F5) {
    const int cb = wave - 2;
    constexpr int PD = CFG_L0_PD;
    static_assert(PD == 4, "four slots for the shortcut's four operands");
    half8 wf[18], bf[PD];
    if constexpr (M16) load_wf_m(wf, (const char *)a.w5 + cb * 1024, 2048);
    else {
#pragma unroll
      for (int i = 0; i < 18; ++i) wf[i] = *(const half8 *)((const char *)a.w5 + (i * 2 + cb) * 1024 + lane * 16);
#pragma unroll
      for (int i = 0; i < 18; ++i) asm volatile("" ::"v"(wf[i]));
    }
    const uint32_t wsa = M16 ? lds_of(W5 + cb * 2048 + (g4 >> 1) * 1024 + ((g4 & 1) * 32 + p16) * 16) : lds_of(W5 + cb * 2048 + lane * 16);
    L0_STEP_END();
    for (int k = 0; k < ksteps; ++k) {
      const int G5 = k - 6;
      if constexpr (M16) {
        if (G5 >= 0 && G5 < 32 * nloc) {
          const int c = G5 >> 5, Y = G5 & 31, g0 = 2 * G5;
          const int lo = (2 * p16) * PS + g4 * 16;
          const uint32_t rows[3] = {lds_of(map_row(Or, nro, g0 - 1, 2 * Y - 1)) + lo, lds_of(Or + slot_of(nro, g0) * ROWB) + lo, lds_of(Or + slot_of(nro, g0 + 1) * ROWB) + lo};
          auto rd = [&](auto itc) {
            constexpr int item = decltype(itc)::value, tp = item >> 1, hf = item & 1, dy = tp / 3, dx = tp - dy * 3;
            lds_read128<(dx + 32 * hf) * PS>(bf[item % PD], rows[dy]);
          };
          static_for<PD>([&](auto ic) { rd(ic); });
          float4v acc[2][2];
#pragma unroll
          for (int q = 0; q < 4; ++q) acc[q >> 1][q & 1] = float4v{0.f, 0.f, 0.f, 0.f};
          static_for<18>([&](auto itc) {
            constexpr int item = decltype(itc)::value, tp = item >> 1, hf = item & 1, e = item - (18 - PD);
            lds_wait<((17 - item) < (PD - 1) ? (17 - item) : (PD - 1)) + (e > 0 ? e : 0)>();
            lds_touch(bf[item % PD]);
            acc[0][hf] = __builtin_amdgcn_mfma_f32_16x16x32_f16(wf[2 * tp], bf[item % PD], acc[0][hf], 0, 0, 0);
            acc[1][hf] = __builtin_amdgcn_mfma_f32_16x16x32_f16(wf[2 * tp + 1], bf[item % PD], acc[1][hf], 0, 0, 0);
            if constexpr (item + PD < 18) rd(std::integral_constant<int, item + PD>{});
            else if constexpr (e < 2) lds_read128<(1 + 32 * e) * PS>(bf[item % PD], rows[1]);
            else lds_read128<(e - 2) * 256>(bf[item % PD], wsa);
          });
          const size_t n = (size_t)blockIdx.x + (size_t)c * gridDim.x;
          char *cu_t = (char *)a.y_t + n * (size_t)(32 * 32 * 64 * 2) + (Y * 32 * 64 + cb * 32) * 2;
          char *cu_sc = (char *)a.y_sc + n * (size_t)(32 * 32 * 64 * 2) + (((2 * cb) << 10) + Y * 32) * 32;
          const uint32_t ot = (uint32_t)(p16 * 128 + g4 * 8), os = (uint32_t)(p16 * 32 + g4 * 8);
          const float *bl5 = BL + 128 + 32 * cb + 4 * g4;
          const half4 none{};
#pragma unroll
          for (int q = 0; q < 4; ++q)
            *(half4 *)(cu_t + ot + 32 * (q >> 1) + 16 * 128 * (q & 1)) = act_quad<0>(acc[q >> 1][q & 1], a.scale5, *(const float4v *)(bl5 + 16 * (q >> 1)), false, none, true);
          lds_wait<0>();
          static_for<PD>([&](auto ic) { lds_touch(bf[decltype(ic)::value]); });
          float4v accs[2][2];
          const float4v z4 = {0.f, 0.f, 0.f, 0.f};
#pragma unroll
          for (int q = 0; q < 4; ++q) accs[q >> 1][q & 1] = __builtin_amdgcn_mfma_f32_16x16x32_f16(bf[(18 - PD + 2 + (q >> 1)) % PD], bf[(18 - PD + (q & 1)) % PD], z4, 0, 0, 0);
#pragma unroll
          for (int q = 0; q < 4; ++q)
            *(half4 *)(cu_sc + os + (q >> 1) * (1024 * 32) + 16 * 32 * (q & 1)) = act_quad<0>(accs[q >> 1][q & 1], a.scale5, *(const float4v *)(bl5 + 64 + 16 * (q >> 1)), false, none, false);
        }
        L0_STEP_END();
        continue;
      }
      if (G5 >= 0 && G5 < 32 * nloc) {
        const int c = G5 >> 5, Y = G5 & 31, g0 = 2 * G5;
        const int lo = (2 * p) * PS + h * 16;
        const uint32_t rows[3] = {lds_of(map_row(Or, nro, g0 - 1, 2 * Y - 1)) + lo, lds_of(Or + slot_of(nro, g0) * ROWB) + lo, lds_of(Or + slot_of(nro, g0 + 1) * ROWB) + lo};
        auto rd = [&](auto itc) {
          constexpr int item = decltype(itc)::value, tp = item >> 1, ks = item & 1, dy = tp / 3, dx = tp - dy * 3;
          lds_read128<dx * PS + ks * 32>(bf[item % PD], rows[dy]);
        };
        static_for<PD>([&](auto ic) { rd(ic); });
        float16v acc;
#pragma unroll
        for (int i = 0; i < 16; ++i) acc[i] = 0.f;
        static_for<18>([&](auto itc) {
          constexpr int item = decltype(itc)::value, e = item - (18 - PD);
          lds_wait<((17 - item) < (PD - 1) ? (17 - item) : (PD - 1)) + (e > 0 ? e : 0)>();
          lds_touch(bf[item % PD]);
          acc = __builtin_amdgcn_mfma_f32_32x32x16_f16(wf[item], bf[item % PD], acc, 0, 0, 0);
          if constexpr (item + PD < 18) rd(std::integral_constant<int, item + PD>{});
          else if constexpr (e < 2) lds_read128<PS + e * 32>(bf[item % PD], rows[1]);
          else lds_read128<(e - 2) * 1024>(bf[item % PD], wsa);
        });
        const size_t n = (size_t)blockIdx.x + (size_t)c * gridDim.x;
        char *cu_t = (char *)a.y_t + n * (size_t)(32 * 32 * 64 * 2) + (Y * 32 * 64 + cb * 32) * 2;
        char *cu_sc = (char *)a.y_sc + n * (size_t)(32 * 32 * 64 * 2) + (((2 * cb) << 10) + Y * 32) * 32;
        const uint32_t ot = (uint32_t)(p * 128 + h * 16), os = (uint32_t)(p * 32 + h * 16);
        const float *bl5 = BL + 128 + 32 * cb + 4 * h;
        static_for<2>([&](auto qc) {
          constexpr int qq = decltype(qc)::value;
          const half4 none{};
          const half4 h0 = act_quad<2 * qq>(acc, a.scale5, *(const float4v *)(bl5 + 8 * (2 * qq)), false, none, true);
          const half4 h1 = act_quad<2 * qq + 1>(acc, a.scale5, *(const float4v *)(bl5 + 8 * (2 * qq + 1)), false, none, true);
          *(uint4v *)(cu_t + ot + 32 * qq) = pair16(h0, h1);
        });
        lds_wait<0>();
        static_for<PD>([&](auto ic) { lds_touch(bf[decltype(ic)::value]); });
        float16v accs;
#pragma unroll
        for (int i = 0; i < 16; ++i) accs[i] = 0.f;
        accs = __builtin_amdgcn_mfma_f32_32x32x16_f16(bf[(18 - PD + 2) % PD], bf[(18 - PD) % PD], accs, 0, 0, 0);
        accs = __builtin_amdgcn_mfma_f32_32x32x16_f16(bf[(18 - PD + 3) % PD], bf[(18 - PD + 1) % PD], accs, 0, 0, 0);
        static_for<2>([&](auto qc) {
          constexpr int qq = decltype(qc)::value;
          const half4 none{};
          const half4 s0 = act_quad<2 * qq>(accs, a.scale5, *(const float4v *)(bl5 + 64 + 8 * (2 * qq)), false, none, false);
          const half4 s1 = act_quad<2 * qq + 1>(accs, a.scale5, *(const float4v *)(bl5 + 64 + 8 * (2 * qq + 1)), false, none, false);
          *(uint4v *)(cu_sc + os + qq * (1024 * 32)) = pair16(s0, s1);
        });
      }
      L0_STEP_END();
    }
  }
#undef L0_STEP_END
}
```

fastintercu-vvc_amd/csrc/mlt_layer1_kernel.inc:

```
#ifndef CFG_L1_PD
#define CFG_L1_PD 4
#endif
#ifndef CFG_L1_KO
#define CFG_L1_KO 0
#endif
template <bool M16>
__global__ __launch_bounds__(1024) void layer1_stream_kernel(const Layer1Args a) {
  constexpr int PS = 144, RW = 34, ROWB = RW * PS;
  constexpr int NRT = 4, NRB = 8, NRU = 4;
  constexpr int HB = 4096;
  constexpr int HEQ = 1104, HEH = 576, HE = 4 * HEQ;
  constexpr int PD = CFG_L1_PD;
  extern __shared__ __attribute__((aligned(16))) char smem[];
  char *Tr = smem, *Br = Tr + NRT * ROWB, *Ur = Br + NRB * ROWB, *Z = Ur + NRU * ROWB;
  char *Sc = Z + ROWB;
  char *Hd = Sc + 2 * 4096;
  char *He = Hd + 3 * 2 * 2 * HB;
  float *BL = (float *)(He + 2 * 2 * HE);
  constexpr int ZERO_BYTES = (NRT + NRB + NRU + 1) * ROWB + 2 * 4096;
  static_assert(ZERO_BYTES % 16 == 0 && MLT_L1_LDS_BYTES == ZERO_BYTES + 3 * 2 * 2 * HB + 2 * 2 * HE + 3 * 64 * 4, "LDS layout");
  const int tid = threadIdx.x, lane = tid & 63;
  const int wave = __builtin_amdgcn_readfirstlane(tid >> 6);
  const int p = lane & 31, h = lane >> 5;
  if ((int)blockIdx.x >= a.n) return;
  const int nloc = (a.n - (int)blockIdx.x + (int)gridDim.x - 1) / (int)gridDim.x;
  const int rows_total = 32 * nloc, ksteps = rows_total + 11;
  for (int o = tid * 16; o < ZERO_BYTES; o += 1024 * 16) *(uint4v *)(smem + o) = uint4v{0u, 0u, 0u, 0u};
  if (tid < 192) BL[tid] = a.bias[tid >> 6][tid & 63];
  asm volatile("s_waitcnt vmcnt(0) lgkmcnt(0)\n\ts_barrier" ::: "memory");
  const uint32_t lds0 = (uint32_t)(uintptr_t)LDS_PTR(smem);
  auto lds_of = [&](const char *q) -> uint32_t { return lds0 + (uint32_t)(q - smem); };
  auto row_of = [&](char *ring, int mask, int g, int r) -> const char * { return (r >= 0 && r < 32) ? ring + (g & mask) * ROWB : Z; };
#define L1_STEP_END() asm volatile("s_waitcnt lgkmcnt(0)\n\ts_barrier" ::: "memory")

  if (wave < 12) {
    const int pair = wave >> 1, cb = wave & 1;
    const int cv = pair < 2 ? 0 : pair < 4 ? 1 : 2;
    const bool second = pair == 1 || pair == 2 || pair == 5;
    const int lag = cv == 0 ? (second ? 3 : 2) : cv == 1 ? (second ? 6 : 5) : (second ? 9 : 8);
    char *in_ring = cv == 0 ? Tr : cv == 1 ? Br : Ur;
    const int in_mask = cv == 1 ? NRB - 1 : NRT - 1;
    half8 wf[18];
    const int p16 = lane & 15, g4 = lane >> 4;
    if constexpr (!M16) {
      const char *w = (const char *)a.w[cv] + (((second ? 18 : 0) * 2 + cb) * 1024) + lane * 16;
#pragma unroll
      for (int i = 0; i < 18; ++i) wf[i] = *(const half8 *)(w + i * 2048);
    } else {
#pragma unroll
      for (int i = 0; i < 18; ++i) {
        const int item = (second ? 18 : 0) + (i & ~1) + (g4 >> 1), lsrc = (g4 & 1) * 32 + 16 * (i & 1) + p16;
        wf[i] = *(const half8 *)((const char *)a.w[cv] + (size_t)(((item * 2 + cb) * 64 + lsrc) * 16));
      }
    }
#pragma unroll
    for (int i = 0; i < 18; ++i) asm volatile("" ::"v"(wf[i]));
    char *hand = Hd + ((cv * 2 + cb) * 2) * HB;
    char *hand_e = He + (cb * 2) * HE;
    const float scale = a.scale[cv];
    L1_STEP_END();
    for (int k = 0; k < ksteps; ++k) {
      const int g = k - lag;
      if (g >= 0 && g < rows_total) {
        const int r = g & 31;
        const int lo = M16 ? p16 * PS + g4 * 16 : p * PS + h * 16;
        const uint32_t rows[3] = {lds_of(row_of(in_ring, in_mask, g - 1, r - 1)) + lo, lds_of(in_ring + (g & in_mask) * ROWB) + lo, lds_of(row_of(in_ring, in_mask, g + 1, r + 1)) + lo};
        half8 bf[PD];
        if constexpr (M16) {
          float4v acc[2][2];
          auto run = [&](auto secc) {
            constexpr int S0 = decltype(secc)::value ? 9 : 0;
            auto rd = [&](auto itc) {
              constexpr int item = decltype(itc)::value, S = S0 + (item >> 1), hf = item & 1, tap = S >> 1, kh = S & 1, dy = tap / 3, dx = tap - dy * 3;
              lds_read128<(dx + 16 * hf) * PS + kh * 64>(bf[item % PD], rows[dy]);
            };
            static_for<PD>([&](auto ic) { rd(ic); });
            static_for<18>([&](auto itc) {
              constexpr int item = decltype(itc)::value, s = item >> 1, hf = item & 1;
              lds_wait<((17 - item) < (PD - 1) ? (17 - item) : (PD - 1))>();
              lds_touch(bf[item % PD]);
              acc[0][hf] = __builtin_amdgcn_mfma_f32_16x16x32_f16(wf[2 * s], bf[item % PD], acc[0][hf], 0, 0, 0);
              acc[1][hf] = __builtin_amdgcn_mfma_f32_16x16x32_f16(wf[2 * s + 1], bf[item % PD], acc[1][hf], 0, 0, 0);
              if constexpr (item + PD < 18) rd(std::integral_constant<int, item + PD>{});
            });
          };
          if (!second) {
#pragma unroll
            for (int q = 0; q < 4; ++q) acc[q >> 1][q & 1] = float4v{0.f, 0.f, 0.f, 0.f};
            run(std::false_type{});
            char *hw = hand + (k & 1) * HB + lane * 16;
            if (CFG_L1_KO & 2) { asm volatile("" ::"v"(acc[0][0]), "v"(acc[0][1]), "v"(acc[1][0]), "v"(acc[1][1])); }
            else
#pragma unroll
            for (int q = 0; q < 4; ++q) *(float4v *)(hw + q * 1024) = acc[q >> 1][q & 1];
          } else {
            const char *hr = hand + ((k - 1) & 1) * HB + lane * 16;
#pragma unroll
            for (int q = 0; q < 4; ++q) acc[q >> 1][q & 1] = (CFG_L1_KO & 2) ? float4v{0.f, 0.f, 0.f, 0.f} : *(const float4v *)(hr + q * 1024);
            run(std::true_type{});
            if (cv == 2) {
              const int c_ = g >> 5;
              const size_t n = (size_t)blockIdx.x + (size_t)c_ * gridDim.x;
              char *cu_y = (char *)a.y + n * (size_t)(32 * 32 * 64 * 2);
              char *hwe = hand_e + (k & 1) * HE;
              static_for<4>([&](auto qc) {
                constexpr int c = decltype(qc)::value >> 1, hf = decltype(qc)::value & 1;
                const int pix = 16 * hf + p16;
                const half4 res = *(const half4 *)(Br + (g & (NRB - 1)) * ROWB + (pix + 1) * PS + cb * 64 + c * 32 + 8 * g4);
                float v[4];
                const half4 o4 = act_quad<0>(acc[c][hf], scale, *(const float4v *)(BL + 2 * 64 + cb * 32 + 16 * c + 4 * g4), true, res, true, v);
                const uint32_t oy = a.y_c16 ? (uint32_t)(((((2 * cb + c) << 10) + r * 32 + pix) * 16 + 4 * g4) * 2)
                                            : (uint32_t)((((r * 32 + pix) * 64) + cb * 32 + 16 * c + 4 * g4) * 2);
                *(half4 *)(cu_y + oy) = o4;
                *(float4v *)(hwe + (2 * c + (g4 >> 1)) * HEQ + (g4 & 1) * HEH + pix * 16) = float4v{fmaxf(v[0], 0.f), fmaxf(v[1], 0.f), fmaxf(v[2], 0.f), fmaxf(v[3], 0.f)};
              });
            } else {
              char *drow = (cv == 0 ? Br + (g & (NRB - 1)) * ROWB : Ur + (g & (NRU - 1)) * ROWB);
              static_for<4>([&](auto qc) {
                constexpr int c = decltype(qc)::value >> 1, hf = decltype(qc)::value & 1;
                const int pix = 16 * hf + p16;
                half4 res{};
                if (cv == 0) res = *(const half4 *)(Sc + ((g & 1) * 4 + 2 * cb + c) * 1024 + pix * 32 + 8 * g4);
                const half4 o4 = act_quad<0>(acc[c][hf], scale, *(const float4v *)(BL + cv * 64 + cb * 32 + 16 * c + 4 * g4), cv == 0, res, true);
                *(half4 *)(drow + (pix + 1) * PS + cb * 64 + c * 32 + 8 * g4) = o4;
              });
            }
          }
        } else {
        float16v acc;
        auto run = [&](auto secc) {
          constexpr int I0 = decltype(secc)::value ? 18 : 0;
          auto rd = [&](auto itc) {
            constexpr int item = decltype(itc)::value, it = I0 + item, tap = it >> 2, ks = it & 3, dy = tap / 3, dx = tap - dy * 3;
            lds_read128<dx * PS + ks * 32>(bf[item % PD], rows[dy]);
          };
          static_for<PD>([&](auto ic) { rd(ic); });
          static_for<18>([&](auto itc) {
            constexpr int item = decltype(itc)::value;
            lds_wait<((17 - item) < (PD - 1) ? (17 - item) : (PD - 1))>();
            lds_touch(bf[item % PD]);
            acc = __builtin_amdgcn_mfma_f32_32x32x16_f16(wf[item], bf[item % PD], acc, 0, 0, 0);
            if constexpr (item + PD < 18) rd(std::integral_constant<int, item + PD>{});
          });
        };
        if (!second) {
#pragma unroll
          for (int i = 0; i < 16; ++i) acc[i] = 0.f;
          run(std::false_type{});
          char *hw = hand + (k & 1) * HB + lane * 16;
          if (CFG_L1_KO & 2) asm volatile("" ::"v"(acc));
          else
#pragma unroll
          for (int q = 0; q < 4; ++q) *(float4v *)(hw + q * 1024) = float4v{acc[4 * q], acc[4 * q + 1], acc[4 * q + 2], acc[4 * q + 3]};
        } else {
          const char *hr = hand + ((k - 1) & 1) * HB + lane * 16;
#pragma unroll
          for (int q = 0; q < 4; ++q) {
            const float4v v = (CFG_L1_KO & 2) ? float4v{0.f, 0.f, 0.f, 0.f} : *(const float4v *)(hr + q * 1024);
            acc[4 * q] = v[0]; acc[4 * q + 1] = v[1]; acc[4 * q + 2] = v[2]; acc[4 * q + 3] = v[3];
          }
          run(std::true_type{});
          if (cv == 2) {
            const float *bl = BL + 2 * 64 + cb * 32 + 4 * h;
            const char *rs = Br + (g & (NRB - 1)) * ROWB + (p + 1) * PS + cb * 64 + 16 * h;
            const int c = g >> 5;
            const size_t n = (size_t)blockIdx.x + (size_t)c * gridDim.x;
            char *cu_y = (char *)a.y + n * (size_t)(32 * 32 * 64 * 2);
            float v[16];
            static_for<2>([&](auto qc) {
              constexpr int qq = decltype(qc)::value;
              half4 ra, rb;
              unpair16(*(const uint4v *)(rs + 32 * qq), ra, rb);
              const half4 h0 = act_quad<2 * qq>(acc, scale, *(const float4v *)(bl + 8 * (2 * qq)), true, ra, true, &v[4 * (2 * qq)]);
              const half4 h1 = act_quad<2 * qq + 1>(acc, scale, *(const float4v *)(bl + 8 * (2 * qq + 1)), true, rb, true, &v[4 * (2 * qq + 1)]);
              const uint32_t oy = a.y_c16 ? (uint32_t)(((((2 * cb + qq) << 10) + r * 32 + p) * 16 + 8 * h) * 2)
                                          : (uint32_t)((((r * 32 + p) * 64) + cb * 32 + 8 * h + 16 * qq) * 2);
              *(uint4v *)(cu_y + oy) = pair16(h0, h1);
            });
            char *hw = hand_e + (k & 1) * HE + h * HEH + p * 16;
#pragma unroll
            for (int q = 0; q < 4; ++q) *(float4v *)(hw + q * HEQ) = float4v{fmaxf(v[4 * q], 0.f), fmaxf(v[4 * q + 1], 0.f), fmaxf(v[4 * q + 2], 0.f), fmaxf(v[4 * q + 3], 0.f)};
          } else {
            const float *bl = BL + cv * 64 + cb * 32 + 4 * h;
            const char *rs = Sc + ((g & 1) * 4 + 2 * cb) * 1024 + p * 32 + 16 * h;
            char *dst = (cv == 0 ? Br + (g & (NRB - 1)) * ROWB : Ur + (g & (NRU - 1)) * ROWB) + (p + 1) * PS + cb * 64 + 16 * h;
            static_for<2>([&](auto qc) {
              constexpr int qq = decltype(qc)::value;
              half4 ra{}, rb{};
              if (cv == 0) unpair16(*(const uint4v *)(rs + qq * 1024), ra, rb);
              const half4 h0 = act_quad<2 * qq>(acc, scale, *(const float4v *)(bl + 8 * (2 * qq)), cv == 0, ra, true);
              const half4 h1 = act_quad<2 * qq + 1>(acc, scale, *(const float4v *)(bl + 8 * (2 * qq + 1)), cv == 0, rb, true);
              *(uint4v *)(dst + 32 * qq) = pair16(h0, h1);
            });
          }
        }
        }
      }
      L1_STEP_END();
    }
  } else {
    const int li = wave - 12;
    constexpr int RD = 4, NP = 1;
    uint4v tc[RD][NP], sc_[RD][NP], tn[RD][NP], sn[RD][NP];
    auto issue = [&](uint4v (&tv)[NP], uint4v (&sv)[NP], int k) {
      int gt = k, gs = k - 2;
      gt = gt < 0 ? 0 : gt < rows_total ? gt : rows_total - 1;
      gs = gs < 0 ? 0 : gs < rows_total ? gs : rows_total - 1;
      const size_t nt = (size_t)blockIdx.x + (size_t)(gt >> 5) * gridDim.x, ns = (size_t)blockIdx.x + (size_t)(gs >> 5) * gridDim.x;
#pragma unroll
      for (int i = 0; i < NP; ++i) {
        const int ch = NP * li + i;
        tv[i] = *(const uint4v *)((const char *)a.t + (nt * 1024 + (size_t)(gt & 31) * 32) * 128 + ch * 1024 + lane * 16);
        sv[i] = *(const uint4v *)((const char *)a.sc + (((ns * 4 + ch) << 10) + (size_t)(gs & 31) * 32) * 32 + lane * 16);
      }
    };
    auto commit = [&](const uint4v (&tv)[NP], const uint4v (&sv)[NP], int k) {
      const int gt = k, gs = k - 2;
#pragma unroll
      for (int i = 0; i < NP; ++i) {
        const int ch = NP * li + i;
        if (gt >= 0 && gt < rows_total) *(uint4v *)(Tr + (gt & (NRT - 1)) * ROWB + (8 * ch + (lane >> 3) + 1) * PS + (lane & 7) * 16) = tv[i];
        if (gs >= 0 && gs < rows_total) *(uint4v *)(Sc + ((gs & 1) * 4 + ch) * 1024 + lane * 16) = sv[i];
      }
    };
    const int cb = li & 1, ch = lane & 31;
    const int hh = (ch >> 2) & 1;
    const char *gbase = He + (cb * 2) * HE + (ch >> 3) * HEQ + hh * HEH + (ch & 3) * 4;
    auto gap_row = [&](int k) {
      const int g = k - 10;
      if (li < 2 && lane < 32 && g >= 0 && g < rows_total && !(CFG_L1_KO & 1)) {
        const int c = g >> 5, r = g & 31;
        const size_t n = (size_t)blockIdx.x + (size_t)c * gridDim.x;
        const char *src = gbase + ((k - 1) & 1) * HE;
        float x[32];
        static_for<32>([&](auto tc_) {
          constexpr int t = decltype(tc_)::value;
          constexpr int pr = t < 4 ? t : t < 12 ? t + 12 : t < 16 ? t - 8 : t < 20 ? t + 8 : t < 28 ? t - 12 : t;
          x[t] = *(const float *)(src + pr * 16);
        });
#pragma unroll
        for (int w = 16; w >= 1; w >>= 1)
#pragma unroll
          for (int i = 0; i < w; ++i) x[i] = x[2 * i] + x[2 * i + 1];
        a.gap[(n * a.gap_slots + r) * 64 + cb * 32 + ch] = x[0];
      }
    };
#pragma unroll
    for (int d = 0; d < RD; ++d) issue(tc[d], sc_[d], d);
    L1_STEP_END();
    for (int k0 = 0; k0 < ksteps; k0 += RD) {
      static_for<RD>([&](auto slc) {
        constexpr int sl = decltype(slc)::value;
        const int k = k0 + sl;
        if (k >= ksteps) return;
        if (!(CFG_L1_KO & 4)) commit(tc[sl], sc_[sl], k);
        if constexpr (sl < RD / 2 && !(CFG_L1_KO & 4)) {
          issue(tn[2 * sl], sn[2 * sl], k0 + RD + 2 * sl);
          issue(tn[2 * sl + 1], sn[2 * sl + 1], k0 + RD + 2 * sl + 1);
        }
        gap_row(k);
        L1_STEP_END();
      });
#pragma unroll
      for (int d = 0; d < RD; ++d)
#pragma unroll
        for (int i = 0; i < NP; ++i) { tc[d][i] = tn[d][i]; sc_[d][i] = sn[d][i]; }
    }
  }
#undef L1_STEP_END
}
```

fastintercu-vvc_amd/csrc/mlt_runtime.h:

```cpp
#pragma once
#include <hip/hip_runtime.h>

#include <algorithm>
#include <chrono>
#include <cmath>
#include <cstddef>
#include <cstdio>
#include <cstdlib>
#include <cstring>
#include <map>
#include <tuple>
#include <mutex>
#include <string>
#include <thread>
#include <vector>

#include "../../include/mltcnn.h"
#include "mlt_kernels.h"
#include "mlt_layout.h"
#include "mlt_model.h"
#include "mlt_tier_search.h"

const char *tuning_env(const char *name);

struct Tuning {
  const char *debug_dump_dir;
  int xl_kill, xl_kill_layer;
  long lat_pixels;
  bool no_exact_lat;
  bool exact_patch_big;
  int wg_cap, wg_cap0, wg_cap1, wg_cap2;
  bool l0_mfma32, l1_mfma32;
  bool no_chain, no_chain_s2, no_c16, chain64, no_block_fusion, no_l0_s5;
  int l0_stream_min, l1_stream_min;
  int guard_wait_mode;
  bool no_small_mix, no_mag_guard, no_graph;
};
const Tuning &tuning();

inline int size_index(int size) {
  switch (size) {
    case 128: return 0;
    case 64: return 1;
    case 32: return 2;
    case 16: return 3;
    default: return -1;
  }
}
inline int ilog2(int v) { int l = 0; while ((1 << l) < v) ++l; return l; }

struct NetCfg {
  int S = 0;
  mlt::Model *m = nullptr, *mback = nullptr, *mx = nullptr;
  unsigned back_mask = 0, x_units = 0;
  mlt::Model &model_of(int s, int u) const { return ((x_units >> (2 * s + u)) & 1u) ? *mx : (mback && ((back_mask >> (2 * s + u)) & 1u)) ? *mback : *m; }
  int h_in(int s) const { int h = S; for (int i = 0; i < s; ++i) h = h / 2 > 0 ? h / 2 : 1; return h; }
};

struct PlanStep {
  enum Kind : uint8_t {
    FLAT_STAT,
    LAYER0_STREAM,
    STEM_BLOCK,
    STEM5,
    CONV_S2,
    CHAIN,
    LAYER1_STREAM,
    CONV_B0C2,
    BLOCK32,
    CONV_B1C1,
    CONV_B1C2,
    HEADS
  } kind;
  int8_t s = 0;
  bool front = false;
  bool inside_s2 = false;
  bool x_c16 = false;
  bool sc_c16 = false;
  bool y_c16 = false;
};
using NetPlan = std::vector<PlanStep>;
using PlanKey = std::tuple<const void *, const void *, const void *, unsigned, unsigned, unsigned>;

struct SizeState {
  bool enabled = false, loaded = false;
  std::map<PlanKey, NetPlan> plans;
  bool exact = false;
  bool w2 = false;
  unsigned w2_mask = 0;
  unsigned w2_units = 0;
  unsigned x_mask = 0;
  unsigned x_units = 0;
  bool lite = false;
  bool cfg_flat_guard = false;
  int flat_div = 8;
  float guard_margin = 3e-3f;
  bool want_exact = false;
  bool flat_guard = false, margin_guard = false, calibrate = false;
  bool small_mix = false;
  bool calibrated = false;
  float mag_thr = 0.f, calib_rel = 0.f, mag_flag = 0.f;
  int mag_kind = 0;
  bool cfg_mag_guard = true;
  float calib_rms = 0.f, calib_max = 0.f;
  int calib_cus = 0, calib_caller_cus = 0;
  std::vector<char> blob;
  uint64_t reruns = 0;
  double guard_us[16] = {0};
  int guard_n[16] = {0};
  int size = 0, head_index = 0;
  int head_off() const { int off = 0; for (int h = 0; h < head_index; ++h) off += model.heads[h].classes; return off; }
  int head_classes() const { return model.heads[head_index].classes; }
  float min_conf = 0.f;
  float conf_band(float tolerance) const { return (min_conf > 0.f && margin_guard) ? MLT_CONF_BAND_FRAC * tolerance : 0.f; }
  float cand_cov = 0.f;
  int cand_max = 0;
  bool cand_used = false;
  bool cand_policy() const { return cand_cov > 0.f || cand_max > 0; }
  float cand_band(float tolerance) const { return (cand_policy() && margin_guard) ? MLT_CONF_BAND_FRAC * tolerance : 0.f; }
  mlt::Model model;
  mlt::Model model_exact;
  mlt::Model model_w2;
  mlt::Model model_xl;
  bool guards() const { return !exact && (flat_guard || margin_guard || mag_thr > 0.f) && model_exact.on_device; }
  NetCfg main_cfg() {
    NetCfg c;
    c.S = size; c.m = &model;
    if (w2) { c.mback = &model_w2; c.back_mask = w2_units; }
    if (x_units) { c.mx = &model_exact; c.x_units = x_units; }
    return c;
  }
  NetCfg exact_cfg() { NetCfg c; c.S = size; c.m = &model_exact; return c; }
};

struct GuardSlot {
  Lay::GuardFields::Ptrs d{};
  int *phase = nullptr;
  int32_t *h_count = nullptr;
  bool single = false;
};
struct GuardTail { int32_t *count, *idx, *flat; int flat_thr, near_thr; float margin, mag_thr; int32_t *next; float conf_band, cand_band; };

using Lay::StageSet;

struct GrowBuf {
  bool pinned = false;
  char *p = nullptr;
  size_t bytes = 0;
  int reserve(mlt_ctx *ctx, size_t want, const char *what, bool zero = false);
  void release() { if (p) (void)(pinned ? hipHostFree(p) : hipFree(p)); p = nullptr; bytes = 0; }
};

struct SingleCu {
  char *h_stage = nullptr, *d_stage = nullptr;
  Lay::SingleLay lay;
  hipGraph_t graph = nullptr;
  hipGraphExec_t exec = nullptr;
  uint64_t ws_gen_at_capture = 0;
  hipStream_t stream_at_capture = nullptr;
};

struct Deferred {
  char *h_in = nullptr, *d_in = nullptr;
  char *h_out = nullptr, *d_out = nullptr;
  Lay::DeferIn in;
  Lay::DeferOut out;
  uint64_t gen = 0;
  int n = 0;
  int n_launched[2] = {0, 0};
  uint64_t gen_of_set[2] = {~0ull, ~0ull};
  hipEvent_t done[2] = {nullptr, nullptr};
  bool has_cand[2] = {false, false};
  bool guard_pending[2] = {false, false};
  int phase[2] = {0, 0};
};

struct mlt_picture {
  mlt_ctx *owner = nullptr;
  int width = 0, height = 0;
  long pitch = 0;
  bool owned = false;
  bool vec = false;
  std::vector<int16_t *> plane;
};

struct ProfAcc { uint32_t launches = 0; double flops = 0, bytes = 0; std::vector<std::pair<hipEvent_t, hipEvent_t>> ev; };

struct mlt_ctx {
  std::vector<mlt_ctx *> peers;
  unsigned rr = 0;
  int device = 0;
  hipStream_t stream = nullptr;
  bool own_stream = false;
  SizeState sz[4];
  float guard_margin = 3e-3f;
  bool guard_margin_configured = false;
  int max_batch = 4096, chunk = 4096;
  char *ws = nullptr;
  size_t ws_bytes = 0;
  uint64_t ws_gen = 1;
  char *zero_page = nullptr;
  hipStream_t copy_stream = nullptr;
  hipEvent_t ev_h2d[2] = {nullptr, nullptr}, ev_done[2] = {nullptr, nullptr};
  int stage_chunk = 512;
  GrowBuf h_res{true};
  SingleCu single[12];
  Deferred deferred[4];
  GrowBuf stage;
  float tolerance = 1e-3f;
  bool xlite = false;
  GrowBuf guard_dev;
  Lay::GuardLay guard_lay;
  int32_t *guard_host = nullptr;
  int guard_phase[2] = {0, 0};
  hipEvent_t ev_guard = nullptr;
  GrowBuf gstage;
  GrowBuf sweep_guard_dev;
  Lay::SweepGuardLay sweep_guard_lay;
  int sweep_phase = 0;
  GrowBuf tree_dev;
  int32_t *tree_host = nullptr;
  std::vector<mlt_picture *> pictures;
  std::string err;
  bool profile = false;
  bool guard_select_kernel = false;
  bool lds_oob_zero = false;
  std::map<std::string, ProfAcc> prof;
  std::vector<std::string> prof_order;
  std::vector<std::string> *plan = nullptr;
  bool plan_detail = false;
};

static_assert(sizeof(mlt_decision) == 48 && sizeof(DecisionRec) == sizeof(mlt_decision), "mlt_decision is 48 bytes");
static_assert(offsetof(mlt_decision, confidence) == offsetof(DecisionRec, confidence) && offsetof(mlt_decision, level_mode) == offsetof(DecisionRec, level_mode) &&
              offsetof(mlt_decision, level_conf) == offsetof(DecisionRec, level_conf) && offsetof(mlt_decision, level_conf) == 32, "mlt_decision layout");

static_assert(sizeof(mlt_tree_node) == 32 && sizeof(TreeNodeRec) == 32 && offsetof(mlt_tree_node, size) == offsetof(TreeNodeRec, size) && offsetof(mlt_tree_node, parent) == 12 &&
              offsetof(TreeNodeRec, parent) == 12 && offsetof(mlt_tree_node, cand_mask) == offsetof(TreeNodeRec, cand_mask) && offsetof(mlt_tree_node, cand_mask) == 28, "mlt_tree_node layout");
static_assert(sizeof(mlt_tree_config) == 40, "mlt_tree_config is 40 bytes");
static_assert(sizeof(mlt_tree_picture) == 24 && MLT_TREES_ROW == MLT_MAX_LOGITS && MLT_TREES_LEVELS == Lay::TreeArena::kLevels && sizeof(TreesEntry) == 48, "mlt_predict_trees layouts");

static_assert(MLT_SWEEP_MAX_QPS == MLT_SWEEP_MAX_QPS_K, "the sweep kernel's point array holds the ABI's maximum");
static_assert(sizeof(mlt_candidates) == 40 && sizeof(CandRec) == sizeof(mlt_candidates) && offsetof(mlt_candidates, order) == offsetof(CandRec, order) &&
              offsetof(mlt_candidates, prob) == offsetof(CandRec, prob) && offsetof(mlt_candidates, prob) == 16, "mlt_candidates layout");

#define HIP_TRY(ctx, expr)                                                                             \
  do {                                                                                                 \
    hipError_t e__ = (expr);                                                                           \
    if (e__ != hipSuccess) {                                                                           \
      (ctx)->err = std::string(#expr) + ": " + hipGetErrorString(e__);                                 \
      return MLT_ERR_HIP;                                                                              \
    }                                                                                                  \
  } while (0)

#define LAUNCH_TRY(ctx, expr) do { if (!(ctx)->plan) HIP_TRY(ctx, expr); } while (0)

inline int check_size(mlt_ctx *ctx, int size, SizeState **out) {
  const int si = size_index(size);
  if (si < 0) { ctx->err = "unsupported CU size"; return MLT_ERR_ARG; }
  SizeState &st = ctx->sz[si];
  if (!st.enabled || !st.loaded) { ctx->err = "CU size not enabled or weights not loaded"; return MLT_ERR_SIZE_DISABLED; }
  *out = &st;
  return MLT_OK;
}

struct Planes {
  const int16_t *org, *pred;
  long org_rs, org_cs, pred_rs, pred_cs;
  static Planes dense(const int16_t *org, const int16_t *pred, int S) { return Planes{org, pred, S, (long)S * S, S, (long)S * S}; }
  bool aligned8() const { return (((uintptr_t)org | (uintptr_t)pred) & 7) == 0 && ((org_rs | org_cs | pred_rs | pred_cs) & 3) == 0; }
  template <class Args> void fill(Args &a) const {
    a.org = org; a.pred = pred; a.org_row_stride = org_rs; a.org_cu_stride = org_cs; a.pred_row_stride = pred_rs; a.pred_cu_stride = pred_cs;
  }
};

struct SweepPart {
  int n_qps = 0;
  int32_t qps[MLT_SWEEP_MAX_QPS] = {0};
  long slab = 0;
  const int32_t *idx = nullptr;
  uint32_t *mask = nullptr;
  const uint32_t *active = nullptr;
};

struct PassIO {
  Planes pl;
  const int32_t *poc, *qp;
  int32_t *split;
  float *logits;
  DecisionRec *dec;
  CandRec *cand = nullptr;
  SweepPart sweep;
};

struct GuardOut {
  int32_t *d_flat = nullptr;
  const GuardTail *tail = nullptr;
  bool flat_is_clear = false;
  float *d_mag = nullptr;
};

struct Launch {
  mlt_ctx *ctx;
  int prof_begin(const std::string &name, double flops, double bytes, hipEvent_t &e0, hipEvent_t &e1, const char *variant = nullptr);
  int prof_end(hipEvent_t e1);
};

inline int shard_lo(int n, int g, int G) { return (int)(((long long)n * g) / G); }
inline mlt_ctx *device_of(mlt_ctx *ctx, int i) { return i == 0 ? ctx : ctx->peers[(size_t)i - 1]; }
template <class F> int run_sharded(mlt_ctx *ctx, int n, F per_device) {
  const int G = 1 + (int)ctx->peers.size();
  std::vector<int> rcs((size_t)G, MLT_OK);
  auto run = [&](int g) { const int lo = shard_lo(n, g, G), hi = shard_lo(n, g + 1, G); if (hi > lo) rcs[(size_t)g] = per_device(g, lo, hi); };
  std::vector<std::thread> th;
  for (int g = 1; g < G; ++g) th.emplace_back(run, g);
  run(0);
  for (std::thread &t : th) t.join();
  for (int g = 0; g < G; ++g)
    if (rcs[(size_t)g]) { if (g) ctx->err = "device " + std::to_string(device_of(ctx, g)->device) + ": " + device_of(ctx, g)->err; return rcs[(size_t)g]; }
  return MLT_OK;
}

void free_pictures(mlt_ctx *ctx);
bool owns_picture(const mlt_ctx *ctx, const mlt_picture *pic);
struct AtPlanes {
  const int16_t *org; long org_pitch; bool org_vec;
  const int16_t *pred; long pred_pitch; bool pred_vec;
  static AtPlanes of(const mlt_picture *o, const mlt_picture *p, int g) { return AtPlanes{o->plane[(size_t)g], o->pitch, o->vec, p->plane[(size_t)g], p->pitch, p->vec}; }
};
struct AtList {
  const int32_t *xy, *poc, *qp;
  bool device; int32_t poc_all, qp_all;
  const int32_t *pic = nullptr; const TreesEntry *entries = nullptr; int n_entries = 0;
  static AtList host(const int32_t *xy, const int32_t *poc, const int32_t *qp) { return AtList{xy, poc, qp, false, 0, 0}; }
  static AtList on_device(const int32_t *d_xy, int32_t poc, int32_t qp) { return AtList{d_xy, nullptr, nullptr, true, poc, qp}; }
  static AtList of_entries(const int32_t *d_xy, const int32_t *d_pic, const TreesEntry *d_entries, int n) { return AtList{d_xy, nullptr, nullptr, true, 0, 0, d_pic, d_entries, n}; }
};
struct AtOut { int32_t *split; float *logits; mlt_decision *dec; mlt_candidates *cand; };
int predict_at_chunks(mlt_ctx *dev, SizeState *st, const AtPlanes &pl, int n, const AtList &at, const AtOut &out);
void release_ws(mlt_ctx *ctx);
int run_network(mlt_ctx *ctx, SizeState &st, const NetCfg &c, int n, const PassIO &io, const GuardOut &go = GuardOut());
int guard_slot(mlt_ctx *ctx, int which, int n, int nl, GuardSlot *g);
int run_fast_async(mlt_ctx *ctx, SizeState &st, int n, const PassIO &io, const GuardSlot &g);
int guard_fixup_async(mlt_ctx *ctx, SizeState &st, int k, const PassIO &io, const GuardSlot &g);
int run_checked(mlt_ctx *ctx, SizeState &st, int n, const PassIO &io);
int run_checked_sweep(mlt_ctx *ctx, SizeState &st, int n, const PassIO &io);
void free_model(mlt::Model &m);
void drop_graphs(mlt_ctx *ctx, int si);
```

Before: 1.016 million.

## Hand off strided shortcut input from layer0 stream to layer1 stream kernel

Instead of having the layer0 stream kernel compute the 1x1 stride-2 shortcut conv and write a 64-channel shortcut tensor, it now writes the 32-channel subsampled input (xs) and the layer1 stream kernel computes the shortcut conv itself with MFMA in its loader waves. This halves the shortcut tensor traffic between the two kernels and moves a small matmul into the consumer. The trade-off is extra MFMA and register pressure in the layer1 loader waves, a changed loop structure there, and the GAP row work is skipped on the xs loader waves (those waves li>=2 presumably never did GAP).

```diff
diff --git a/fastintercu-vvc_amd/csrc/mlt_dispatch.cpp b/fastintercu-vvc_amd/csrc/mlt_dispatch.cpp
--- a/fastintercu-vvc_amd/csrc/mlt_dispatch.cpp
+++ b/fastintercu-vvc_amd/csrc/mlt_dispatch.cpp
@@ -20,6 +20,7 @@
     u.no_block_fusion = on("MLT_NO_BLOCK_FUSION");
     u.no_chain = on("MLT_NO_CHAIN") || u.no_block_fusion; u.no_chain_s2 = on("MLT_NO_CHAIN_S2"); u.no_c16 = on("MLT_NO_C16"); u.chain64 = !on("MLT_NO_CHAIN64");
     u.no_l0_s5 = on("MLT_NO_L0_S5");
+    u.no_xs_handoff = on("MLT_NO_XS_HANDOFF") || u.debug_dump_dir != nullptr;
     u.l0_stream_min = on("MLT_NO_L0_STREAM") ? 0 : (int)num("MLT_L0_STREAM_MIN", 128);
     u.l1_stream_min = on("MLT_NO_L1_STREAM") ? 0 : (int)num("MLT_L1_STREAM_MIN", 128);
     u.guard_wait_mode = on("MLT_GUARD_SPIN_WAIT") ? 1 : on("MLT_GUARD_BLOCKING_WAIT") ? 2 : 0;
@@ -262,7 +263,7 @@
 }
 
 int run_layer0_stream(mlt_ctx *ctx, const mlt::Model &m0, const mlt::Model &m1, int n, const Planes &pl, void *y, int32_t *d_flat, bool flat_is_clear,
-                      const mlt::PackedConv *c5, void *y_t, void *y_sc) {
+                      const mlt::PackedConv *c5, void *y_t, void *y_sc, bool xs) {
   const mlt::PackedConv &c2 = m0.blocks[0][0].conv2;
   const mlt::Block &B1 = m1.blocks[0][1];
   Layer0Args a{};
@@ -277,13 +278,13 @@
   const double px = (double)n * 64 * 64;
   Launch L{ctx};
   hipEvent_t e0 = nullptr, e1 = nullptr;
-  int rc = c5 ? L.prof_begin("layer0_stream_h64(stem+layer0+layer1.0.conv1+sc)", 2.0 * px * 32 * (50 + 18 + 3 * 288) + 2.0 * (px / 4) * 64 * (288 + 32),
-                             (double)n * 128 * 128 * 4 + (px / 4) * 64 * 2 * 2, e0, e1)
+  int rc = c5 ? L.prof_begin("layer0_stream_h64(stem+layer0+layer1.0.conv1+sc)", 2.0 * px * 32 * (50 + 18 + 3 * 288) + 2.0 * (px / 4) * 64 * (288 + (xs ? 0 : 32)),
+                             (double)n * 128 * 128 * 4 + (px / 4) * (64 + (xs ? 32 : 64)) * 2, e0, e1, xs ? "xs hand-off" : nullptr)
               : L.prof_begin("layer0_stream_h64(stem+layer0.0+layer0.1)", 2.0 * px * 32 * (50 + 18 + 3 * 288), (double)n * 128 * 128 * 4 + px * 32 * 2, e0, e1);
   if (rc) return rc;
   const bool mfma32 = tuning().l0_mfma32;
   plan_note(ctx, {{"y", c5 ? nullptr : y}, {"y_t", c5 ? y_t : nullptr}, {"y_sc", c5 ? y_sc : nullptr}, {"flat", d_flat}}, {{"flat_is_clear", flat_is_clear}, {"grid", grid_x}});
-  LAUNCH_TRY(ctx, mlt_launch_layer0_stream(a, c5 != nullptr, mfma32, grid_x, ctx->stream));
+  LAUNCH_TRY(ctx, mlt_launch_layer0_stream(a, c5 != nullptr, mfma32, xs, grid_x, ctx->stream));
   if ((rc = L.prof_end(e1))) return rc;
   if (c5) {
     if ((rc = debug_dump(ctx, "conv3x3_s2_32to64_h32+sc", y_t, (size_t)(px / 4) * 64 * 2))) return rc;
@@ -360,8 +361,10 @@
   return MLT_OK;
 }
 
-int run_layer1_stream(mlt_ctx *ctx, const mlt::Block &B0, const mlt::Block &B1, int n, const void *t, const void *sc, void *y, float *gap, bool y_c16) {
+int run_layer1_stream(mlt_ctx *ctx, const mlt::Block &B0, const mlt::Block &B1, int n, const void *t, const void *sc, void *y, float *gap, bool y_c16, const mlt::PackedConv *c5xs) {
   Layer1Args a{};
+  const bool xs = c5xs != nullptr;
+  if (xs) { a.w_sc = c5xs->d_w; a.bias_sc = c5xs->d_bias_sc; a.scale_sc = c5xs->acc_scale; }
   a.t = t; a.sc = sc; a.y = y; a.y_c16 = y_c16 ? 1 : 0; a.gap = gap; a.gap_slots = gap_slots(32 * 32); a.n = n;
   const mlt::PackedConv *pcs[3] = {&B0.conv2, &B1.conv1, &B1.conv2};
   for (int k = 0; k < 3; ++k) { a.w[k] = pcs[k]->d_w; a.bias[k] = pcs[k]->d_bias; a.scale[k] = pcs[k]->acc_scale; }
@@ -370,11 +373,12 @@
   const double px = (double)n * 32 * 32;
   Launch L{ctx};
   hipEvent_t e0 = nullptr, e1 = nullptr;
-  int rc = L.prof_begin("layer1_stream_h32(conv2+conv1+conv2)", 3.0 * 2.0 * px * 64 * 64 * 9, px * 64 * 2 * 3 + 3.0 * 72 * 1024, e0, e1, y_c16 ? "single pass, y chunk-major, GAP" : "single pass, GAP");
+  int rc = L.prof_begin("layer1_stream_h32(conv2+conv1+conv2)", 3.0 * 2.0 * px * 64 * 64 * 9 + (xs ? 2.0 * px * 64 * 32 : 0.0), px * (64 * 2 + (xs ? 32 : 64)) * 2 + 3.0 * 72 * 1024 + (xs ? 4096.0 : 0.0), e0, e1,
+                        xs ? (y_c16 ? "xs hand-off, single pass, y chunk-major, GAP" : "xs hand-off, single pass, GAP") : y_c16 ? "single pass, y chunk-major, GAP" : "single pass, GAP");
   if (rc) return rc;
   const bool mfma32 = tuning().l1_mfma32;
   plan_note(ctx, {{"t", t}, {"sc", sc}, {"y", y}, {"gap", gap}}, {{"grid", grid_x}});
-  LAUNCH_TRY(ctx, mlt_launch_layer1_stream(a, mfma32, grid_x, ctx->stream));
+  LAUNCH_TRY(ctx, mlt_launch_layer1_stream(a, mfma32, xs, grid_x, ctx->stream));
   if ((rc = L.prof_end(e1))) return rc;
   return debug_dump(ctx, "chain3_s1_64_h32(conv2+conv1+conv2)", y, (size_t)px * 64 * 2);
 }
@@ -416,6 +420,7 @@
   };
   bool cur_c16 = false;
   bool l0_front = false;
+  int l0_front_step = -1;
   for (int s = 0; s < m.n_stages; ++s) {
     const bool last = s == m.n_stages - 1;
     const mlt::Model &ms = c.model_of(s, 0);
@@ -429,6 +434,7 @@
       l0_front = !tn.no_l0_s5 && m.n_stages > 1 && !m10.exact && !m10.w2 && wants_chain(1) && !wants_s2(1) && m.planes[1] == 64 && !tn.no_c16 &&
                  c5.has_sc && c5.taps == 9 && c5.kc == 32 && c5.ct == 64 && c5.cin == 32 && c5.cout == 64 && c5.stride == 2;
       add(PlanStep::LAYER0_STREAM, 0).front = l0_front;
+      if (l0_front) l0_front_step = (int)P.size() - 1;
       continue;
     }
     if (fused_b0) add(PlanStep::STEM_BLOCK, 0);
@@ -449,6 +455,7 @@
                             q2.taps == 9 && q2.kc == 64 && q2.ct == 64 && !last;
         PlanStep &st = add(stream ? PlanStep::LAYER1_STREAM : PlanStep::CHAIN, s);
         st.inside_s2 = chain_s2; st.x_c16 = cur_c16; st.sc_c16 = sc_c16; st.y_c16 = out_c16;
+        if (stream && l0_front && l0_front_step >= 0 && !tn.no_xs_handoff && !tn.l0_mfma32 && tn.l1_mfma32) st.xs = P[(size_t)l0_front_step].xs = true;
         cur_c16 = out_c16;
         continue;
       }
@@ -528,7 +535,7 @@
     }
     case PlanStep::LAYER0_STREAM:
       rc = run_layer0_stream(ctx, ms, mt, n, io.pl, outs[0], go.d_flat, go.flat_is_clear,
-                             ps.front ? &c.model_of(1, 0).blocks[1][0].conv1 : nullptr, pool[0], pool[1]);
+                             ps.front ? &c.model_of(1, 0).blocks[1][0].conv1 : nullptr, pool[0], pool[1], ps.front && ps.xs);
       break;
     case PlanStep::STEM_BLOCK:
       rc = run_stem_block(ctx, ms, n, S, io.pl, pool[2], go.d_flat, go.flat_is_clear);
@@ -547,7 +554,7 @@
                       ps.x_c16, ps.y_c16, pool[2], ps.sc_c16);
       break;
     case PlanStep::LAYER1_STREAM:
-      rc = run_layer1_stream(ctx, mt.blocks[s][0], mt.blocks[s][1], n, pool[0], pool[1], outs[s], gaps[s], ps.y_c16);
+      rc = run_layer1_stream(ctx, mt.blocks[s][0], mt.blocks[s][1], n, pool[0], pool[1], outs[s], gaps[s], ps.y_c16, ps.xs ? &c.model_of(1, 0).blocks[1][0].conv1 : nullptr);
       break;
     case PlanStep::CONV_B0C2:
       cv.x = pool[0]; cv.y = pool[2]; cv.res = pool[1]; cv.relu = true;
diff --git a/fastintercu-vvc_amd/csrc/mlt_kernels.h b/fastintercu-vvc_amd/csrc/mlt_kernels.h
--- a/fastintercu-vvc_amd/csrc/mlt_kernels.h
+++ b/fastintercu-vvc_amd/csrc/mlt_kernels.h
@@ -92,9 +92,13 @@
 };
 
 #define MLT_L1_LDS_BYTES 159008
+#define MLT_L1X_LDS_BYTES 159264
 struct Layer1Args {
   const void *t;
   const void *sc;
+  const void *w_sc;
+  const float *bias_sc;
+  float scale_sc;
   const void *w[3];
   const float *bias[3];
   float scale[3];
@@ -363,7 +367,7 @@
 hipError_t mlt_launch_stem5(const Stem5Args &a, int nsplit, int grid_x, int lds, hipStream_t st);
 hipError_t mlt_launch_block32(const Block32Args &a, bool w2, int grid_x, hipStream_t st);
 hipError_t mlt_launch_stem_block(const StemBlockArgs &a, bool w2, int grid_x, hipStream_t st);
-hipError_t mlt_launch_layer0_stream(const Layer0Args &a, bool fuse5, bool mfma32, int grid_x, hipStream_t st);
-hipError_t mlt_launch_layer1_stream(const Layer1Args &a, bool mfma32, int grid_x, hipStream_t st);
+hipError_t mlt_launch_layer0_stream(const Layer0Args &a, bool fuse5, bool mfma32, bool xs, int grid_x, hipStream_t st);
+hipError_t mlt_launch_layer1_stream(const Layer1Args &a, bool mfma32, bool xs, int grid_x, hipStream_t st);
 hipError_t mlt_launch_heads(const HeadArgs &a, int n, hipStream_t st);
 hipError_t mlt_launch_heads_sweep(const HeadSweepArgs &a, int n, hipStream_t st);
diff --git a/fastintercu-vvc_amd/csrc/mlt_kernels.hip b/fastintercu-vvc_amd/csrc/mlt_kernels.hip
--- a/fastintercu-vvc_amd/csrc/mlt_kernels.hip
+++ b/fastintercu-vvc_amd/csrc/mlt_kernels.hip
@@ -692,13 +692,26 @@
   hipLaunchKernelGGL((layer0_stream_kernel<F5, M16>), dim3(grid_x), dim3(1024), F5 ? MLT_L0F_LDS_BYTES : MLT_L0_LDS_BYTES, st, a);
   return hipGetLastError();
 }
-hipError_t mlt_launch_layer0_stream(const Layer0Args &a, bool fuse5, bool mfma32, int grid_x, hipStream_t st) {
+hipError_t mlt_launch_layer0_stream(const Layer0Args &a, bool fuse5, bool mfma32, bool xs, int grid_x, hipStream_t st) {
+  if (xs) {
+    if (!fuse5 || mfma32) return hipErrorInvalidValue;
+    static DeviceOnce once;
+    if (hipError_t e = ensure_big_lds(layer0_stream_xs_kernel, once); e != hipSuccess) return e;
+    hipLaunchKernelGGL(layer0_stream_xs_kernel, dim3(grid_x), dim3(1024), MLT_L0F_LDS_BYTES, st, a);
+    return hipGetLastError();
+  }
   if (fuse5) return mfma32 ? launch_layer0_stream_t<true, false>(a, grid_x, st) : launch_layer0_stream_t<true, true>(a, grid_x, st);
   return launch_layer0_stream_t<false, false>(a, grid_x, st);
 }
 
-hipError_t mlt_launch_layer1_stream(const Layer1Args &a, bool mfma32, int grid_x, hipStream_t st) {
-  static DeviceOnce once[2];
+hipError_t mlt_launch_layer1_stream(const Layer1Args &a, bool mfma32, bool xs, int grid_x, hipStream_t st) {
+  static DeviceOnce once[3];
+  if (xs) {
+    if (!mfma32 || !a.w_sc || !a.bias_sc) return hipErrorInvalidValue;
+    if (hipError_t e = ensure_big_lds(layer1_stream_xs_kernel, once[2]); e != hipSuccess) return e;
+    hipLaunchKernelGGL(layer1_stream_xs_kernel, dim3(grid_x), dim3(1024), MLT_L1X_LDS_BYTES, st, a);
+    return hipGetLastError();
+  }
   if (mfma32) {
     if (hipError_t e = ensure_big_lds(layer1_stream_kernel<false>, once[0]); e != hipSuccess) return e;
     hipLaunchKernelGGL(layer1_stream_kernel<false>, dim3(grid_x), dim3(1024), MLT_L1_LDS_BYTES, st, a);
diff --git a/fastintercu-vvc_amd/csrc/mlt_layer0_kernel.inc b/fastintercu-vvc_amd/csrc/mlt_layer0_kernel.inc
--- a/fastintercu-vvc_amd/csrc/mlt_layer0_kernel.inc
+++ b/fastintercu-vvc_amd/csrc/mlt_layer0_kernel.inc
@@ -19,8 +19,9 @@
 #ifndef CFG_L0_MAP
 #define CFG_L0_MAP 0
 #endif
-template <bool F5, bool M16>
-__global__ __launch_bounds__(1024) void layer0_stream_kernel(const Layer0Args a) {
+template <bool F5, bool M16, bool XS>
+__device__ __forceinline__ void layer0_stream_body(const Layer0Args &a) {
+  static_assert(!XS || (F5 && M16), "the xs hand-off exists for the five-stage 16x16x32 form");
   constexpr int PS = 80, RW = 66, ROWB = RW * PS;
   constexpr int NRT = F5 ? 6 : 8, NRB = 8, NRU = F5 ? 6 : 8, NRO = F5 ? 6 : 0;
   constexpr int RP = 136, RAWB = RP * 4, NRAW = 16;
@@ -57,11 +58,11 @@
     BL[96 + tid] = a.bias4[tid];
     if constexpr (F5) {
       BL[128 + tid] = a.bias5[tid]; BL[160 + tid] = a.bias5[32 + tid];
-      BL[192 + tid] = a.bias5_sc[tid]; BL[224 + tid] = a.bias5_sc[32 + tid];
+      if constexpr (!XS) { BL[192 + tid] = a.bias5_sc[tid]; BL[224 + tid] = a.bias5_sc[32 + tid]; }
     }
   }
   if (wave < 4) *(uint4v *)(WB + wave * 1024 + lane * 16) = *(const uint4v *)((const char *)a.w + ((wave < 2 ? 7 : 3) + wave) * 1024 + lane * 16);
-  if (F5 && wave >= 4 && wave < 8) {
+  if (F5 && !XS && wave >= 4 && wave < 8) {
     const int cb = (wave - 4) >> 1, ks = (wave - 4) & 1;
     *(uint4v *)(W5 + (cb * 2 + ks) * 1024 + lane * 16) = *(const uint4v *)((const char *)a.w5 + ((18 + ks) * 2 + cb) * 1024 + lane * 16);
   }
@@ -592,11 +593,12 @@
           for (int q = 0; q < 4; ++q) acc[q >> 1][q & 1] = float4v{0.f, 0.f, 0.f, 0.f};
           static_for<18>([&](auto itc) {
             constexpr int item = decltype(itc)::value, tp = item >> 1, hf = item & 1, e = item - (18 - PD);
-            lds_wait<((17 - item) < (PD - 1) ? (17 - item) : (PD - 1)) + (e > 0 ? e : 0)>();
+            lds_wait<((17 - item) < (PD - 1) ? (17 - item) : (PD - 1)) + (e > 0 ? (XS ? 1 : e) : 0)>();
             lds_touch(bf[item % PD]);
             acc[0][hf] = __builtin_amdgcn_mfma_f32_16x16x32_f16(wf[2 * tp], bf[item % PD], acc[0][hf], 0, 0, 0);
             acc[1][hf] = __builtin_amdgcn_mfma_f32_16x16x32_f16(wf[2 * tp + 1], bf[item % PD], acc[1][hf], 0, 0, 0);
             if constexpr (item + PD < 18) rd(std::integral_constant<int, item + PD>{});
+            else if constexpr (XS) { if constexpr (e == 0) lds_read128<PS>(bf[item % PD], rows[1] + cb * (32 * PS)); }
             else if constexpr (e < 2) lds_read128<(1 + 32 * e) * PS>(bf[item % PD], rows[1]);
             else lds_read128<(e - 2) * 256>(bf[item % PD], wsa);
           });
@@ -610,6 +612,10 @@
           for (int q = 0; q < 4; ++q)
             *(half4 *)(cu_t + ot + 32 * (q >> 1) + 16 * 128 * (q & 1)) = act_quad<0>(acc[q >> 1][q & 1], a.scale5, *(const float4v *)(bl5 + 16 * (q >> 1)), false, none, true);
           lds_wait<0>();
+          if constexpr (XS) {
+            lds_touch(bf[(18 - PD) % PD]);
+            *(half8 *)((char *)a.y_sc + n * (size_t)(32 * 32 * 32 * 2) + (Y * 32 + 16 * cb) * 64 + p16 * 64 + g4 * 16) = bf[(18 - PD) % PD];
+          } else {
           static_for<PD>([&](auto ic) { lds_touch(bf[decltype(ic)::value]); });
           float4v accs[2][2];
           const float4v z4 = {0.f, 0.f, 0.f, 0.f};
@@ -618,6 +624,7 @@
 #pragma unroll
           for (int q = 0; q < 4; ++q)
             *(half4 *)(cu_sc + os + (q >> 1) * (1024 * 32) + 16 * 32 * (q & 1)) = act_quad<0>(accs[q >> 1][q & 1], a.scale5, *(const float4v *)(bl5 + 64 + 16 * (q >> 1)), false, none, false);
+          }
         }
         L0_STEP_END();
         continue;
@@ -675,3 +682,6 @@
   }
 #undef L0_STEP_END
 }
+template <bool F5, bool M16>
+__global__ __launch_bounds__(1024) void layer0_stream_kernel(const Layer0Args a) { layer0_stream_body<F5, M16, false>(a); }
+__global__ __launch_bounds__(1024) void layer0_stream_xs_kernel(const Layer0Args a) { layer0_stream_body<true, true, true>(a); }
diff --git a/fastintercu-vvc_amd/csrc/mlt_layer1_kernel.inc b/fastintercu-vvc_amd/csrc/mlt_layer1_kernel.inc
--- a/fastintercu-vvc_amd/csrc/mlt_layer1_kernel.inc
+++ b/fastintercu-vvc_amd/csrc/mlt_layer1_kernel.inc
@@ -4,8 +4,9 @@
 #ifndef CFG_L1_KO
 #define CFG_L1_KO 0
 #endif
-template <bool M16>
-__global__ __launch_bounds__(1024) void layer1_stream_kernel(const Layer1Args a) {
+template <bool M16, bool XS>
+__device__ __forceinline__ void layer1_stream_body(const Layer1Args &a) {
+  static_assert(!XS || !M16, "the xs hand-off exists for the 32x32x16 form");
   constexpr int PS = 144, RW = 34, ROWB = RW * PS;
   constexpr int NRT = 4, NRB = 8, NRU = 4;
   constexpr int HB = 4096;
@@ -18,7 +19,7 @@
   char *He = Hd + 3 * 2 * 2 * HB;
   float *BL = (float *)(He + 2 * 2 * HE);
   constexpr int ZERO_BYTES = (NRT + NRB + NRU + 1) * ROWB + 2 * 4096;
-  static_assert(ZERO_BYTES % 16 == 0 && MLT_L1_LDS_BYTES == ZERO_BYTES + 3 * 2 * 2 * HB + 2 * 2 * HE + 3 * 64 * 4, "LDS layout");
+  static_assert(ZERO_BYTES % 16 == 0 && MLT_L1_LDS_BYTES == ZERO_BYTES + 3 * 2 * 2 * HB + 2 * 2 * HE + 3 * 64 * 4 && MLT_L1X_LDS_BYTES == MLT_L1_LDS_BYTES + 64 * 4, "LDS layout");
   const int tid = threadIdx.x, lane = tid & 63;
   const int wave = __builtin_amdgcn_readfirstlane(tid >> 6);
   const int p = lane & 31, h = lane >> 5;
@@ -27,6 +28,7 @@
   const int rows_total = 32 * nloc, ksteps = rows_total + 11;
   for (int o = tid * 16; o < ZERO_BYTES; o += 1024 * 16) *(uint4v *)(smem + o) = uint4v{0u, 0u, 0u, 0u};
   if (tid < 192) BL[tid] = a.bias[tid >> 6][tid & 63];
+  if (XS && tid >= 192 && tid < 256) BL[tid] = a.bias_sc[tid - 192];
   asm volatile("s_waitcnt vmcnt(0) lgkmcnt(0)\n\ts_barrier" ::: "memory");
   const uint32_t lds0 = (uint32_t)(uintptr_t)LDS_PTR(smem);
   auto lds_of = [&](const char *q) -> uint32_t { return lds0 + (uint32_t)(q - smem); };
@@ -211,7 +213,37 @@
       for (int i = 0; i < NP; ++i) {
         const int ch = NP * li + i;
         tv[i] = *(const uint4v *)((const char *)a.t + (nt * 1024 + (size_t)(gt & 31) * 32) * 128 + ch * 1024 + lane * 16);
-        sv[i] = *(const uint4v *)((const char *)a.sc + (((ns * 4 + ch) << 10) + (size_t)(gs & 31) * 32) * 32 + lane * 16);
+        if constexpr (!XS) sv[i] = *(const uint4v *)((const char *)a.sc + (((ns * 4 + ch) << 10) + (size_t)(gs & 31) * 32) * 32 + lane * 16);
+      }
+    };
+    const int cbx = li & 1;
+    half8 xa[2];
+    uint4v xr[RD][2];
+    auto issue_x = [&](uint4v (&xv)[2], int k) {
+      int gs = k - 2;
+      gs = gs < 0 ? 0 : gs < rows_total ? gs : rows_total - 1;
+      const size_t ns = (size_t)blockIdx.x + (size_t)(gs >> 5) * gridDim.x;
+      const char *src = (const char *)a.sc + ((ns * 1024 + (size_t)(gs & 31) * 32 + p) * 32 + 8 * h) * 2;
+      xv[0] = *(const uint4v *)src;
+      xv[1] = *(const uint4v *)(src + 32);
+    };
+    auto sc_row = [&](const uint4v (&xv)[2], int k) {
+      const int gs = k - 2;
+      if (gs >= 0 && gs < rows_total) {
+        float16v accs;
+#pragma unroll
+        for (int i = 0; i < 16; ++i) accs[i] = 0.f;
+        accs = __builtin_amdgcn_mfma_f32_32x32x16_f16(xa[0], *(const half8 *)&xv[0], accs, 0, 0, 0);
+        accs = __builtin_amdgcn_mfma_f32_32x32x16_f16(xa[1], *(const half8 *)&xv[1], accs, 0, 0, 0);
+        const float *bl = BL + 3 * 64 + cbx * 32 + 4 * h;
+        char *dst = Sc + ((gs & 1) * 4 + 2 * cbx) * 1024 + p * 32 + 16 * h;
+        static_for<2>([&](auto qc) {
+          constexpr int qq = decltype(qc)::value;
+          const half4 none{};
+          const half4 s0 = act_quad<2 * qq>(accs, a.scale_sc, *(const float4v *)(bl + 8 * (2 * qq)), false, none, false);
+          const half4 s1 = act_quad<2 * qq + 1>(accs, a.scale_sc, *(const float4v *)(bl + 8 * (2 * qq + 1)), false, none, false);
+          *(uint4v *)(dst + qq * 1024) = pair16(s0, s1);
+        });
       }
     };
     auto commit = [&](const uint4v (&tv)[NP], const uint4v (&sv)[NP], int k) {
@@ -220,7 +252,7 @@
       for (int i = 0; i < NP; ++i) {
         const int ch = NP * li + i;
         if (gt >= 0 && gt < rows_total) *(uint4v *)(Tr + (gt & (NRT - 1)) * ROWB + (8 * ch + (lane >> 3) + 1) * PS + (lane & 7) * 16) = tv[i];
-        if (gs >= 0 && gs < rows_total) *(uint4v *)(Sc + ((gs & 1) * 4 + ch) * 1024 + lane * 16) = sv[i];
+        if (!XS && gs >= 0 && gs < rows_total) *(uint4v *)(Sc + ((gs & 1) * 4 + ch) * 1024 + lane * 16) = sv[i];
       }
     };
     const int cb = li & 1, ch = lane & 31;
@@ -245,27 +277,52 @@
         a.gap[(n * a.gap_slots + r) * 64 + cb * 32 + ch] = x[0];
       }
     };
-#pragma unroll
-    for (int d = 0; d < RD; ++d) issue(tc[d], sc_[d], d);
-    L1_STEP_END();
-    for (int k0 = 0; k0 < ksteps; k0 += RD) {
-      static_for<RD>([&](auto slc) {
-        constexpr int sl = decltype(slc)::value;
-        const int k = k0 + sl;
-        if (k >= ksteps) return;
-        if (!(CFG_L1_KO & 4)) commit(tc[sl], sc_[sl], k);
-        if constexpr (sl < RD / 2 && !(CFG_L1_KO & 4)) {
-          issue(tn[2 * sl], sn[2 * sl], k0 + RD + 2 * sl);
-          issue(tn[2 * sl + 1], sn[2 * sl + 1], k0 + RD + 2 * sl + 1);
-        }
-        gap_row(k);
-        L1_STEP_END();
-      });
-#pragma unroll
-      for (int d = 0; d < RD; ++d)
-#pragma unroll
-        for (int i = 0; i < NP; ++i) { tc[d][i] = tn[d][i]; sc_[d][i] = sn[d][i]; }
-    }
+    auto loader = [&](auto xsc) {
+      constexpr bool X = decltype(xsc)::value;
+#pragma unroll
+      for (int d = 0; d < RD; ++d) issue(tc[d], sc_[d], d);
+      if constexpr (X) {
+#pragma unroll
+        for (int ks = 0; ks < 2; ++ks) xa[ks] = *(const half8 *)((const char *)a.w_sc + ((18 + ks) * 2 + cbx) * 1024 + lane * 16);
+        asm volatile("" ::"v"(xa[0]), "v"(xa[1]));
+        issue_x(xr[0], 0);
+        issue_x(xr[1], 1);
+      }
+      L1_STEP_END();
+      int k0 = 0;
+      for (; X ? k0 + RD <= ksteps : k0 < ksteps; k0 += RD) {
+        static_for<RD>([&](auto slc) {
+          constexpr int sl = decltype(slc)::value;
+          const int k = k0 + sl;
+          if constexpr (!X) { if (k >= ksteps) return; }
+          if (!(CFG_L1_KO & 4)) commit(tc[sl], sc_[sl], k);
+          if constexpr (sl < RD / 2 && !(CFG_L1_KO & 4)) {
+            issue(tn[2 * sl], sn[2 * sl], k0 + RD + 2 * sl);
+            issue(tn[2 * sl + 1], sn[2 * sl + 1], k0 + RD + 2 * sl + 1);
+          }
+          if constexpr (X && !(CFG_L1_KO & 4)) {
+            sc_row(xr[sl], k);
+            if constexpr (sl < RD / 2) {
+              issue_x(xr[RD / 2 + sl], k0 + RD / 2 + sl);
+              issue_x(xr[sl], k0 + RD + sl);
+            }
+          }
+          if constexpr (!X) gap_row(k);
+          L1_STEP_END();
+        });
+#pragma unroll
+        for (int d = 0; d < RD; ++d)
+#pragma unroll
+          for (int i = 0; i < NP; ++i) { tc[d][i] = tn[d][i]; sc_[d][i] = sn[d][i]; }
+      }
+      if constexpr (X)
+        for (; k0 < ksteps; ++k0) L1_STEP_END();
+    };
+    if (XS && li >= 2) loader(std::true_type{});
+    else loader(std::false_type{});
   }
 #undef L1_STEP_END
 }
+template <bool M16>
+__global__ __launch_bounds__(1024) void layer1_stream_kernel(const Layer1Args a) { layer1_stream_body<M16, false>(a); }
+__global__ __launch_bounds__(1024) void layer1_stream_xs_kernel(const Layer1Args a) { layer1_stream_body<false, true>(a); }
diff --git a/fastintercu-vvc_amd/csrc/mlt_runtime.h b/fastintercu-vvc_amd/csrc/mlt_runtime.h
--- a/fastintercu-vvc_amd/csrc/mlt_runtime.h
+++ b/fastintercu-vvc_amd/csrc/mlt_runtime.h
@@ -32,6 +32,7 @@
   int wg_cap, wg_cap0, wg_cap1, wg_cap2;
   bool l0_mfma32, l1_mfma32;
   bool no_chain, no_chain_s2, no_c16, chain64, no_block_fusion, no_l0_s5;
+  bool no_xs_handoff;
   int l0_stream_min, l1_stream_min;
   int guard_wait_mode;
   bool no_small_mix, no_mag_guard, no_graph;
@@ -74,6 +75,7 @@
   } kind;
   int8_t s = 0;
   bool front = false;
+  bool xs = false;
   bool inside_s2 = false;
   bool x_c16 = false;
   bool sc_c16 = false;
```

Result: faster. 1.032 million, median of 6 (+1.6%).
